# manuelbb-upb/Morbit.jl

Hardware: AMD Instinct MI355X
Metric: RBF build+solve+eval cycles/sec (higher is better)
Workload: dtype f64

## Files before the change

### include/mrbf.h

```cpp
#ifndef MRBF_H
#define MRBF_H

#include <stdint.h>

#ifdef __cplusplus
extern "C" {
#endif

typedef struct mrbf_ctx mrbf_ctx;
typedef struct mrbf_model mrbf_model;

enum {
    MRBF_CUBIC = 0,
    MRBF_INV_MULTIQUADRIC = 1,
    MRBF_MULTIQUADRIC = 2,
    MRBF_THIN_PLATE_SPLINE = 3,
    MRBF_GAUSSIAN = 4
};

enum {
    MRBF_OK = 0,
    MRBF_ENOTPD = 1,
    MRBF_ESINGULAR = 2,
    MRBF_EHIP = 3,
// ... 88 lines not shown
int32_t mrbf_affine_select(mrbf_ctx *ctx, int64_t mc, int32_t d, const double *shifted, int32_t j0, const double *Q0, int32_t max_picks,
                           double pivot_val, int32_t p_is_inf, int64_t *picked_out, int32_t *n_picked, double *Z_out);

typedef struct {
    int64_t mc;
    int32_t j0;
    int32_t max_picks;
    double pivot_val;
    const double *shifted;
    const double *Q0;
    int64_t *picked_out;
    double *Z_out;
    int32_t n_picked;
    int32_t reserved;
} mrbf_affine_job;
int32_t mrbf_affine_select_batch(mrbf_ctx *ctx, int64_t n_starts, int32_t d, int32_t p_is_inf, mrbf_affine_job *jobs,
                                 float *ms_total);

typedef struct mrbf_round4_state mrbf_round4_state;
int32_t mrbf_round4(mrbf_ctx *ctx, int64_t n0, int32_t d, const double *start_sites, int64_t mc, const double *cand_sites,
                    int32_t kernel_id, double a, double b, int32_t poly_deg, int32_t max_points, double theta_pivot_cholesky,
                    int32_t *accepted_out, int32_t *n_accepted, mrbf_round4_state **state);
int32_t mrbf_fit_from_round4(mrbf_ctx *ctx, const mrbf_round4_state *state, int32_t k, const double *values, mrbf_model **model,
                             double *weights_out, double *poly_out, mrbf_fit_info *info);
int32_t mrbf_round4_sites(const mrbf_round4_state *state, int64_t *n0, int64_t *n_candidates, int32_t *n_accepted);
int32_t mrbf_free_round4(mrbf_ctx *ctx, mrbf_round4_state *state);

typedef struct {
    int64_t n0, mc;
    const double *start_sites;
    const double *cand_sites;
    int32_t kernel_id, poly_deg;
    double a, b;
    int32_t max_points;
    double theta_pivot_cholesky;
    int32_t *accepted_out;
    int32_t n_accepted;
    int32_t rc;
} mrbf_round4_job;
int32_t mrbf_round4_batch(mrbf_ctx *ctx, int64_t n_starts, int32_t d, mrbf_round4_job *jobs, float *ms_total);

int32_t mrbf_model_dims(const mrbf_model *model, int64_t *n, int32_t *d, int32_t *k, int32_t *q);
int32_t mrbf_free_model(mrbf_ctx *ctx, mrbf_model *model);

typedef struct {
    int64_t n, m;
    int32_t d, k, kernel_id, poly_deg;
    double a, b;
    const double *centres;
    const double *values;
    const double *X;
    double *weights_out;
    double *poly_out;
    double *vals_out;
    double *jac_out;
} mrbf_problem;

typedef struct {
    int32_t status;
    int32_t device;
    mrbf_fit_info fit;
    float ms_eval;
    double checksum_w;
    double checksum_vals;
} mrbf_result;

int32_t mrbf_batch_run(int32_t n_dev, const int32_t *device_ids, int64_t n_problems, const mrbf_problem *problems,
                       mrbf_result *results);

typedef struct {
    int64_t n;
    int32_t d, k, kernel_id, poly_deg;
    double a, b;
    const double *centres, *values;
    double *weights_out, *poly_out;
    mrbf_model *model;
    int32_t status;
    int32_t reserved;
    mrbf_fit_info info;
} mrbf_fit_job;
int32_t mrbf_fit_batch(mrbf_ctx *ctx, int64_t n_starts, mrbf_fit_job *jobs, float *ms_total);

int32_t mrbf_debug_env(const char *name);
int32_t mrbf_debug_mfma_layout(mrbf_ctx *ctx, double *out16x16_a_times_b, const double *A16x4, const double *B4x16);
int32_t mrbf_debug_potrf(mrbf_ctx *ctx, int64_t n, double *A_colmajor_inout, int32_t impl, int32_t *info, float *ms);
int32_t mrbf_debug_diag(mrbf_ctx *ctx, const double *A128, int32_t reps, float *ms_per_call, double *shader_cycles,
                        double *realtime_us);
int32_t mrbf_debug_mfma_peak(mrbf_ctx *ctx, int32_t blocks_per_cu, int32_t threads, int32_t iters, float *ms, double *tflops);
int32_t mrbf_debug_mfma_asm(mrbf_ctx *ctx, int32_t variant, int32_t blocks_per_cu, int32_t iters, float *ms, double *tflops,
                            double *cycles_per_mfma);
int32_t mrbf_debug_dgemm(mrbf_ctx *ctx, int32_t m, int32_t n, int32_t k, float *ms, double *tflops);
int32_t mrbf_debug_mega_tables(int32_t nt, int32_t mt, int32_t slack, int32_t slack_chain, int32_t first, int32_t win, int32_t srows,
                               int32_t half_cols, int64_t *out6);
int32_t mrbf_debug_mega_tables2(int32_t nt, int32_t mt, int32_t slack, int32_t slack_chain, int32_t first, int32_t win, int32_t srows,
                                int32_t half_cols, const int32_t *opt5, int64_t *out6);
int32_t mrbf_debug_mega_plan(int32_t nt, int32_t mt, int32_t xreal, int64_t *out39);

enum { MRBF_PS_OK = 0, MRBF_PS_CRITICAL = 1, MRBF_PS_FAILURE = 2 };
typedef struct {
    int32_t max_ideal_evals;
    int32_t max_ps_evals;
    int32_t max_polish_evals;
    int32_t reserved;
    uint64_t seed;
    double t0;
    double xtol_rel;
} mrbf_ps_options;
typedef struct {
    int32_t status;
    int32_t generations;
    int32_t evals_ideal, evals_ps, evals_polish;
    float ms_total;
    double tau;
} mrbf_ps_info;
int32_t mrbf_ps_step(mrbf_ctx *ctx, const mrbf_model *model, const double *x_n, const double *lb_eff, const double *ub_eff,
                     const double *fx_n, const double *r_or_null, const mrbf_ps_options *opts, double *x_trial, double *mx_trial,
                     double *r_out, mrbf_ps_info *info);

enum { MRBF_ROLE_NONE = -1, MRBF_ROLE_EQ = -2, MRBF_ROLE_INEQ = -3 };
typedef struct {
    int32_t n_models, n_objectives;
    const mrbf_model *const *models;
    const int32_t *roles;
    int32_t n_lin_eq, n_lin_ineq;
    const double *A_eq, *b_eq, *A_ineq, *b_ineq;
    double eq_tol;
} mrbf_ps_problem;
int32_t mrbf_ps_step_problem(mrbf_ctx *ctx, const mrbf_ps_problem *problem, const double *x_n, const double *lb_eff,
                             const double *ub_eff, const double *fx_n, const double *r_or_null, const mrbf_ps_options *opts,
                             double *x_trial, double *mx_trial, double *r_out, mrbf_ps_info *info);
int32_t mrbf_debug_ps_rank(mrbf_ctx *ctx, int32_t lam, const double *f, const double *phi, uint64_t seed, int32_t gen, int32_t impl,
                           int32_t *order_out, int32_t *gave_up);

enum { MRBF_SD_OK = 0, MRBF_SD_NO_OBJECTIVE = 1, MRBF_SD_INFEASIBLE = 2, MRBF_SD_GAVE_UP = 3 };
int32_t mrbf_sd_direction(mrbf_ctx *ctx, int64_t n_lp, int32_t d, int32_t k, int32_t m_eq, int32_t m_ineq, const double *G,
                          const double *x, const double *lb, const double *ub, const double *A_eq, const double *b_eq,
                          const double *A_ineq, const double *b_ineq, int32_t normalize, double *d_out, double *omega_out,
                          double *dual_out, int32_t *status_out, int32_t *iters_out);
typedef struct {
    int32_t status;
    int32_t iterations;
    int32_t bound_flips;
    float ms_total;
    double omega;
} mrbf_sd_info;
int32_t mrbf_sd_criticality(mrbf_ctx *ctx, const mrbf_ps_problem *problem, const double *x, const double *x_n, const double *lb,
                            const double *ub, int32_t normalize, double *d_out, double *dual_out, mrbf_sd_info *info);

enum { MRBF_NS_OK = 0, MRBF_NS_INFEASIBLE = 1, MRBF_NS_GAVE_UP = 2 };
int32_t mrbf_normal_direction(mrbf_ctx *ctx, int64_t n_lp, int32_t d, int32_t m_eq, int32_t m_ineq, const double *x, const double *lb,
                              const double *ub, const double *A_eq, const double *b_eq, const double *A_ineq, const double *b_ineq,
                              double *n_out, double *alpha_out, double *dual_out, int32_t *status_out, int32_t *iters_out);
typedef struct {
    int32_t status;
    int32_t iterations;
    int32_t bound_flips;
    float ms_total;
    double alpha;
    double delta;
} mrbf_normal_info;
int32_t mrbf_normal_step(mrbf_ctx *ctx, const mrbf_ps_problem *problem, int32_t d, const double *x, const double *lb, const double *ub,
                         double delta, double kappa_delta, double delta_max, int32_t variable_radius, double *n_out, double *dual_out,
                         mrbf_normal_info *info);

typedef struct {
    int32_t strict;
    int32_t max_loops;
    double const_rhs;
    double shrink;
    double min_stepsize;
} mrbf_sd_step_options;
typedef struct {
    int32_t branch;
    int32_t loops;
    float ms_total;
    double sigma;
    double omega;
    double step_norm;
} mrbf_sd_step_info;
// ... 60 lines not shown
```

### morbit.jl_amd/_lib.py

```python
import ctypes
import os

import numpy as np

_HERE = os.path.dirname(os.path.abspath(__file__))
LIB_PATH = os.environ.get("MRBF_LIB") or os.path.join(_HERE, "libmrbf.so")

c_dp = ctypes.POINTER(ctypes.c_double)
c_fp = ctypes.POINTER(ctypes.c_float)
c_ip = ctypes.POINTER(ctypes.c_int32)
c_vp = ctypes.c_void_p

MRBF_OK, MRBF_ENOTPD, MRBF_ESINGULAR, MRBF_EHIP, MRBF_EBLAS, MRBF_ENOMEM, MRBF_ENODEVICE, MRBF_ENCCL = range(8)
PATH_CHOL, PATH_PROJ_CHOL, PATH_LU, PATH_MINNORM, PATH_ROUND4 = 1, 2, 3, 4, 5
OPT_GRAM_MODE, OPT_RESIDUAL, OPT_FORCE_PATH, OPT_CHOL_IMPL, OPT_EVAL_IMPL, OPT_TIMING, OPT_DIAG_IMPL, OPT_CHOL_WINDOW = 1, 2, 3, 4, 5, 6, 7, 8
OPT_SPIN_MS, OPT_DEBUG_FAULT, OPT_LAST_DEVICE_MS, OPT_SLOW_LAUNCHES = 9, 10, 11, 12
OPT_ARENA_BYTES, OPT_LIVE_HANDLES = 13, 14
FB_CHOL_HOST_DRIVEN, FB_BACKSOLVE_BLOCKED, FB_LU = 1, 2, 4


class FitInfo(ctypes.Structure):
    _fields_ = [("path", ctypes.c_int32), ("factor_info", ctypes.c_int32), ("n", ctypes.c_int32), ("q", ctypes.c_int32),
                ("rel_residual", ctypes.c_double), ("max_pitw", ctypes.c_double), ("mu", ctypes.c_double),
                ("ms_gram", ctypes.c_float), ("ms_project", ctypes.c_float), ("ms_factor", ctypes.c_float),
# ... 90 lines not shown
    _fields_ = [("status", ctypes.c_int32), ("iterations", ctypes.c_int32), ("bound_flips", ctypes.c_int32), ("reserved", ctypes.c_int32),
                ("alpha", ctypes.c_double), ("delta", ctypes.c_double)]

    def asdict(self):
        return {f: getattr(self, f) for f, _ in self._fields_}


class AffineJob(ctypes.Structure):
    _fields_ = [("mc", ctypes.c_int64), ("j0", ctypes.c_int32), ("max_picks", ctypes.c_int32), ("pivot_val", ctypes.c_double),
                ("shifted", ctypes.c_void_p), ("Q0", ctypes.c_void_p), ("picked_out", ctypes.c_void_p), ("Z_out", ctypes.c_void_p),
                ("n_picked", ctypes.c_int32), ("reserved", ctypes.c_int32)]


class Round4Job(ctypes.Structure):
    _fields_ = [("n0", ctypes.c_int64), ("mc", ctypes.c_int64), ("start_sites", ctypes.c_void_p), ("cand_sites", ctypes.c_void_p),
                ("kernel_id", ctypes.c_int32), ("poly_deg", ctypes.c_int32), ("a", ctypes.c_double), ("b", ctypes.c_double),
                ("max_points", ctypes.c_int32), ("theta_pivot_cholesky", ctypes.c_double), ("accepted_out", ctypes.c_void_p),
                ("n_accepted", ctypes.c_int32), ("rc", ctypes.c_int32)]


class FitJob(ctypes.Structure):
    _fields_ = [("n", ctypes.c_int64), ("d", ctypes.c_int32), ("k", ctypes.c_int32), ("kernel_id", ctypes.c_int32),
                ("poly_deg", ctypes.c_int32), ("a", ctypes.c_double), ("b", ctypes.c_double), ("centres", ctypes.c_void_p),
                ("values", ctypes.c_void_p), ("weights_out", ctypes.c_void_p), ("poly_out", ctypes.c_void_p), ("model", ctypes.c_void_p),
                ("status", ctypes.c_int32), ("reserved", ctypes.c_int32), ("info", FitInfo)]


class Problem(ctypes.Structure):
    _fields_ = [("n", ctypes.c_int64), ("m", ctypes.c_int64), ("d", ctypes.c_int32), ("k", ctypes.c_int32),
                ("kernel_id", ctypes.c_int32), ("poly_deg", ctypes.c_int32), ("a", ctypes.c_double), ("b", ctypes.c_double),
                ("centres", c_dp), ("values", c_dp), ("X", c_dp), ("weights_out", c_dp), ("poly_out", c_dp),
                ("vals_out", c_dp), ("jac_out", c_dp)]


class Result(ctypes.Structure):
    _fields_ = [("status", ctypes.c_int32), ("device", ctypes.c_int32), ("fit", FitInfo), ("ms_eval", ctypes.c_float),
                ("checksum_w", ctypes.c_double), ("checksum_vals", ctypes.c_double)]


SIGNATURES = {
    "mrbf_init": (ctypes.c_int32, [ctypes.c_int32, ctypes.POINTER(c_vp)]),
    "mrbf_shutdown": (ctypes.c_int32, [c_vp]),
    "mrbf_last_error": (ctypes.c_char_p, [c_vp]),
    "mrbf_version": (ctypes.c_char_p, []),
    "mrbf_set_option": (ctypes.c_int32, [c_vp, ctypes.c_int32, ctypes.c_double]),
    "mrbf_get_option": (ctypes.c_int32, [c_vp, ctypes.c_int32, c_dp]),
    "mrbf_set_stream": (ctypes.c_int32, [c_vp, c_vp]),
    "mrbf_sync": (ctypes.c_int32, [c_vp]),
    "mrbf_gram": (ctypes.c_int32, [c_vp, ctypes.c_int64, ctypes.c_int32, c_vp, ctypes.c_int32, ctypes.c_double,
                                   ctypes.c_double, ctypes.c_int32, c_vp, c_vp, c_fp]),
    "mrbf_cross_gram": (ctypes.c_int32, [c_vp, ctypes.c_int64, ctypes.c_int64, ctypes.c_int32, c_vp, c_vp, ctypes.c_int32, ctypes.c_double,
                                         ctypes.c_double, c_vp]),
    "mrbf_fit": (ctypes.c_int32, [c_vp, ctypes.c_int64, ctypes.c_int32, ctypes.c_int32, c_vp, c_vp, ctypes.c_int32,
                                  ctypes.c_double, ctypes.c_double, ctypes.c_int32, ctypes.POINTER(c_vp), c_vp, c_vp,
                                  ctypes.POINTER(FitInfo)]),
    "mrbf_model_from_coeffs": (ctypes.c_int32, [c_vp, ctypes.c_int64, ctypes.c_int32, ctypes.c_int32, c_vp, c_vp, c_vp,
                                                ctypes.c_int32, ctypes.c_double, ctypes.c_double, ctypes.c_int32,
                                                ctypes.POINTER(c_vp)]),
    "mrbf_eval": (ctypes.c_int32, [c_vp, c_vp, ctypes.c_int64, c_vp, c_vp, c_vp, ctypes.POINTER(EvalInfo)]),
    "mrbf_backtrack": (ctypes.c_int32, [c_vp, c_vp, c_vp, c_vp, ctypes.c_double, ctypes.c_double, ctypes.c_int32,
                                        ctypes.c_double, ctypes.c_double, ctypes.c_double, ctypes.c_int32, c_vp, c_vp,
                                        c_vp, c_ip]),
    "mrbf_affine_scores": (ctypes.c_int32, [c_vp, ctypes.c_int64, ctypes.c_int32, ctypes.c_int32, c_vp, c_vp, ctypes.c_int32, c_vp,
                                            ctypes.POINTER(ctypes.c_int64), c_dp]),
    "mrbf_affine_select": (ctypes.c_int32, [c_vp, ctypes.c_int64, ctypes.c_int32, c_vp, ctypes.c_int32, c_vp, ctypes.c_int32, ctypes.c_double,
                                            ctypes.c_int32, ctypes.POINTER(ctypes.c_int64), c_ip, c_vp]),
    "mrbf_affine_select_batch": (ctypes.c_int32, [c_vp, ctypes.c_int64, ctypes.c_int32, ctypes.c_int32, ctypes.POINTER(AffineJob), c_fp]),
    "mrbf_round4": (ctypes.c_int32, [c_vp, ctypes.c_int64, ctypes.c_int32, c_vp, ctypes.c_int64, c_vp, ctypes.c_int32, ctypes.c_double,
                                     ctypes.c_double, ctypes.c_int32, ctypes.c_int32, ctypes.c_double, c_vp, c_ip, ctypes.POINTER(c_vp)]),
    "mrbf_fit_from_round4": (ctypes.c_int32, [c_vp, c_vp, ctypes.c_int32, c_vp, ctypes.POINTER(c_vp), c_vp, c_vp, ctypes.POINTER(FitInfo)]),
    "mrbf_round4_sites": (ctypes.c_int32, [c_vp, ctypes.POINTER(ctypes.c_int64), ctypes.POINTER(ctypes.c_int64), c_ip]),
    "mrbf_free_round4": (ctypes.c_int32, [c_vp, c_vp]),
    "mrbf_round4_batch": (ctypes.c_int32, [c_vp, ctypes.c_int64, ctypes.c_int32, ctypes.POINTER(Round4Job), c_fp]),
    "mrbf_dispatch_round4_batch": (ctypes.c_int32, [ctypes.c_int64, ctypes.c_int32]),
    "mrbf_model_dims": (ctypes.c_int32, [c_vp, ctypes.POINTER(ctypes.c_int64), c_ip, c_ip, c_ip]),
    "mrbf_free_model": (ctypes.c_int32, [c_vp, c_vp]),
    "mrbf_batch_run": (ctypes.c_int32, [ctypes.c_int32, c_ip, ctypes.c_int64, ctypes.POINTER(Problem),
                                        ctypes.POINTER(Result)]),
    "mrbf_fit_batch": (ctypes.c_int32, [c_vp, ctypes.c_int64, ctypes.POINTER(FitJob), c_fp]),
    "mrbf_dispatch_fit_batch": (ctypes.c_int32, [ctypes.c_int64]),
    "mrbf_debug_mfma_layout": (ctypes.c_int32, [c_vp, c_vp, c_vp, c_vp]),
    "mrbf_debug_potrf": (ctypes.c_int32, [c_vp, ctypes.c_int64, c_vp, ctypes.c_int32, c_ip, c_fp]),
    "mrbf_debug_env": (ctypes.c_int32, [ctypes.c_char_p]),
    "mrbf_debug_diag": (ctypes.c_int32, [c_vp, c_vp, ctypes.c_int32, c_fp, c_dp, c_dp]),
    "mrbf_debug_ps_rank": (ctypes.c_int32, [c_vp, ctypes.c_int32, c_vp, c_vp, ctypes.c_uint64, ctypes.c_int32, ctypes.c_int32, c_ip, c_ip]),
    "mrbf_debug_mfma_peak": (ctypes.c_int32, [c_vp, ctypes.c_int32, ctypes.c_int32, ctypes.c_int32, c_fp, c_dp]),
    "mrbf_debug_mfma_asm": (ctypes.c_int32, [c_vp, ctypes.c_int32, ctypes.c_int32, ctypes.c_int32, c_fp, c_dp, c_dp]),
    "mrbf_debug_dgemm": (ctypes.c_int32, [c_vp, ctypes.c_int32, ctypes.c_int32, ctypes.c_int32, c_fp, c_dp]),
    "mrbf_debug_mega_tables": (ctypes.c_int32, [ctypes.c_int32] * 8 + [c_vp]),
    "mrbf_debug_mega_tables2": (ctypes.c_int32, [ctypes.c_int32] * 8 + [c_vp, c_vp]),
    "mrbf_debug_mega_plan": (ctypes.c_int32, [ctypes.c_int32] * 3 + [c_vp]),
    "mrbf_stochastic_rank": (ctypes.c_int32, [ctypes.c_int32, c_vp, c_vp, c_vp, ctypes.c_double, c_vp]),
    "mrbf_ps_step": (ctypes.c_int32, [c_vp, c_vp, c_vp, c_vp, c_vp, c_vp, c_vp, ctypes.POINTER(PsOptions), c_vp, c_vp, c_vp,
                                      ctypes.POINTER(PsInfo)]),
    "mrbf_ps_step_problem": (ctypes.c_int32, [c_vp, ctypes.POINTER(PsProblem), c_vp, c_vp, c_vp, c_vp, c_vp, ctypes.POINTER(PsOptions),
                                              c_vp, c_vp, c_vp, ctypes.POINTER(PsInfo)]),
    "mrbf_sd_direction": (ctypes.c_int32, [c_vp, ctypes.c_int64, ctypes.c_int32, ctypes.c_int32, ctypes.c_int32, ctypes.c_int32] + [c_vp] * 8
                          + [ctypes.c_int32, c_vp, c_vp, c_vp, c_vp, c_vp]),
    "mrbf_sd_criticality": (ctypes.c_int32, [c_vp, ctypes.POINTER(PsProblem), c_vp, c_vp, c_vp, c_vp, ctypes.c_int32, c_vp, c_vp,
                                             ctypes.POINTER(SdInfo)]),
    "mrbf_normal_direction": (ctypes.c_int32, [c_vp, ctypes.c_int64, ctypes.c_int32, ctypes.c_int32, ctypes.c_int32] + [c_vp] * 12),
    "mrbf_normal_step": (ctypes.c_int32, [c_vp, ctypes.POINTER(PsProblem), ctypes.c_int32, c_vp, c_vp, c_vp, ctypes.c_double, ctypes.c_double,
                                          ctypes.c_double, ctypes.c_int32, c_vp, c_vp, ctypes.POINTER(NormalInfo)]),
    "mrbf_sd_step": (ctypes.c_int32, [c_vp, ctypes.POINTER(PsProblem), c_vp, c_vp, ctypes.c_double, c_vp, c_vp, ctypes.c_double, c_vp,
                                      ctypes.POINTER(SdStepOptions), c_vp, c_vp, ctypes.POINTER(SdStepInfo)]),
    "mrbf_sd_iterate_batch": (ctypes.c_int32, [c_vp, ctypes.c_int64, ctypes.POINTER(PsProblem), ctypes.POINTER(ctypes.c_void_p), c_vp, c_vp, c_vp,
                                               c_vp, c_vp, ctypes.c_int32, ctypes.POINTER(SdStepOptions), c_vp, c_vp, c_vp,
                                               ctypes.POINTER(SdBatchRecord), c_fp]),
    "mrbf_dispatch_sd_batch": (ctypes.c_int32, [ctypes.c_int64] + [ctypes.c_int32] * 7),
    "mrbf_normal_step_batch": (ctypes.c_int32, [c_vp, ctypes.c_int64, ctypes.POINTER(PsProblem), ctypes.POINTER(ctypes.c_void_p), ctypes.c_int32,
                                                c_vp, c_vp, c_vp, c_vp, ctypes.c_double, ctypes.c_double, ctypes.c_int32, c_vp, c_vp, c_vp,
                                                ctypes.POINTER(NormalBatchRecord), c_fp]),
    "mrbf_dispatch_normal_batch": (ctypes.c_int32, [ctypes.c_int64] + [ctypes.c_int32] * 5),
    "mrbf_dispatch_ps": (ctypes.c_int32, [ctypes.c_int32] * 6),
    "mrbf_dispatch_sd_step": (ctypes.c_int32, [ctypes.c_int32] * 7),
    "mrbf_dispatch_sd": (ctypes.c_int32, [ctypes.c_int32] * 6),
    "mrbf_dispatch_normal": (ctypes.c_int32, [ctypes.c_int32] * 5),
    "mrbf_dispatch_backtrack": (ctypes.c_int32, [ctypes.c_int32] * 3),
    "mrbf_dispatch_affine": (ctypes.c_int32, [ctypes.c_int64, ctypes.c_int32]),
    "mrbf_dispatch_affine_batch": (ctypes.c_int32, [ctypes.c_int64, ctypes.c_int32, ctypes.c_int32]),
    "mrbf_dispatch_round4": (ctypes.c_int32, [ctypes.c_int64, ctypes.c_int32, ctypes.c_int32, ctypes.c_int64]),
    "mrbf_dispatch_fit": (ctypes.c_int32, [ctypes.c_int64, ctypes.c_int64, ctypes.c_int32, ctypes.c_int32, ctypes.c_int32]),
    "mrbf_dispatch_after": (ctypes.c_int32, [ctypes.c_int32, ctypes.c_int32]),
}

_LIB = None


class MrbfError(RuntimeError):
    def __init__(self, code, msg):
        super().__init__("libmrbf error %d: %s" % (code, msg))
        self.code = code


def load():
    global _LIB
    if _LIB is None:
        if not os.path.exists(LIB_PATH):
            raise ImportError("libmrbf.so is not built (%s); run `python -c 'import __graft_entry__ as g; g.build()'` "
                              "or `make -C morbit.jl_amd/csrc`. There is no CPU fallback." % LIB_PATH)
        lib = ctypes.CDLL(LIB_PATH)
        for name, (res, args) in SIGNATURES.items():
            fn = getattr(lib, name)
            fn.restype = res
            fn.argtypes = args
        _LIB = lib
    return _LIB


def as_ptr(a):
    if a is None:
        return None
    if isinstance(a, np.ndarray):
        return ctypes.c_void_p(a.ctypes.data)
    if hasattr(a, "data_ptr"):
        return ctypes.c_void_p(a.data_ptr())
    raise TypeError("expected numpy array or tensor, got %r" % type(a))


def host_f64(a, shape=None):
    a = np.ascontiguousarray(a, dtype=np.float64)
    if shape is not None:
        a = a.reshape(shape)
    return a


class Context:

    def __init__(self, device_id=-1):
        self.lib = load()
        h = c_vp()
        rc = self.lib.mrbf_init(device_id, ctypes.byref(h))
        if rc != 0:
            raise MrbfError(rc, (self.lib.mrbf_last_error(None) or b"").decode())
# ... 40 lines not shown
```

### morbit.jl_amd/csrc/api.hip

```cpp
#include <algorithm>
#include <mutex>
#include <thread>

#include "common.hpp"

using namespace mrbf;

namespace mrbf {
int check_kernel(mrbf_ctx *ctx, int kid, double a, double b, int deg, int argpos) {
    if (kid < 0 || kid > 4) return fail(ctx, -argpos, "kernel_id %d not in 0..4 (Morbit.RbfKernels)", kid);
    if (kid == MRBF_CUBIC && !(a >= 1.0 && std::fmod(a, 2.0) == 1.0))
        return fail(ctx, -(argpos + 1), "cubic exponent must be an odd integer >= 1 (got %g)", a);
    if (kid == MRBF_THIN_PLATE_SPLINE && !(a >= 1.0 && std::fmod(a, 1.0) == 0.0 && a <= 16.0))
        return fail(ctx, -(argpos + 1), "thin plate spline k must be an integer >= 1 (got %g)", a);
    if ((kid == MRBF_GAUSSIAN || kid == MRBF_MULTIQUADRIC || kid == MRBF_INV_MULTIQUADRIC) && !(a > 0.0))
        return fail(ctx, -(argpos + 1), "shape parameter must be strictly positive (got %g)", a);
    if (kid == MRBF_MULTIQUADRIC && !(b > 0.0 && std::fmod(b, 1.0) != 0.0))
        return fail(ctx, -(argpos + 2), "multiquadric exponent must be positive and non-integer (got %g)", b);
    if (kid == MRBF_INV_MULTIQUADRIC && !(b > 0.0))
        return fail(ctx, -(argpos + 2), "inverse multiquadric exponent must be positive (got %g)", b);
    if (deg < -1 || deg > 1) return fail(ctx, -(argpos + 3), "polynomial_degree must be -1, 0 or 1 (RbfModel.jl:21), got %d", deg);
    return 0;
}
}
// ... 297 lines not shown
    for (int t = 0; t < d; ++t) Xb[t] = hx[t];
    for (int i = 0; i < L; ++i)
        for (int t = 0; t < d; ++t) Xb[(size_t)(i + 1) * d + t] = hx[t] + steps[i] * hd[t];
    int rc = mrbf_eval(ctx, model, L + 1, Xb.data(), Vb.data(), nullptr, nullptr);
    if (rc != 0) return rc;
    const double *mx = Vb.data();
    int i = 0;
    while (i < max_loops) {
        const double *mp = Vb.data() + (size_t)(i + 1) * k;
        bool ok;
        if (strict) {
            ok = true;
            for (int l = 0; l < k; ++l) ok = ok && ((mx[l] - mp[l]) >= steps[i] * const_rhs * omega);
        } else {
            ok = (*std::max_element(mx, mx + k) - *std::max_element(mp, mp + k)) >= steps[i] * const_rhs * omega;
        }
        if (ok) break;
        if (steps[i] <= min_stepsize) break;
        ++i;
    }
    std::vector<double> hs(d);
    for (int t = 0; t < d; ++t) hs[t] = steps[i] * hd[t];
    auto put = [&](double *dst, const double *src, size_t cnt) -> int {
        if (!dst) return 0;
        if (is_device_ptr(dst)) {
            MRBF_HIP(ctx, hipMemcpy(dst, src, cnt * sizeof(double), hipMemcpyHostToDevice));
        } else {
            std::memcpy(dst, src, cnt * sizeof(double));
        }
        return 0;
    };
    MRBF_TRY(put(x_plus, Xb.data() + (size_t)(i + 1) * d, d));
    MRBF_TRY(put(mx_plus, Vb.data() + (size_t)(i + 1) * k, k));
    MRBF_TRY(put(step, hs.data(), d));
    if (n_loops) *n_loops = i;
    return MRBF_OK;
}

int32_t mrbf_model_dims(const mrbf_model *model, int64_t *n, int32_t *d, int32_t *k, int32_t *q) {
    if (!model) return -1;
    if (n) *n = model->n;
    if (d) *d = model->d;
    if (k) *k = model->k;
    if (q) *q = model->q;
    return MRBF_OK;
}

int32_t mrbf_free_model(mrbf_ctx *ctx, mrbf_model *model) {
    if (!ctx) return -1;
    if (!model) return MRBF_OK;
    (void)hipSetDevice(ctx->device);
    (void)hipStreamSynchronize(ctx->stream);
    destroy_model(ctx, model);
    return MRBF_OK;
}

}

extern "C" int32_t mrbf_stochastic_rank(int32_t lam, const double *f, const double *phi, const double *u, double pf, int32_t *idx_out) {
    if (lam <= 0) return -1;
    if (!f) return -2;
    if (!phi) return -3;
    if (!u) return -4;
    if (!idx_out) return -6;
    for (int32_t i = 0; i < lam; ++i) idx_out[i] = i;
    for (int32_t sweep = 0; sweep < lam; ++sweep) {
        bool swapped = false;
        const double *us = u + (size_t)sweep * (size_t)(lam - 1);
        for (int32_t j = 0; j + 1 < lam; ++j) {
            const int32_t a = idx_out[j], b = idx_out[j + 1];
            const bool by_f = (phi[a] == 0.0 && phi[b] == 0.0) || us[j] < pf;
            const bool worse = by_f ? (f[a] > f[b]) : (phi[a] > phi[b]);
            if (worse) {
                idx_out[j] = b;
                idx_out[j + 1] = a;
                swapped = true;
            }
        }
        if (!swapped) break;
    }
    return MRBF_OK;
}

extern "C" int32_t mrbf_debug_env(const char *name) {
    if (!name) return -1;
    return mrbf::mrbf_env(name) ? 1 : 0;
}
```

### morbit.jl_amd/csrc/batch.hip

```cpp
#include <algorithm>
#include <thread>

#include "common.hpp"
#include "small.hpp"

namespace mrbf {

int batch_run_chain(int n_dev, const int *devs, const std::vector<int64_t> &which, const mrbf_problem *problems, mrbf_result *results);
mrbf_ctx *batch_pool_acquire(int device, int *rc);
void batch_pool_release(mrbf_ctx *c);
void fill_small_prob(const mrbf_ctx *ctx, const mrbf_model *M, const double *Y, double *ws, int *flags, double *scal, int *cl, smallfit::Prob *P);
int small_fit_verdict(const mrbf_model *M, const int *hflags, const double *hscal, mrbf_fit_info *info);
int check_kernel(mrbf_ctx *ctx, int kid, double a, double b, int deg, int argpos);

struct CheckDesc {
    const double *V, *Y;
    const double *C, *Wc, *W;
    const double *vals;
    int64_t n, npad, m;
    int d, k, q;
    double *out;
};

__global__ __launch_bounds__(256) void batch_check_kernel(const CheckDesc *__restrict__ many, int part) {
// ... 35 lines not shown
    const double *V = E.V, *Y = E.Y;
    const double s0 = strided_sum(E.n * E.k, [&](int64_t i) { const double df = V[i] - Y[i]; return df * df; });
    const double s1 = strided_sum(E.n * E.k, [&](int64_t i) { return Y[i] * Y[i]; });
    tree(s0, s1, false);
    if (tid == 0) {
        E.out[0] = r0[0];
        E.out[1] = r1[0];
    }
    __syncthreads();
    double mx = 0.0;
    for (int e = tid; e < E.q * E.k; e += 256) {
        const int t = e % E.q, l = e / E.q;
        const double *wl = E.Wc + (int64_t)l * E.npad;
        double acc = 0.0;
        int64_t i = 0;
        for (; i + 8 <= E.n; i += 8) {
            double c[8], w[8];
#pragma unroll
            for (int u = 0; u < 8; ++u) {
                c[u] = t == 0 ? 1.0 : E.C[(i + u) * E.d + (t - 1)];
                w[u] = wl[i + u];
            }
#pragma unroll
            for (int u = 0; u < 8; ++u) acc = fma(c[u], w[u], acc);
        }
        for (; i < E.n; ++i) acc = fma(t == 0 ? 1.0 : E.C[i * E.d + (t - 1)], wl[i], acc);
        mx = fmax(mx, fabs(acc));
    }
    const double *W = E.W;
    const double sw = strided_sum(E.n * E.k, [&](int64_t i) { return W[i]; });
    tree(mx, sw, true);
    if (tid == 0) {
        E.out[2] = r0[0];
        E.out[3] = r1[0];
    }
}

static inline size_t al16(size_t c) { return (c + 15) & ~size_t(15); }

struct CopySeg {
    const double *src;
    double *dst;
    int64_t cnt;
};
__global__ __launch_bounds__(256) void batch_copy_kernel(const CopySeg *__restrict__ many) {
    const CopySeg S = many[blockIdx.y];
    const int tid = threadIdx.x;
    if (((reinterpret_cast<uintptr_t>(S.src) | reinterpret_cast<uintptr_t>(S.dst)) & 15) == 0) {
        const double2 *__restrict__ s2 = reinterpret_cast<const double2 *>(S.src);
        double2 *__restrict__ d2 = reinterpret_cast<double2 *>(S.dst);
        const int64_t pairs = S.cnt >> 1;
        for (int64_t i0 = (int64_t)blockIdx.x * 1024 + tid; i0 < pairs; i0 += (int64_t)gridDim.x * 1024) {
            double2 v[4];
#pragma unroll
            for (int u = 0; u < 4; ++u)
                if (i0 + 256 * u < pairs) v[u] = s2[i0 + 256 * u];
#pragma unroll
            for (int u = 0; u < 4; ++u)
                if (i0 + 256 * u < pairs) d2[i0 + 256 * u] = v[u];
        }
        if ((S.cnt & 1) && blockIdx.x == 0 && tid == 0) S.dst[S.cnt - 1] = S.src[S.cnt - 1];
    } else {
        for (int64_t i = (int64_t)blockIdx.x * 256 + tid; i < S.cnt; i += (int64_t)gridDim.x * 256) S.dst[i] = S.src[i];
    }
}
static int launch_batch_copy(mrbf_ctx *ctx, const CopySeg *hsegs, const CopySeg *dsegs, int count) {
    int64_t longest = 0;
    for (int i = 0; i < count; ++i) longest = std::max(longest, hsegs[i].cnt);
    if (longest == 0) return 0;
    const unsigned gx = (unsigned)std::min<int64_t>((longest + 2047) / 2048, 256);
    hipLaunchKernelGGL(batch_copy_kernel, dim3(gx, (unsigned)count), dim3(256), 0, ctx->stream, dsegs);
    MRBF_HIP(ctx, hipGetLastError());
    return 0;
}

static int run_small_batch(mrbf_ctx *ctx, const std::vector<int64_t> &idx, const mrbf_problem *problems, mrbf_result *results,
                           std::vector<int64_t> *redo, int force_nc = 0, const mrbf_model *keep = nullptr, float *ms_sum = nullptr) {
    const int P = (int)idx.size();
    if (P == 0) return 0;
    (void)hipSetDevice(ctx->device);
    struct Lay {
        size_t C, Y, X, Xc, sq, mean, W, Wc, lam, ws, Xq0, xsq0, vp0, gp0, V0, Xq1, xsq1, vp1, gp1, vals, jac, out;
        int nsplit0, nsplit1, D, q, KO;
        int64_t npad, mpad0, mpad1;
        bool w_host, lam_host;
    };
    std::vector<Lay> lay(P);
    size_t total = 0;
    auto take = [&](size_t cnt) {
        const size_t at = total;
        total += al16(std::max<size_t>(cnt, 1));
        return at;
    };
    const bool check = ctx->residual != 0;
    const size_t out0 = take((size_t)10 * P);
    for (int i = 0; i < P; ++i) {
        const mrbf_problem &pr = problems[idx[i]];
        Lay &L = lay[i];
        const int d = pr.d, k = pr.k;
        L.q = poly_dim(d, pr.poly_deg);
        L.npad = round_up(pr.n, 128);
        L.D = d <= 64 ? 64 : 128;
        L.KO = outputs_per_pass(k, L.D);
        const int q16 = (int)round_up(std::max(L.q, 1), 16);
        L.C = (keep || is_device_ptr(pr.centres)) ? (size_t)-1 : take((size_t)pr.n * d);
        L.Y = is_device_ptr(pr.values) ? (size_t)-1 : take((size_t)pr.n * k);
        L.X = (pr.m == 0 || is_device_ptr(pr.X)) ? (size_t)-1 : take((size_t)pr.m * d);
        const bool w_dev = pr.weights_out && is_device_ptr(pr.weights_out), lam_dev = pr.poly_out && L.q > 0 && is_device_ptr(pr.poly_out);
        L.w_host = pr.weights_out && !w_dev;
        L.lam_host = pr.poly_out && L.q > 0 && !lam_dev;
        L.Xc = L.sq = L.mean = L.W = L.Wc = L.lam = (size_t)-1;
        if (!keep) {
            L.Xc = take((size_t)L.npad * L.D);
            L.sq = take((size_t)L.npad);
            L.mean = take((size_t)L.D);
            if (!w_dev) L.W = take((size_t)pr.n * k);
            L.Wc = take((size_t)L.npad * k);
            if (!lam_dev) L.lam = take((size_t)std::max(L.q, 1) * k);
        }
        L.ws = take(smallfit::carve((int)L.npad, q16).total);
        L.mpad0 = check ? round_up(pr.n, 64) : 0;
        L.nsplit0 = check ? eval_nsplit(ctx, pr.n, (int)((pr.n + 63) / 64), true) : 1;
        L.Xq0 = take((size_t)L.mpad0 * L.D);
        L.xsq0 = take((size_t)L.mpad0);
        L.vp0 = take(L.nsplit0 > 1 ? (size_t)L.nsplit0 * L.mpad0 * L.KO * 2 : 0);
        L.gp0 = take((size_t)0);
        L.V0 = take((size_t)pr.n * k);
        L.mpad1 = round_up(pr.m, 64);
        L.nsplit1 = pr.m > 0 ? eval_nsplit(ctx, pr.m, (int)((pr.n + 63) / 64)) : 1;
        L.Xq1 = take((size_t)L.mpad1 * L.D);
        L.xsq1 = take((size_t)L.mpad1);
        L.vp1 = take(L.nsplit1 > 1 ? (size_t)L.nsplit1 * L.mpad1 * L.KO * 2 : 0);
        L.gp1 = take((pr.jac_out && L.nsplit1 > 1) ? (size_t)L.nsplit1 * L.mpad1 * L.KO * L.D : 0);
        L.vals = (pr.m == 0 || (pr.vals_out && is_device_ptr(pr.vals_out))) ? (size_t)-1 : take((size_t)pr.m * k);
        L.jac = (pr.m == 0 || !pr.jac_out || is_device_ptr(pr.jac_out)) ? (size_t)-1 : take((size_t)pr.m * k * d);
        L.out = out0 + (size_t)8 * i;
    }
    const size_t arena_budget = (size_t)(mrbf_env("MRBF_BATCH_ARENA_MB") ? atoll(mrbf_env("MRBF_BATCH_ARENA_MB")) : 8192) << 20;
    auto halves = [&]() -> int {
        const std::vector<int64_t> lo(idx.begin(), idx.begin() + P / 2), hi(idx.begin() + P / 2, idx.end());
        MRBF_TRY(run_small_batch(ctx, lo, problems, results, redo, force_nc, keep, ms_sum));
        return run_small_batch(ctx, hi, problems, results, redo, force_nc, keep, ms_sum);
    };
    if (P > 1 && total * sizeof(double) > arena_budget) return halves();
    double *base;
    int *flags = nullptr;
    {
        const int rc = get_buf(ctx, S_SMALL_WS, total, &base);
        if (rc == MRBF_ENOMEM && P > 1) return halves();
        if (rc != 0) return rc;
    }
    flags = reinterpret_cast<int *>(base + out0 + (size_t)8 * P);
    PinGuard pin(ctx);
    const size_t desc_bytes = (size_t)P * (sizeof(smallfit::Prob) + 2 * sizeof(EvalDesc) + sizeof(CheckDesc) + smallfit::CL_WORDS * sizeof(int) +
                                           (keep ? 3 * sizeof(CopySeg) : 0)) + 256;
    char *ddesc;
    MRBF_TRY(get_buf(ctx, S_SMALL_DESC, desc_bytes, (void **)&ddesc));
    smallfit::Prob *dprobs = (smallfit::Prob *)ddesc;
    EvalDesc *devs_ = (EvalDesc *)(ddesc + al16((size_t)P * sizeof(smallfit::Prob)));
    CheckDesc *dchk = (CheckDesc *)((char *)devs_ + al16((size_t)2 * P * sizeof(EvalDesc)));
    int *dcl = (int *)((char *)dchk + al16((size_t)P * sizeof(CheckDesc)));
    CopySeg *dsegs = (CopySeg *)((char *)dcl + al16((size_t)P * smallfit::CL_WORDS * sizeof(int)));
    std::vector<CopySeg> segs(keep ? (size_t)3 * P : 0, CopySeg{nullptr, nullptr, 0});
    std::vector<char> hdesc;
    std::vector<smallfit::Prob> probs(P);
    std::vector<EvalDesc> evs((size_t)2 * P);
    std::vector<CheckDesc> chk(P);
    std::vector<mrbf_model> models(P);
    hipStream_t st = ctx->stream;
    auto dev_in = [&](const double *user, size_t off, size_t cnt, const double **out) -> int {
        if (off == (size_t)-1) {
            *out = user;
            return 0;
        }
        MRBF_HIP(ctx, hipMemcpyAsync(base + off, user, cnt * sizeof(double), hipMemcpyHostToDevice, st));
        *out = base + off;
        return 0;
    };
    for (int i = 0; i < P; ++i) {
        const mrbf_problem &pr = problems[idx[i]];
        const Lay &L = lay[i];
        const double *C, *Y, *X = nullptr;
        if (keep) {
            C = keep[idx[i]].C;
            if (is_device_ptr(pr.centres))
                segs[i] = CopySeg{pr.centres, keep[idx[i]].C, pr.n * pr.d};
            else
                MRBF_HIP(ctx, hipMemcpyAsync(keep[idx[i]].C, pr.centres, (size_t)pr.n * pr.d * sizeof(double), hipMemcpyHostToDevice, st));
        } else {
            MRBF_TRY(dev_in(pr.centres, L.C, (size_t)pr.n * pr.d, &C));
        }
        MRBF_TRY(dev_in(pr.values, L.Y, (size_t)pr.n * pr.k, &Y));
        if (pr.m > 0) MRBF_TRY(dev_in(pr.X, L.X, (size_t)pr.m * pr.d, &X));
        mrbf_model &M = models[i];
        M.n = pr.n;
        M.npad = L.npad;
        M.d = pr.d;
        M.dpad = L.D;
        M.k = pr.k;
        M.q = L.q;
        M.deg = pr.poly_deg;
        M.kp = make_kp(pr.kernel_id, pr.a, pr.b);
        M.C = const_cast<double *>(C);
        if (keep) {
            const mrbf_model &K = keep[idx[i]];
            M.Xc = K.Xc;
            M.sq = K.sq;
            M.mean = K.mean;
            M.W = K.W;
            M.Wc = K.Wc;
            M.lam = K.lam;
            if (pr.weights_out && !L.w_host) segs[(size_t)P + i] = CopySeg{M.W, pr.weights_out, pr.n * pr.k};
            if (pr.poly_out && L.q > 0 && !L.lam_host) segs[(size_t)2 * P + i] = CopySeg{M.lam, pr.poly_out, (int64_t)L.q * pr.k};
        } else {
            M.Xc = base + L.Xc;
            M.sq = base + L.sq;
            M.mean = base + L.mean;
            M.W = L.W == (size_t)-1 ? pr.weights_out : base + L.W;
            M.Wc = base + L.Wc;
            M.lam = L.lam == (size_t)-1 ? pr.poly_out : base + L.lam;
        }
        fill_small_prob(ctx, &M, Y, base + L.ws, flags + 4 * i, base + L.out + 5, dcl + smallfit::CL_WORDS * i, &probs[i]);
        probs[i].mean_given = 1;
        for (int e = 0; e < 2; ++e) {
            EvalDesc &E = evs[(size_t)e * P + i];
            eval_desc_model(E, &M, e == 0 ? (check ? pr.n : 0) : pr.m, e == 0 ? L.nsplit0 : L.nsplit1);
            E.X = e == 0 ? C : X;
            E.Xq = base + (e == 0 ? L.Xq0 : L.Xq1);
            E.xsq = base + (e == 0 ? L.xsq0 : L.xsq1);
            E.vpart = base + (e == 0 ? L.vp0 : L.vp1);
            E.sapart = E.vpart + (size_t)E.nsplit * E.mpad * L.KO;
            E.gpart = base + (e == 0 ? L.gp0 : L.gp1);
            E.vals = e == 0 ? base + L.V0 : (L.vals == (size_t)-1 ? pr.vals_out : base + L.vals);
            E.jac = e == 0 ? nullptr : (pr.jac_out ? (L.jac == (size_t)-1 ? pr.jac_out : base + L.jac) : nullptr);
        }
        CheckDesc &K = chk[i];
        K.V = base + L.V0;
        K.Y = Y;
        K.C = C;
        K.Wc = M.Wc;
        K.W = M.W;
        K.vals = pr.m > 0 ? evs[(size_t)P + i].vals : nullptr;
        K.n = check ? pr.n : 0;
        K.npad = L.npad;
        K.m = pr.m;
        K.d = pr.d;
        K.k = pr.k;
        K.q = check ? L.q : 0;
        K.out = base + L.out;
    }
    {
        char *hd = desc_bytes <= ((size_t)4 << 20) ? pin_take(ctx, desc_bytes) : nullptr;
        if (hd) {
            memset(hd, 0, desc_bytes);
        } else {
            hdesc.assign(desc_bytes, 0);
            hd = hdesc.data();
        }
        memcpy(hd, probs.data(), (size_t)P * sizeof(smallfit::Prob));
        memcpy(hd + ((char *)devs_ - ddesc), evs.data(), (size_t)2 * P * sizeof(EvalDesc));
        memcpy(hd + ((char *)dchk - ddesc), chk.data(), (size_t)P * sizeof(CheckDesc));
        if (keep) memcpy(hd + ((char *)dsegs - ddesc), segs.data(), segs.size() * sizeof(CopySeg));
        MRBF_HIP(ctx, hipMemcpyAsync(ddesc, hd, desc_bytes, hipMemcpyHostToDevice, st));
    }
    MRBF_HIP(ctx, hipEventRecord(ctx->ev[0], st));
    const int nc = force_nc > 0 ? force_nc : small_fit_cluster(ctx, P);
    hipStream_t side = (ctx->panel_stream && ctx->panel_stream != st) ? ctx->panel_stream : st;
    if (keep) MRBF_TRY(launch_batch_copy(ctx, segs.data(), dsegs, P));
    MRBF_TRY(launch_small_means(ctx, dprobs, P));
    if (side != st) {
        MRBF_HIP(ctx, hipEventRecord(ctx->evx[0], st));
        MRBF_HIP(ctx, hipStreamWaitEvent(side, ctx->evx[0], 0));
    }
    MRBF_TRY(launch_small_fit(ctx, probs.data(), P, dprobs, nc));
    MRBF_HIP(ctx, hipEventRecord(ctx->ev[1], st));
    if (keep) {
        MRBF_TRY(launch_batch_copy(ctx, segs.data() + P, dsegs + P, P));
        MRBF_TRY(launch_batch_copy(ctx, segs.data() + 2 * (size_t)P, dsegs + 2 * (size_t)P, P));
    }
    {
        int64_t max_mpad = 0;
        for (const EvalDesc &E : evs) max_mpad = std::max(max_mpad, E.mpad);
        ctx->stream = side;
        const int rc = max_mpad > 0 ? center_pad_batch(ctx, devs_, 2 * P, max_mpad) : 0;
        ctx->stream = st;
        if (rc != 0) return rc;
    }
    if (side != st) {
        MRBF_HIP(ctx, hipEventRecord(ctx->evx[0], st));
        MRBF_HIP(ctx, hipStreamWaitEvent(side, ctx->evx[0], 0));
        MRBF_HIP(ctx, hipEventRecord(ctx->evx[2], side));
        MRBF_HIP(ctx, hipStreamWaitEvent(st, ctx->evx[2], 0));
    }
    {
        struct RestoreStream {
            mrbf_ctx *c;
            hipStream_t s;
            ~RestoreStream() { c->stream = s; }
        } restore{ctx, st};
        std::vector<char> done((size_t)2 * P, 0);
        for (size_t a = 0; a < evs.size(); ++a) {
            if (done[a]) continue;
            const mrbf_problem &pa = problems[idx[a % P]];
            const KP kpa = evs[a].kp;
            const bool ja = evs[a].jac != nullptr;
            const bool is_check = a < (size_t)P;
            std::vector<EvalDesc> grp;
            std::vector<size_t> members;
            for (size_t b = a; b < (is_check ? (size_t)P : evs.size()); ++b) {
                const mrbf_problem &pb = problems[idx[b % P]];
                if (!done[b] && evs[b].kp.kid == kpa.kid && evs[b].kp.fast == kpa.fast && lay[b % P].D == lay[a % P].D && pb.k == pa.k &&
                    (evs[b].jac != nullptr) == ja && (evs[b].nsplit > 1) == (evs[a].nsplit > 1)) {
                    done[b] = 1;
                    if (evs[b].m > 0) members.push_back(b);
// ... 283 lines not shown
```

### morbit.jl_amd/csrc/batch_chain.hpp

```cpp
#pragma once
#include "small.hpp"

namespace mrbf {
namespace chain {

inline int batch_fetch(mrbf_ctx *ctx, const double *src, size_t cnt, double *dst) {
    if (!cnt) return 0;
    if (is_device_ptr(src)) MRBF_HIP(ctx, hipMemcpy(dst, src, cnt * sizeof(double), hipMemcpyDeviceToHost));
    else std::memcpy(dst, src, cnt * sizeof(double));
    return 0;
}

constexpr int64_t MAX_GROUP_LAUNCH = 65535;

struct Member {
    int site, j;
    int64_t p;
    int group;
    const mrbf_model *M;
    int64_t mq;
    bool jac;
    size_t X = 0, vals = 0, jacs = 0;
    size_t Xq = 0, xsq = 0, vpart = 0, gpart = 0;
    int64_t mpad = 0;
    int nsplit = 1, KO = 0;
};
struct Group {
    int site, D, k;
    bool jac;
    KP kp;
    std::vector<size_t> members;
    size_t first;
};

struct Plan {
    std::vector<Member> mem;
    std::vector<Group> groups;
    size_t n_desc = 0;

    void add(const mrbf_ctx *ctx, int site, int64_t p, int j, const mrbf_model *M, int64_t mq, bool jac) {
        Member mb;
        mb.site = site, mb.j = j, mb.p = p, mb.M = M, mb.mq = mq, mb.jac = jac;
        mb.nsplit = eval_nsplit(ctx, mq, (int)((M->n + 63) / 64));
        mb.group = group_of(ctx, site, M, jac, mb.nsplit > 1);
        if (mb.group >= 0) groups[mb.group].members.push_back(mem.size());
        mem.push_back(mb);
    }
    void close() {
        n_desc = 0;
        for (Group &G : groups) G.first = n_desc, n_desc += G.members.size();
    }
    size_t desc_doubles() const { return (n_desc * sizeof(EvalDesc) + sizeof(double) - 1) / sizeof(double); }
    template <class Take>
    void carve(Take &&take) {
        for (Member &S : mem) {
            if (S.group < 0) continue;
            S.mpad = round_up(S.mq, 64);
            S.KO = outputs_per_pass(S.M->k, S.M->dpad, S.jac);
            S.Xq = take((size_t)S.mpad * S.M->dpad);
            S.xsq = take((size_t)S.mpad);
            S.vpart = take(S.nsplit > 1 ? (size_t)S.nsplit * S.mpad * S.KO * 2 : 0);
            S.gpart = take((S.nsplit > 1 && S.jac) ? (size_t)S.nsplit * S.mpad * S.KO * S.M->dpad : 0);
        }
    }
    void fill(double *base, EvalDesc *hdesc) const {
        for (const Group &G : groups)
            for (size_t r = 0; r < G.members.size(); ++r) {
                const Member &S = mem[G.members[r]];
                EvalDesc E;
                std::memset(&E, 0, sizeof(E));
                eval_desc_model(E, S.M, S.mq, S.nsplit);
                E.X = base + S.X;
                E.Xq = base + S.Xq;
                E.xsq = base + S.xsq;
                if (S.nsplit > 1) {
                    E.vpart = base + S.vpart;
                    E.sapart = E.vpart + (size_t)S.nsplit * S.mpad * S.KO;
                    if (S.jac) E.gpart = base + S.gpart;
                }
                E.vals = base + S.vals;
                E.jac = S.jac ? base + S.jacs : nullptr;
                std::memcpy(&hdesc[G.first + r], &E, sizeof(E));
            }
    }
    int launch(mrbf_ctx *ctx, int site, double *base, const EvalDesc *hdesc, const EvalDesc *ddesc) const {
        for (const Group &G : groups) {
            if (G.site != site) continue;
            for (size_t r0 = 0; r0 < G.members.size(); r0 += MAX_GROUP_LAUNCH) {
                const int cnt = (int)std::min<size_t>(MAX_GROUP_LAUNCH, G.members.size() - r0);
                MRBF_TRY(eval_fused_batch(ctx, G.kp, G.D, G.k, G.jac, hdesc + G.first + r0, ddesc + G.first + r0, cnt));
            }
        }
        for (const Member &S : mem) {
            if (S.site != site || S.group >= 0) continue;
            MRBF_TRY(eval_model(ctx, S.M, S.mq, base + S.X, base + S.vals, S.jac ? base + S.jacs : nullptr, nullptr));
        }
        return 0;
    }

private:
    int group_of(const mrbf_ctx *ctx, int site, const mrbf_model *M, bool jac, bool split) {
        if (ctx->eval_impl == 1 || !(M->dpad == 64 || M->dpad == 128 || M->dpad == 256)) return -1;
        for (size_t g = 0; g < groups.size(); ++g) {
            const Group &G = groups[g];
            if (G.site == site && G.D == M->dpad && G.k == M->k && G.jac == jac && std::memcmp(&G.kp, &M->kp, sizeof(KP)) == 0) {
                return (int)(g & ~(size_t)1) + (split ? 1 : 0);
            }
        }
        for (int s = 0; s < 2; ++s) {
            Group G;
            G.site = site, G.D = M->dpad, G.k = M->k, G.jac = jac, G.kp = M->kp, G.first = 0;
            groups.push_back(G);
        }
        return (int)groups.size() - 2 + (split ? 1 : 0);
    }
};

}
}
```

### morbit.jl_amd/csrc/chol_blocked.hip

```cpp
#include "common.hpp"
#include "mega_gemm.hpp"

namespace mrbf {

typedef double v4d __attribute__((ext_vector_type(4)));
typedef double v2d __attribute__((ext_vector_type(2)));

constexpr int CNB = 128;

enum { UPD_LOWER_SUB = 0, UPD_OVERWRITE = 1, UPD_FULL_SUB = 2, UPD_COLUMN_SUB = 3 };
int launch_diag_v4(mrbf_ctx *ctx, hipStream_t st, double *Ajj, int64_t lda, double *Linv, int *dinfo, int col0);

template <int TM, int MODE>
__global__ __launch_bounds__(256, 2) void chol_update_kernel(const double *__restrict__ A, int64_t lda,
                                                             const double *__restrict__ B, int64_t ldb,
                                                             double *__restrict__ C, int64_t ldc, int K,
                                                             const int *__restrict__ info, int mt_sq = 0, int ntiles_total = 0,
                                                             const double *__restrict__ cvec = nullptr, double cs = 0.0, int64_t cn = 0) {
    constexpr int NJ = (TM == 128) ? 4 : 2;
    __shared__ __attribute__((aligned(16))) double smem[mega::NSTG * mega::STG];
    if (info && *info != 0) return;
    if (MODE == UPD_OVERWRITE || MODE == UPD_COLUMN_SUB) __builtin_amdgcn_s_setprio(2);
    const int tid = threadIdx.x, lane = tid & 63, wave = tid >> 6;
    const int l15 = lane & 15, l4 = lane >> 4;
    const int tile_end = (MODE == UPD_LOWER_SUB && ntiles_total > 0) ? ntiles_total : (int)blockIdx.x + 1;
    for (int bid = blockIdx.x; bid < tile_end; bid += gridDim.x) {
    int ti, tj;
    if (MODE == UPD_LOWER_SUB) {
        const int ntri = mt_sq * (mt_sq + 1) / 2;
        if (bid < ntri || mt_sq == 0) {
            int t = (int)((sqrt(8.0 * (double)bid + 1.0) - 1.0) * 0.5);
            while ((t + 1) * (t + 2) / 2 <= bid) ++t;
            while (t * (t + 1) / 2 > bid) --t;
            ti = t;
            tj = bid - t * (t + 1) / 2;
        } else {
            ti = mt_sq + (bid - ntri) / mt_sq;
            tj = (bid - ntri) % mt_sq;
        }
    } else {
        ti = blockIdx.x;
        tj = blockIdx.y;
    }
    const int64_t I0 = (int64_t)ti * TM, J0 = (int64_t)tj * 128;
    const int ioff = (TM == 128) ? (wave >> 1) * 64 : 0;
    const int joff = (TM == 128) ? (wave & 1) * 64 : wave * 32;

    v4d acc[NJ][4];
#pragma unroll
    for (int j = 0; j < NJ; ++j)
#pragma unroll
        for (int i = 0; i < 4; ++i) acc[j][i] = (v4d){0.0, 0.0, 0.0, 0.0};

    asm volatile("s_waitcnt vmcnt(0)" ::: "memory");
    constexpr bool NEG_START = (MODE == UPD_LOWER_SUB);
    if (NEG_START) {
#pragma unroll
        for (int j = 0; j < NJ; ++j)
#pragma unroll
            for (int r = 0; r < 4; ++r) {
                const int64_t gj = J0 + joff + j * 16 + l4 + 4 * r;
#pragma unroll
                for (int i = 0; i < 4; ++i) acc[j][i][r] = -C[(I0 + ioff + i * 16 + l15) + gj * ldc];
            }
    }
    mega::gemm_acc<TM>(A + I0, lda, B + J0, ldb, K, acc, smem);
    double cvi[4] = {0.0, 0.0, 0.0, 0.0}, cei[4] = {0.0, 0.0, 0.0, 0.0};
    if (MODE == UPD_LOWER_SUB && cvec) {
#pragma unroll
        for (int i = 0; i < 4; ++i) {
            const int64_t gi = I0 + ioff + i * 16 + l15;
            cvi[i] = cs * cvec[gi];
            cei[i] = gi < cn ? cs : 0.0;
        }
    }
#pragma unroll
    for (int j = 0; j < NJ; ++j) {
        double cv[4][4];
        double cvj[4] = {0.0, 0.0, 0.0, 0.0}, cej[4] = {0.0, 0.0, 0.0, 0.0};
        if (MODE == UPD_LOWER_SUB && cvec) {
#pragma unroll
            for (int r = 0; r < 4; ++r) {
                const int64_t gj = J0 + joff + j * 16 + l4 + 4 * r;
                cvj[r] = cvec[gj];
                cej[r] = gj < cn ? 1.0 : 0.0;
            }
        }
        if (MODE != UPD_OVERWRITE && !NEG_START) {
#pragma unroll
            for (int r = 0; r < 4; ++r) {
                const int64_t gj = J0 + joff + j * 16 + l4 + 4 * r;
#pragma unroll
                for (int i = 0; i < 4; ++i) cv[r][i] = C[(I0 + ioff + i * 16 + l15) + gj * ldc];
            }
        }
#pragma unroll
        for (int r = 0; r < 4; ++r) {
            const int64_t gj = J0 + joff + j * 16 + l4 + 4 * r;
#pragma unroll
            for (int i = 0; i < 4; ++i) {
                const int64_t gi = I0 + ioff + i * 16 + l15;
                double *dst = C + gi + gj * ldc;
                if (MODE == UPD_OVERWRITE) {
                    *dst = acc[j][i][r];
                } else if (MODE == UPD_FULL_SUB) {
                    *dst = cv[r][i] - acc[j][i][r];
                } else if (MODE == UPD_COLUMN_SUB) {
                    if (gi >= gj) *dst = cv[r][i] - acc[j][i][r];
                } else {
                    double x = -acc[j][i][r];
                    if (cvec) x -= fma(cei[i], cvj[r], cvi[i] * cej[r]);
                    if (ti != tj || gi >= gj) *dst = x;
                }
            }
        }
    }
    if (bid + (int)gridDim.x < tile_end) __syncthreads();
    }
}

struct __attribute__((aligned(16))) DiagShared {
    double col[2][2 * CNB];
    double rinv[2];
    int sbad;
    unsigned long long seg[4];
    int stamp;
};

__device__ __forceinline__ double fast_rsqrt(double x) {
    double y = __builtin_amdgcn_rsq(x);
    const double h = 0.5 * x;
#pragma unroll
    for (int it = 0; it < 3; ++it) y = y * fma(-h, y * y, 1.5);
    return y;
}

template <int KV, bool STAMP>
__device__ __forceinline__ void diag_phase(double (&a)[8][8], DiagShared &sh, int ti, int tj, int half, int &buf, int &bad) {
    constexpr int KN = (KV < 7) ? KV + 1 : 7;
    double piv = 0.0;
    if (half == 0) piv = __shfl(a[KV][KV], tj, 16);
#pragma unroll 1
    for (int kk = 0; kk < 16; ++kk) {
        const int k = KV * 16 + kk;
        const bool st = STAMP && threadIdx.x < 64;
        unsigned long long s0 = 0, s1 = 0, s2 = 0, s3 = 0;
        if (st) s0 = __builtin_amdgcn_s_memtime();
        __syncthreads();
        if (st) s1 = __builtin_amdgcn_s_memtime();
        double lj[8];
#pragma unroll
        for (int v = KV; v < 8; ++v) lj[v] = sh.col[buf][tj + 16 * v];
        if (half == 0) {
            double li[8];
#pragma unroll
            for (int u = KV; u < 8; ++u) li[u] = sh.col[buf][ti + 16 * u];
            if (st) {
                asm volatile("s_waitcnt lgkmcnt(0)" ::: "memory");
                s2 = __builtin_amdgcn_s_memtime();
            }
            if (kk < 15) {
                if (tj > kk) piv = fma(-lj[KV], lj[KV], piv);
                if (tj == kk + 1) {
                    const int kn = k + 1;
                    double rinv = 0.0;
                    if (piv > 0.0) {
                        rinv = fast_rsqrt(piv);
                    } else if (bad == 0) {
                        bad = kn + 1;
                    }
                    if (ti == 0) sh.rinv[buf ^ 1] = rinv;
                    double w[8];
#pragma unroll
                    for (int u = 0; u < 8; ++u) {
                        const int i = ti + 16 * u;
                        double val = 0.0;
                        if (u >= KV && i >= kn) {
                            val = fma(-li[u], lj[KV], a[u][KV]) * rinv;
                            a[u][KV] = val;
                        }
                        w[u] = val;
                    }
#pragma unroll
                    for (int u = 0; u < 8; ++u) sh.col[buf ^ 1][ti + 16 * u] = w[u];
                }
            } else if (KV < 7) {
                if (tj == 0) {
                    const int kn = k + 1;
                    const double pv = __shfl(fma(-li[KN], lj[KN], a[KN][KN]), 0, 16);
                    double rinv = 0.0;
                    if (pv > 0.0) {
                        rinv = fast_rsqrt(pv);
                    } else if (bad == 0) {
                        bad = kn + 1;
                    }
                    if (ti == 0) sh.rinv[buf ^ 1] = rinv;
                    double w[8];
#pragma unroll
                    for (int u = 0; u < 8; ++u) {
// ... 118 lines not shown
    __syncthreads();
    if (sh.sbad != 0x7fffffff) {
        if (tid == 0) *info = col0 + sh.sbad;
        return;
    }
#pragma unroll
    for (int v = 0; v < 8; ++v)
#pragma unroll
        for (int u = 0; u < 8; ++u) {
            const int i = ti + 16 * u, j = tj + 16 * v;
            if (half == 0) {
                if (i >= j) A[i + (int64_t)j * lda] = a[u][v];
            } else {
                Linv[j + i * CNB] = (j >= i) ? a[u][v] : 0.0;
            }
        }
    if (STAMP && threadIdx.x == 0) {
        stamps[0] = __builtin_amdgcn_s_memtime() - t0;
        stamps[1] = __builtin_amdgcn_s_memrealtime() - r0;
        for (int q = 0; q < 4; ++q) stamps[2 + q] = sh.seg[q];
    }
}

__global__ void pad_identity_kernel(double *__restrict__ A, int64_t n, int64_t npad, int64_t ld) {
    const int64_t idx = (int64_t)blockIdx.x * blockDim.x + threadIdx.x;
    const int64_t pw = npad - n;
    if (idx >= npad * pw) return;
    const int64_t j = n + idx / npad, i = idx % npad;
    A[i + j * ld] = (i == j) ? 1.0 : 0.0;
    if (i < n) A[j + i * ld] = 0.0;
}

int launch_pad_identity(mrbf_ctx *ctx, double *A, int64_t n, int64_t npad, int64_t ld) {
    if (npad == n) return 0;
    const int64_t cnt = npad * (npad - n);
    hipLaunchKernelGGL(pad_identity_kernel, dim3((unsigned)((cnt + 255) / 256)), dim3(256), 0, ctx->stream, A, n, npad, ld);
    MRBF_HIP(ctx, hipGetLastError());
    return 0;
}

int debug_diag(mrbf_ctx *ctx, const double *A128_dev, int reps, float *ms_per_call, unsigned long long *stamps_host) {
    const bool with_stamps = reps > 0;
    if (reps < 0) reps = -reps;
    double *W, *Linv;
    int *dinfo;
    unsigned long long *st;
    MRBF_TRY(get_buf(ctx, S_PHI, (size_t)CNB * CNB * reps, &W));
    MRBF_TRY(get_buf(ctx, S_CHOL_WS, (size_t)CNB * CNB, &Linv));
    MRBF_TRY(get_buf(ctx, S_INFO, (size_t)4, &dinfo));
    MRBF_TRY(get_buf(ctx, S_MISC, (size_t)8, (double **)&st));
    for (int r = 0; r < reps; ++r)
        MRBF_HIP(ctx, hipMemcpyAsync(W + (size_t)r * CNB * CNB, A128_dev, sizeof(double) * CNB * CNB, hipMemcpyDeviceToDevice, ctx->stream));
    MRBF_HIP(ctx, hipMemsetAsync(dinfo, 0, sizeof(int), ctx->stream));
    MRBF_HIP(ctx, hipEventRecord(ctx->ev[0], ctx->stream));
    for (int r = 0; r < reps; ++r)
        if (ctx->diag_impl != 1)
            launch_diag_v4(ctx, ctx->stream, W + (size_t)r * CNB * CNB, (int64_t)CNB, Linv, dinfo, 0);
        else if (with_stamps)
            hipLaunchKernelGGL(chol_diag_kernel<true>, dim3(1), dim3(512), 0, ctx->stream, W + (size_t)r * CNB * CNB, (int64_t)CNB, Linv,
                               dinfo, 0, st);
        else
            hipLaunchKernelGGL(chol_diag_kernel<false>, dim3(1), dim3(512), 0, ctx->stream, W + (size_t)r * CNB * CNB, (int64_t)CNB, Linv,
                               dinfo, 0, (unsigned long long *)nullptr);
    MRBF_HIP(ctx, hipEventRecord(ctx->ev[1], ctx->stream));
    MRBF_HIP(ctx, hipEventSynchronize(ctx->ev[1]));
    float t;
    MRBF_HIP(ctx, hipEventElapsedTime(&t, ctx->ev[0], ctx->ev[1]));
    *ms_per_call = t / reps;
    if (const char *e = mrbf_env("MRBF_DIAG_DBG")) {
        if (atoi(e) & 4) {
            double seg[6];
            MRBF_HIP(ctx, hipMemcpy(seg, Linv, sizeof(seg), hipMemcpyDeviceToHost));
            fprintf(stderr, "diag segments (wave 0, cycles over 8 panels): pre-leaf %.0f leaf %.0f post-leaf %.0f wait-X %.0f deferred %.0f wait-Y %.0f\n",
                    seg[0], seg[1], seg[2], seg[3], seg[4], seg[5]);
        }
    }
    MRBF_HIP(ctx, hipMemcpy(stamps_host, st, 6 * sizeof(unsigned long long), hipMemcpyDeviceToHost));
    return 0;
}

int launch_update_lower(mrbf_ctx *ctx, const double *A, int64_t lda, const double *B, int64_t ldb, double *C, int64_t ldc, int64_t nt,
                        int K, const double *cvec, double cs, int64_t cn) {
    if (nt <= 0 || K <= 0) return 0;
    hipLaunchKernelGGL((chol_update_kernel<128, UPD_LOWER_SUB>), dim3((unsigned)(nt * (nt + 1) / 2)), dim3(256), 0, ctx->stream, A,
                       lda, B, ldb, C, ldc, K, (const int *)nullptr, (int)nt, 0, cvec, cs, cn);
    MRBF_HIP(ctx, hipGetLastError());
    return 0;
}

int potrf_blocked_tall(mrbf_ctx *ctx, int64_t ncols, int64_t mrows, double *A, int64_t lda, int *dinfo, double *linv_all, PotrfOpts opt) {
    if (ncols % CNB != 0 || mrows % CNB != 0 || mrows < ncols || (lda & 1) || (reinterpret_cast<uintptr_t>(A) & 15))
        return fail(ctx, MRBF_EHIP, "potrf_blocked needs 128-padded, 16-byte aligned storage (ncols=%lld mrows=%lld lda=%lld)",
                    (long long)ncols, (long long)mrows, (long long)lda);
    const int impl = opt.impl != 0 ? opt.impl : ctx->chol_impl;
    if ((impl == 3 || (impl == 0 && ncols <= ctx->mega.max)) && (opt.any_size || ncols >= ctx->mega.min))
        return potrf_mega_tall(ctx, ncols, mrows, A, lda, dinfo, linv_all, opt);
    double *Lone = nullptr;
    if (!linv_all) MRBF_TRY(get_buf(ctx, S_CHOL_WS, (size_t)CNB * CNB, &Lone));
    hipStream_t S = ctx->stream, M = ctx->bulk_stream, P = ctx->panel_stream;
    hipEvent_t evStart = ctx->evx[0], evT = ctx->evx[1], evU2 = ctx->evx[2], evEnd = ctx->evx[3];
    const bool single = ncols <= 4 * CNB;
    if (single) M = P = S;
    MRBF_HIP(ctx, hipMemsetAsync(dinfo, 0, sizeof(int), S));
    if (!single) {
        MRBF_HIP(ctx, hipEventRecord(evStart, S));
        MRBF_HIP(ctx, hipStreamWaitEvent(P, evStart, 0));
        MRBF_HIP(ctx, hipStreamWaitEvent(M, evStart, 0));
    }
    const int nb = (int)(ncols / CNB);
    bool have_u2 = false;
    int w0 = 0, W = 1;
    for (int j = 0; j < nb; ++j) {
        const int64_t c = (int64_t)j * CNB;
        if (j == w0) {
            const int64_t rem = ncols - c;
            W = (rem > 4800) ? 4 : (rem > 2400 ? 2 : 1);
            if (ctx->chol_window > 0) W = ctx->chol_window;
        }
        const bool last_in_window = (j == w0 + W - 1) || (j == nb - 1);
        const int kpan = (int)((j - w0 + 1) * CNB);
        const int64_t cw = (int64_t)w0 * CNB;
        double *Ajj = A + c + c * lda;
        double *Linv = linv_all ? linv_all + (size_t)j * CNB * CNB : Lone;
        if (ctx->diag_impl == 1)
            hipLaunchKernelGGL(chol_diag_kernel<false>, dim3(1), dim3(512), 0, P, Ajj, lda, Linv, dinfo, (int)c,
                               (unsigned long long *)nullptr);
        else
            launch_diag_v4(ctx, P, Ajj, lda, Linv, dinfo, (int)c);
        const int64_t m = mrows - c - CNB;
        if (m <= 0) break;
        double *A21 = A + (c + CNB) + c * lda;
        hipLaunchKernelGGL((chol_update_kernel<64, UPD_OVERWRITE>), dim3((unsigned)(m / 64), 1), dim3(256), 0, P, A21, lda, Linv,
                           (int64_t)CNB, A21, lda, CNB, dinfo);
        if (c + CNB >= ncols) break;
        if (!single) MRBF_HIP(ctx, hipEventRecord(evT, P));
        if (have_u2 && !single) {
            MRBF_HIP(ctx, hipStreamWaitEvent(P, evU2, 0));
            have_u2 = false;
        }
        const double *Pw = A + (c + CNB) + cw * lda;
        double *A22 = A + (c + CNB) + (c + CNB) * lda;
        hipLaunchKernelGGL((chol_update_kernel<64, UPD_COLUMN_SUB>), dim3((unsigned)(m / 64), 1), dim3(256), 0, P, Pw, lda, Pw, lda,
                           A22, lda, kpan, dinfo);
        if (last_in_window) {
            const int64_t mt2 = (ncols - c - 2 * CNB) / CNB;
            if (mt2 > 0) {
                if (!single) MRBF_HIP(ctx, hipStreamWaitEvent(M, evT, 0));
                const int64_t mx = (mrows - ncols) / CNB;
                const int64_t rem_next = ncols - c - CNB;
                int Wn = (rem_next > 4800) ? 4 : (rem_next > 2400 ? 2 : 1);
                if (ctx->chol_window > 0) Wn = ctx->chol_window;
                const int64_t na = std::min<int64_t>(Wn, mt2);
                const double *P2 = A + (c + 2 * CNB) + cw * lda;
                double *C2 = A + (c + 2 * CNB) + (c + 2 * CNB) * lda;
                hipLaunchKernelGGL((chol_update_kernel<128, UPD_LOWER_SUB>),
                                   dim3((unsigned)(na * (na + 1) / 2 + (mt2 - na + mx) * na)), dim3(256), 0, M, P2, lda, P2, lda, C2, lda,
                                   kpan, dinfo, (int)na);
                if (!single) MRBF_HIP(ctx, hipEventRecord(evU2, M));
                have_u2 = true;
                const int64_t mb2 = mt2 - na;
                if (mb2 > 0) {
                    const double *P3 = P2 + na * CNB;
                    double *C3 = C2 + na * CNB + na * CNB * lda;
                    const int64_t nt3 = mb2 * (mb2 + 1) / 2 + mx * mb2;
                    const int64_t g3 = (ctx->bulk_grid > 0 && nt3 > ctx->bulk_grid) ? ctx->bulk_grid : nt3;
                    hipLaunchKernelGGL((chol_update_kernel<128, UPD_LOWER_SUB>), dim3((unsigned)g3), dim3(256), 0, M, P3, lda, P3, lda,
                                       C3, lda, kpan, dinfo, (int)mb2, (int)nt3);
                }
// ... 104 lines not shown
```

### morbit.jl_amd/csrc/common.hpp

```cpp
#pragma once
#include <hip/hip_runtime.h>
#include <rocblas/rocblas.h>
#include <rocsolver/rocsolver.h>

#include <cmath>
#include <cstdlib>
#include <cstdint>
#include <cstdio>
#include <cstring>
#include <map>
#include <string>
#include <vector>

#include "../../include/mrbf.h"
#include "model_pool.hpp"

namespace mrbf {

struct KP {
    int kid;
    double a, b;
    double a2;
    double sgn;
    int fast;
    int ik;
    double phi0;
};
KP make_kp(int kid, double a, double b);
int cpd_order(int kid, double a, double b);
inline int poly_dim(int d, int deg) { return deg < 0 ? 0 : (deg == 0 ? 1 : d + 1); }

enum Slot {
    S_XC = 0, S_SQ, S_MEAN, S_PHI, S_PI, S_Q1, S_W1, S_G, S_R, S_TAU, S_RHS, S_T1, S_T2, S_IPIV, S_INFO,
    S_STAGE_A, S_STAGE_B, S_STAGE_C, S_STAGE_D, S_EVAL_E, S_EVAL_A, S_EVAL_J, S_EVAL_SA, S_EVAL_XC, S_EVAL_XSQ,
    S_OUT_A, S_OUT_B, S_CHOL_WS, S_MISC, S_MEGA_JOBS, S_MEGA_FLAGS, S_MEGA_WQ, S_MEGA_IT, S_BSOLVE_FLAGS, S_MEGA_TRACE, S_MEGA_JLOG,
    S_T1W, S_PS_STATE, S_PS_STAT, S_PS_POLISH, S_BSOLVE_X, S_V0, S_QR_INV, S_DIAG_SCR, S_SMALL_WS, S_SMALL_DESC, S_SMALL_FLAGS, S_MEGA_STAT, S_BSOLVE_M, S_SMALL_CL, S_GW_PART, S_GW_RS, S_GW_GP, S_GW_M, S_CHECK_SCAL, S_TAIL_PART, S_PS_RANK, S_SD_IN, S_SD_OUT, S_SD_WS, S_NS_IN, S_NS_OUT, S_NS_WS, S_SD_STEP, S_SD_BATCH, S_AFF_BATCH, S_NS_BATCH, S_R4_BATCH, S_NSLOTS
};
}

namespace mrbf {
namespace mega {
struct Edge {
    int head, tail_c0, srows_edge, pstream_edge;
    int shalf, sh_head, sh_tail_c0;
    int tfull1;
    int xhalf;
};
struct TableParams {
    int slack, slack_chain, first, win, srows, half_cols, tail_half, tail_half_w, chainq;
    Edge edge;
};
constexpr bool operator==(const TableParams &a, const TableParams &b) {
    return a.slack == b.slack && a.slack_chain == b.slack_chain && a.first == b.first && a.win == b.win && a.srows == b.srows &&
           a.half_cols == b.half_cols && a.tail_half == b.tail_half && a.tail_half_w == b.tail_half_w && a.chainq == b.chainq &&
           a.edge.head == b.edge.head && a.edge.tail_c0 == b.edge.tail_c0 && a.edge.srows_edge == b.edge.srows_edge &&
           a.edge.pstream_edge == b.edge.pstream_edge && a.edge.shalf == b.edge.shalf && a.edge.sh_head == b.edge.sh_head &&
           a.edge.sh_tail_c0 == b.edge.sh_tail_c0 && a.edge.tfull1 == b.edge.tfull1 && a.edge.xhalf == b.edge.xhalf;
}
struct Knobs {
    int grid = 512, dedicated = 64, look = 2, quiet = 1, slack = 3, half_cols = 0, first_window = 1, wbias = 4, xhalf = 1, chainq = 0, cboost = 12, panel_dma = 1;
    int min = 256, max = 32768;
    int chain = 0, slack_chain = 0, win = 0, pstream = 0, srows = 0;
    int shalf = -1, shalf_head = -1, head = -1, tail = -1, reserve = -1, tail_half = -1, tail_half_w = -1, xchain = -1, quiet_tail = -1;
    int tfull = -1;
};
}
struct MegaTables {
    int nt, mt;
    mega::TableParams params;
    void *block, *jobs, *wq;
    int npanel, nbulk, nchainjobs, nwin;
    unsigned long long stamp;
};
struct PotrfOpts {
    int impl = 0;
    bool any_size = false;
    int xreal = 0;
    bool info_clean = false;
};
struct EvalHints {
    bool population = false;
    bool check_call = false;
    const double *pre_xq = nullptr;
};
}

struct mrbf_ctx {
    int device = 0;
    int ncu = 256;
    hipStream_t own_stream = nullptr;
    hipStream_t stream = nullptr;
    rocblas_handle blas = nullptr;
    mrbf::Buf slots[mrbf::S_NSLOTS];
    hipEvent_t ev[8] = {};
    hipStream_t panel_stream = nullptr;
    hipEvent_t evx[4] = {};
    hipStream_t bulk_stream = nullptr;
    int bulk_masked = 0;
    int bulk_grid = 384;
    mrbf::mega::Knobs mega;
    std::string err;
    std::vector<mrbf::Buf> model_pool;
    int gram_mode = 0, residual = 1, force_path = 0, chol_impl = 0, eval_impl = 0, timing = 1, diag_impl = 0, chol_window = 0;
    int spin_ms = 1000, debug_fault = 0;
    unsigned long long *mega_stat_dev = nullptr;
    long mega_stat_shape = 0;
    int mega_stat_pending = 0;
    char *pin_base = nullptr;
    size_t pin_off = 0;
    bool pin_armed = false;
    struct PinOut {
        void *user;
        const void *pin;
        size_t bytes;
    };
    std::vector<PinOut> pin_out;
    unsigned long long *hpin = nullptr;
    float last_device_ms = 0.f;
    int slow_launches = 0;
    int small_nc = 4;
    int small_cluster_ok = 0;
    int small_timeouts = 0;
    int live_models = 0, live_round4 = 0;
    unsigned ps_rank_epoch = 0;
    int ps_multi_off = 0;
    std::map<long, float> mega_best_ms;
    std::vector<mrbf::MegaTables> mega_tables;
    unsigned long long mega_table_clock = 0;
};

struct mrbf_model {
    int64_t n = 0, npad = 0;
    int d = 0, dpad = 0, k = 0, q = 0, deg = -1;
    mrbf::KP kp{};
    double *C = nullptr;
    double *Xc = nullptr;
    double *sq = nullptr;
    double *mean = nullptr;
    double *W = nullptr;
    double *Wc = nullptr;
    double *lam = nullptr;
    void *block = nullptr;
    size_t block_bytes = 0;
    mrbf::ModelSlab *slab = nullptr;
};

namespace mrbf {

int fail(mrbf_ctx *ctx, int code, const char *fmt, ...);
#define MRBF_HIP(ctx, call)                                                                                  \
    do {                                                                                                      \
        hipError_t e__ = (call);                                                                              \
        if (e__ != hipSuccess)                                                                                \
            return mrbf::fail(ctx, e__ == hipErrorOutOfMemory ? MRBF_ENOMEM : MRBF_EHIP, "%s: %s (%s:%d)", #call, \
                              hipGetErrorString(e__), __FILE__, __LINE__);                                    \
    } while (0)
#define MRBF_BLAS(ctx, call)                                                                                 \
    do {                                                                                                      \
        rocblas_status s__ = (call);                                                                          \
        if (s__ != rocblas_status_success)                                                                    \
            return mrbf::fail(ctx, MRBF_EBLAS, "%s: rocblas status %d (%s:%d)", #call, (int)s__, __FILE__, __LINE__); \
    } while (0)
#define MRBF_TRY(call)             \
    do {                           \
        int rc__ = (call);         \
        if (rc__ != 0) return rc__; \
    } while (0)

int get_buf(mrbf_ctx *ctx, Slot s, size_t bytes, void **out);
template <class T>
inline int get_buf(mrbf_ctx *ctx, Slot s, size_t count, T **out) {
    return get_buf(ctx, s, count * sizeof(T), (void **)out);
}
bool is_device_ptr(const void *p);
int stage_in(mrbf_ctx *ctx, Slot s, const double *user, size_t count, const double **dev);
int stage_out(mrbf_ctx *ctx, Slot s, double *user, size_t count, double **dev);
int finish_out(mrbf_ctx *ctx, double *user, const double *dev, size_t count);
void pin_reset(mrbf_ctx *ctx);
void pin_flush(mrbf_ctx *ctx);
void pin_discard(mrbf_ctx *ctx);
char *pin_take(mrbf_ctx *ctx, size_t bytes);
struct PinGuard {
    mrbf_ctx *ctx;
    bool flushed = false;
    explicit PinGuard(mrbf_ctx *c) : ctx(c) { pin_reset(c); }
    void flush() {
        pin_flush(ctx);
// ... 61 lines not shown
```

### morbit.jl_amd/csrc/eval_fused.hip

```cpp
#include <type_traits>

#include "radial.hpp"
#ifndef MRBF_EVAL_DBG
#define MRBF_EVAL_DBG 0
#endif
#include "small.hpp"

namespace mrbf {

typedef double v4d __attribute__((ext_vector_type(4)));
typedef double v2d __attribute__((ext_vector_type(2)));

constexpr int EQ = 64;
constexpr int EC = 64;

template <int KID, bool FAST, int KOUT, bool JAC, bool FINAL>
__global__ __launch_bounds__(256, 2) void eval_fused_kernel(EvalDesc one, const EvalDesc *__restrict__ many, int l0) {
    constexpr int D = 64, DT = D / 16, LDC = D + 2;
    __shared__ __attribute__((aligned(16))) double Cs[EC * LDC];
    __shared__ double Ws[KOUT * EC];
    __shared__ double Sq[EC];
    const EvalDesc &E = many ? many[blockIdx.z] : one;
    if (many && ((int64_t)blockIdx.x * EQ >= E.mpad || (int)blockIdx.y >= E.nsplit)) return;
    const double *__restrict__ Xq = E.Xq;
    const double *__restrict__ Cc = E.Cc;
    const double *__restrict__ csq = E.csq;
    const double *__restrict__ Wc = E.Wc;
    const int64_t npad = E.npad, mpad = E.mpad;
    const int tiles_per_split = E.tiles_per_split;
    const KP kp = E.kp;
    const int tid = threadIdx.x, lane = tid & 63, wave = tid >> 6;
    const int l15 = lane & 15, l4 = lane >> 4;
    const int64_t q0 = (int64_t)blockIdx.x * EQ;
    const int split = blockIdx.y;
    const int64_t qrow = q0 + wave * 16 + l15;

    double xb[D / 4];
#pragma unroll
    for (int s = 0; s < D / 4; ++s) xb[s] = Xq[qrow * D + 4 * s + l4];
    const double xs = E.xsq[qrow];

    v4d JT[KOUT][DT];
    double vsum[KOUT], sasum[KOUT];
#pragma unroll
    for (int l = 0; l < KOUT; ++l) {
        vsum[l] = 0.0;
        sasum[l] = 0.0;
#pragma unroll
        for (int t = 0; t < DT; ++t) JT[l][t] = (v4d){0.0, 0.0, 0.0, 0.0};
    }

    const int64_t c_begin = (int64_t)split * tiles_per_split * EC;
    const int ntiles_all = E.ntiles;
    const int nsub = __builtin_amdgcn_readfirstlane(E.nsub);
    const int my_tiles = min(tiles_per_split, ntiles_all - split * tiles_per_split);
    constexpr int NLD = 2 * DT;
    v2d stg[NLD];
    auto load_tile = [&](int64_t c0) {
        const v2d *src = reinterpret_cast<const v2d *>(Cc + c0 * D);
#pragma unroll
        for (int u = 0; u < NLD; ++u) stg[u] = src[tid + 256 * u];
    };
    auto store_tile = [&]() {
#pragma unroll
        for (int u = 0; u < NLD; ++u) {
            const int e = (tid + 256 * u) * 2;
            const int row = e / D, col = e % D;
            *(v2d *)&Cs[row * LDC + col] = stg[u];
        }
    };
    constexpr int NSC = ((KOUT + 1) * EC + 255) / 256;
    double stg_s[NSC];
    auto load_scalars = [&](int64_t c0) {
#pragma unroll
        for (int u = 0; u < NSC; ++u) {
            const int e = tid + 256 * u;
            if (e < EC)
                stg_s[u] = csq[c0 + e];
            else if (e < (KOUT + 1) * EC)
                stg_s[u] = Wc[(int64_t)(l0 + (e - EC) / EC) * npad + c0 + ((e - EC) % EC)];
        }
    };
    load_tile(c_begin);
    load_scalars(c_begin);
    for (int tile = 0; tile < my_tiles; ++tile) {
        const int64_t c0 = c_begin + (int64_t)tile * EC;
        __syncthreads();
        store_tile();
#pragma unroll
        for (int u = 0; u < NSC; ++u) {
            const int e = tid + 256 * u;
            if (e < EC)
                Sq[e] = stg_s[u];
            else if (e < (KOUT + 1) * EC)
                Ws[e - EC] = stg_s[u];
        }
        __syncthreads();
        if (tile + 1 < my_tiles) {
            load_tile(c0 + EC);
            load_scalars(c0 + EC);
        }
#pragma unroll
        for (int ct = 0; ct < 4; ++ct) {
            if ((int)(c0 >> 4) + ct >= nsub) break;
            v4d S = {0.0, 0.0, 0.0, 0.0};
            const double *crow = &Cs[(16 * ct + l15) * LDC + l4];
#pragma unroll
            for (int s = 0; s < D / 4; ++s) S = __builtin_amdgcn_mfma_f64_16x16x4f64(crow[4 * s], xb[s], S, 0, 0, 0);
            v4d Aw[KOUT];
#pragma unroll
            for (int r = 0; r < 4; ++r) {
                const int c = 16 * ct + l4 + 4 * r;
                double s2 = fma(-2.0, S[r], xs + Sq[c]);
                s2 = s2 > 0.0 ? s2 : 0.0;
                double phi, psi;
                rbf_phi_psi_t<KID, FAST>(s2, kp, phi, psi);
#pragma unroll
                for (int l = 0; l < KOUT; ++l) {
                    const double w = Ws[l * EC + c];
                    vsum[l] = fma(w, phi, vsum[l]);
                    if constexpr (JAC) {
                        const double a = w * psi;
                        sasum[l] += a;
                        Aw[l][r] = a;
                    }
                }
            }
            if (JAC) {
#pragma unroll
                for (int tt = 0; tt < DT; ++tt) {
#pragma unroll
                    for (int s = 0; s < 4; ++s) {
                        const double cop = Cs[(16 * ct + 4 * s + l4) * LDC + 16 * tt + l15];
#pragma unroll
                        for (int l = 0; l < KOUT; ++l) JT[l][tt] = __builtin_amdgcn_mfma_f64_16x16x4f64(cop, Aw[l][s], JT[l][tt], 0, 0, 0);
                    }
                }
            }
        }
    }
#pragma unroll
    for (int l = 0; l < KOUT; ++l) {
        vsum[l] += __shfl_xor(vsum[l], 16);
        vsum[l] += __shfl_xor(vsum[l], 32);
        sasum[l] += __shfl_xor(sasum[l], 16);
        sasum[l] += __shfl_xor(sasum[l], 32);
    }
    if constexpr (!FINAL) {
        double *__restrict__ vpart = E.vpart, *__restrict__ sapart = E.sapart, *__restrict__ gpart = E.gpart;
        if (l4 == 0) {
#pragma unroll
            for (int l = 0; l < KOUT; ++l) {
                vpart[((int64_t)split * mpad + qrow) * KOUT + l] = vsum[l];
                sapart[((int64_t)split * mpad + qrow) * KOUT + l] = sasum[l];
            }
        }
        if (JAC) {
            __syncthreads();
            double *T = Cs + wave * 16 * LDC;
#pragma unroll
            for (int l = 0; l < KOUT; ++l) {
#pragma unroll
                for (int tt = 0; tt < DT; ++tt)
#pragma unroll
                    for (int r = 0; r < 4; ++r) T[l15 * LDC + 16 * tt + l4 + 4 * r] = JT[l][tt][r];
                __syncthreads();
                for (int e = lane; e < 16 * D; e += 64) {
                    const int qq = e / D, t = e % D;
                    gpart[(((int64_t)split * mpad + q0 + wave * 16 + qq) * KOUT + l) * D + t] = T[qq * LDC + t];
                }
                __syncthreads();
            }
        }
    } else {
        const int d = E.d, k = E.k, q = E.q;
        const int64_t m = E.m;
        const double *__restrict__ lam = E.lam;
        double *__restrict__ vals = E.vals;
        double *__restrict__ jac = E.jac;
        if (vals) {
            __syncthreads();
            double *Lm = Cs;
            for (int e = tid; e < (KOUT + 1) * D; e += 256) {
                const int l = e / D, t = e % D;
                Lm[e] = (t < d && q > 1) ? (l < KOUT ? (l0 + l < k ? lam[(int64_t)(t + 1) * k + l0 + l] : 0.0) : E.mean[t]) : 0.0;
            }
            __syncthreads();
#pragma unroll
            for (int l = 0; l < KOUT; ++l) {
                double acc = 0.0, cst = 0.0;
#pragma unroll
                for (int s = 0; s < D / 4; ++s) acc = fma(Lm[l * D + 4 * s + l4], xb[s], acc);
                for (int t = lane; t < D; t += 64) cst = fma(Lm[l * D + t], Lm[KOUT * D + t], cst);
                for (int off = 32; off > 0; off >>= 1) cst += __shfl_xor(cst, off);
                acc += __shfl_xor(acc, 16);
                acc += __shfl_xor(acc, 32);
                double v = vsum[l];
                if (q > 0 && l0 + l < k) v += lam[l0 + l];
                if (q > 1) v += acc + cst;
                if (l4 == 0 && qrow < m && l0 + l < k) vals[qrow * k + l0 + l] = v;
            }
        }
        if (JAC && jac) {
            __syncthreads();
            double *T = Cs + wave * 16 * LDC;
            double *SA = Ws;
#pragma unroll
            for (int l = 0; l < KOUT; ++l)
                if (l4 == 0) SA[l * EQ + wave * 16 + l15] = sasum[l];
#pragma unroll
            for (int l = 0; l < KOUT; ++l) {
#pragma unroll
                for (int tt = 0; tt < DT; ++tt)
#pragma unroll
                    for (int r = 0; r < 4; ++r) T[l15 * LDC + 16 * tt + l4 + 4 * r] = JT[l][tt][r];
                __syncthreads();
                if (l0 + l < k) {
                    for (int e = lane; e < 16 * D; e += 64) {
                        const int qq = e / D, t = e % D;
                        const int64_t row = q0 + wave * 16 + qq;
                        if (row < m && t < d) {
                            double v = fma(SA[l * EQ + wave * 16 + qq], Xq[row * D + t], -T[qq * LDC + t]);
                            if (q > 1) v += lam[(int64_t)(t + 1) * k + l0 + l];
                            jac[row * (int64_t)k * d + (int64_t)t * k + l0 + l] = v;
                        }
                    }
                }
                __syncthreads();
            }
        }
    }
}

template <int KID, bool FAST, int KOUT, int H, int ECT, bool JAC, bool FINAL>
__global__ __launch_bounds__(512, 2) void eval_fused_split_kernel(EvalDesc one, const EvalDesc *__restrict__ many, int l0) {
    constexpr int D = 2 * H, LDC = D + 2, LDT = 65, NCT = ECT / 16, HT = H / 16;
    static_assert(8 * 16 * LDT <= ECT * LDC + 2 * 8 * 256, "epilogue transpose area");
    __shared__ __attribute__((aligned(16))) double smem[ECT * LDC + 2 * 8 * 256];
    double *Cs = smem;
    double *Sx = smem + ECT * LDC;
    __shared__ double Ws[KOUT * ECT];
    __shared__ double Sq[ECT];
    const EvalDesc &E = many ? many[blockIdx.z] : one;
    if (many && ((int64_t)blockIdx.x * EQ >= E.mpad || (int)blockIdx.y >= E.nsplit)) return;
    const double *__restrict__ Xq = E.Xq;
    const double *__restrict__ Cc = E.Cc;
    const double *__restrict__ csq = E.csq;
    const double *__restrict__ Wc = E.Wc;
    const int64_t npad = E.npad, mpad = E.mpad;
    const KP kp = E.kp;
    const int tid = threadIdx.x, lane = tid & 63, wave = tid >> 6, grp = wave >> 2, qw = wave & 3;
    const int l15 = lane & 15, l4 = lane >> 4;
    const int64_t q0 = (int64_t)blockIdx.x * EQ;
    const int split = blockIdx.y;
    const int64_t qrow = q0 + qw * 16 + l15;
    double xb[H / 4];
#pragma unroll
    for (int s = 0; s < H / 4; ++s) xb[s] = Xq[qrow * D + H * grp + 4 * s + l4];
    const double xs = E.xsq[qrow];
    v4d JT[KOUT][HT];
    double vsum[KOUT], sasum[KOUT];
#pragma unroll
    for (int l = 0; l < KOUT; ++l) {
        vsum[l] = 0.0;
        sasum[l] = 0.0;
#pragma unroll
        for (int t = 0; t < HT; ++t) JT[l][t] = (v4d){0.0, 0.0, 0.0, 0.0};
    }
    const int64_t c_begin = (int64_t)split * E.tiles_per_split * EC;
    const int ntiles_all = E.ntiles;
    const int nsub = __builtin_amdgcn_readfirstlane(E.nsub);
    const int my_tiles = min(E.tiles_per_split, ntiles_all - split * E.tiles_per_split) * (EC / ECT);
    constexpr int NLD = ECT * D / 2 / 512;
    v2d stg[NLD];
    auto load_tile = [&](int64_t c0) {
        const v2d *src = reinterpret_cast<const v2d *>(Cc + c0 * D);
#pragma unroll
        for (int u = 0; u < NLD; ++u) stg[u] = src[tid + 512 * u];
    };
    auto store_tile = [&]() {
#pragma unroll
        for (int u = 0; u < NLD; ++u) {
            const int e = (tid + 512 * u) * 2;
            const int row = e / D, col = e % D;
            *(v2d *)&Cs[row * LDC + col] = stg[u];
        }
    };
    static_assert((KOUT + 1) * ECT <= 512, "one staged scalar per thread");
    double stg_w = 0.0;
    auto load_scalars = [&](int64_t c0) {
        if (tid < ECT)
            stg_w = csq[c0 + tid];
        else if (tid < (KOUT + 1) * ECT)
            stg_w = Wc[(int64_t)(l0 + (tid - ECT) / ECT) * npad + c0 + ((tid - ECT) % ECT)];
    };
    load_tile(c_begin);
    load_scalars(c_begin);
    for (int tile = 0; tile < my_tiles; ++tile) {
        const int64_t c0 = c_begin + (int64_t)tile * ECT;
        __syncthreads();
        store_tile();
        if (tid < ECT)
            Sq[tid] = stg_w;
        else if (tid < (KOUT + 1) * ECT)
            Ws[tid - ECT] = stg_w;
        __syncthreads();
        if (tile + 1 < my_tiles) {
            load_tile(c0 + ECT);
            load_scalars(c0 + ECT);
        }
#pragma unroll
        for (int ct = 0; ct < NCT; ++ct) {
            if ((int)(c0 >> 4) + ct >= nsub) break;
// ... 198 lines not shown
    const int64_t qrow = q0 + wave * 16 + l15;
    const bool qin = qrow < mpad;
    const int64_t qld = qin ? qrow : mpad - 1;
    double xb[D / 4];
#pragma unroll
    for (int s = 0; s < D / 4; ++s) xb[s] = Xq[qld * D + 4 * s + l4];
    const double xs = E.xsq[qld];
    double vsum[KOUT];
#pragma unroll
    for (int l = 0; l < KOUT; ++l) vsum[l] = 0.0;
    const int64_t c_begin = (int64_t)split * E.tiles_per_split * EC;
    const int nsub = __builtin_amdgcn_readfirstlane(E.nsub);
    const int my_tiles = min(E.tiles_per_split, E.ntiles - split * E.tiles_per_split) * (EC / ECT);
    constexpr int NLD = ECT * D / 2 / 512;
    v2d stg[NLD];
    auto load_tile = [&](int64_t c0) {
        const v2d *src = reinterpret_cast<const v2d *>(Cc + c0 * D);
#pragma unroll
        for (int u = 0; u < NLD; ++u) stg[u] = src[tid + 512 * u];
    };
    static_assert((KOUT + 1) * ECT <= 512, "one staged scalar per thread");
    double stg_w = 0.0;
    auto load_scalars = [&](int64_t c0) {
        if (tid < ECT)
            stg_w = csq[c0 + tid];
        else if (tid < (KOUT + 1) * ECT)
            stg_w = Wc[(int64_t)(l0 + (tid - ECT) / ECT) * npad + c0 + ((tid - ECT) % ECT)];
    };
    load_tile(c_begin);
    load_scalars(c_begin);
    for (int tile = 0; tile < my_tiles; ++tile) {
        const int64_t c0 = c_begin + (int64_t)tile * ECT;
        __syncthreads();
#pragma unroll
        for (int u = 0; u < NLD; ++u) {
            const int e = (tid + 512 * u) * 2;
            *(v2d *)&Cs[(e / D) * LDC + (e % D)] = stg[u];
        }
        if (tid < ECT)
            Sq[tid] = stg_w;
        else if (tid < (KOUT + 1) * ECT)
            Ws[tid - ECT] = stg_w;
        __syncthreads();
        if (tile + 1 < my_tiles) {
            load_tile(c0 + ECT);
            load_scalars(c0 + ECT);
        }
#pragma unroll
        for (int ct = 0; ct < NCT; ++ct) {
            if ((int)(c0 >> 4) + ct >= nsub) break;
            v4d S0 = {0.0, 0.0, 0.0, 0.0}, S1 = {0.0, 0.0, 0.0, 0.0};
            const double *crow = &Cs[(16 * ct + l15) * LDC + l4];
#pragma unroll
            for (int s = 0; s < H / 4; ++s) {
                S0 = __builtin_amdgcn_mfma_f64_16x16x4f64(crow[4 * s], xb[s], S0, 0, 0, 0);
                S1 = __builtin_amdgcn_mfma_f64_16x16x4f64(crow[H + 4 * s], xb[H / 4 + s], S1, 0, 0, 0);
            }
#pragma unroll
            for (int r = 0; r < 4; ++r) {
                const int c = 16 * ct + l4 + 4 * r;
                double s2 = fma(-2.0, S0[r] + S1[r], xs + Sq[c]);
                s2 = s2 > 0.0 ? s2 : 0.0;
                double phi, psi;
                rbf_phi_psi_t<KID, FAST>(s2, kp, phi, psi);
#pragma unroll
                for (int l = 0; l < KOUT; ++l) vsum[l] = fma(Ws[l * ECT + c], phi, vsum[l]);
            }
        }
    }
#pragma unroll
    for (int l = 0; l < KOUT; ++l) {
        vsum[l] += __shfl_xor(vsum[l], 16);
        vsum[l] += __shfl_xor(vsum[l], 32);
    }
    if (l4 == 0 && qin) {
#pragma unroll
        for (int l = 0; l < KOUT; ++l) {
            E.vpart[((int64_t)split * mpad + qrow) * KOUT + l] = vsum[l];
            E.sapart[((int64_t)split * mpad + qrow) * KOUT + l] = 0.0;
        }
    }
}

template <int KOUT>
__global__ __launch_bounds__(128) void eval_combine_kernel(EvalDesc one, const EvalDesc *__restrict__ many, int l0, int D) {
    const EvalDesc &E = many ? many[blockIdx.y] : one;
    const int64_t p = blockIdx.x, m = E.m, mpad = E.mpad;
    if (p >= m) return;
    const double *__restrict__ vpart = E.vpart, *__restrict__ sapart = E.sapart, *__restrict__ gpart = E.gpart;
    const double *__restrict__ Xq = E.Xq, *__restrict__ Xorig = E.X, *__restrict__ lam = E.lam;
    double *__restrict__ vals = E.vals, *__restrict__ jac = E.jac;
    const int nsplit = E.nsplit, d = E.d, k = E.k, q = E.q;
    __shared__ double sa[KOUT], sv[KOUT];
    __shared__ double pdot[KOUT][128];
    const int tid = threadIdx.x;
    if (tid < KOUT && l0 + tid < k) {
        double v = 0.0, a = 0.0;
        for (int s0 = 0; s0 < nsplit; s0 += 8) {
            double xv[8], xa[8];
#pragma unroll
            for (int u = 0; u < 8; ++u) {
                xv[u] = s0 + u < nsplit ? vpart[((int64_t)(s0 + u) * mpad + p) * KOUT + tid] : 0.0;
                xa[u] = s0 + u < nsplit ? sapart[((int64_t)(s0 + u) * mpad + p) * KOUT + tid] : 0.0;
            }
#pragma unroll
            for (int u = 0; u < 8; ++u)
                if (s0 + u < nsplit) {
                    v += xv[u];
                    a += xa[u];
                }
        }
        sa[tid] = a;
        sv[tid] = v;
    }
    if (vals && q > 1) {
#pragma unroll
        for (int l = 0; l < KOUT; ++l) {
            double acc = 0.0;
            if (l0 + l < k)
                for (int t = tid; t < d; t += 128) acc = fma(lam[(int64_t)(t + 1) * k + l0 + l], Xorig[p * d + t], acc);
            pdot[l][tid] = acc;
        }
    }
    __syncthreads();
    if (vals && tid < KOUT && l0 + tid < k) {
        double v = sv[tid];
        if (q > 0) v += lam[l0 + tid];
        if (q > 1) {
            const int nt = d < 128 ? d : 128;
            double dsum = 0.0;
            for (int t = 0; t < nt; ++t) dsum += pdot[tid][t];
            v += dsum;
        }
        vals[p * k + l0 + tid] = v;
    }
    for (int e = tid; e < KOUT * d; e += blockDim.x) {
        const int l = e / d, t = e % d;
        if (l0 + l >= k) continue;
        double g = 0.0;
        for (int s0 = 0; s0 < nsplit; s0 += 8) {
            double x[8];
#pragma unroll
            for (int u = 0; u < 8; ++u) x[u] = s0 + u < nsplit ? gpart[(((int64_t)(s0 + u) * mpad + p) * KOUT + l) * D + t] : 0.0;
#pragma unroll
            for (int u = 0; u < 8; ++u)
                if (s0 + u < nsplit) g += x[u];
        }
        double v = fma(sa[l], Xq[p * D + t], -g);
        if (q > 1) v += lam[(int64_t)(t + 1) * k + l0 + l];
        jac[p * (int64_t)k * d + (int64_t)t * k + l0 + l] = v;
    }
}

template <int KOUT>
__global__ __launch_bounds__(256) void eval_combine_vals_kernel(EvalDesc one, const EvalDesc *__restrict__ many, int l0) {
    const EvalDesc &E = many ? many[blockIdx.y] : one;
    const int lane = threadIdx.x & 63, wave = threadIdx.x >> 6;
    const int64_t p = (int64_t)blockIdx.x * 4 + wave, m = E.m, mpad = E.mpad;
    const bool active = p < m;
    const double *__restrict__ vpart = E.vpart, *__restrict__ Xorig = E.X, *__restrict__ lam = E.lam;
    const int nsplit = E.nsplit, d = E.d, k = E.k, q = E.q;
    __shared__ double pdot[4][KOUT][128];
    double v = 0.0;
    if (active && lane < KOUT && l0 + lane < k) {
        for (int s0 = 0; s0 < nsplit; s0 += 8) {
            double x[8];
#pragma unroll
            for (int u = 0; u < 8; ++u) x[u] = s0 + u < nsplit ? vpart[((int64_t)(s0 + u) * mpad + p) * KOUT + lane] : 0.0;
#pragma unroll
            for (int u = 0; u < 8; ++u)
                if (s0 + u < nsplit) v += x[u];
        }
    }
    if (q > 1) {
#pragma unroll
        for (int l = 0; l < KOUT; ++l)
#pragma unroll
            for (int h = 0; h < 2; ++h) {
                const int t0 = lane + 64 * h;
                double acc = 0.0;
                if (active && l0 + l < k)
                    for (int t = t0; t < d; t += 128) acc = fma(lam[(int64_t)(t + 1) * k + l0 + l], Xorig[p * d + t], acc);
                pdot[wave][l][t0] = acc;
            }
    }
    __syncthreads();
    if (active && lane < KOUT && l0 + lane < k) {
        if (q > 0) v += lam[l0 + lane];
        if (q > 1) {
            const int nt = d < 128 ? d : 128;
            double dsum = 0.0;
            for (int t = 0; t < nt; ++t) dsum += pdot[wave][lane][t];
            v += dsum;
        }
        if (E.vals) E.vals[p * k + l0 + lane] = v;
    }
}

__global__ void center_pad_batch_kernel(const EvalDesc *__restrict__ many, int Dfixed) {
    const EvalDesc &E = many[blockIdx.y];
    const int D = Dfixed > 0 ? Dfixed : (E.d <= 64 ? 64 : 128);
    const int lane = threadIdx.x & 63;
    const int64_t row = (int64_t)blockIdx.x * (blockDim.x >> 6) + (threadIdx.x >> 6);
    if (row >= E.mpad) return;
    double s = 0.0;
    for (int t = lane; t < D; t += 64) {
        double v = 0.0;
        if (row < E.m && t < E.d) v = E.X[row * E.d + t] - E.mean[t];
        E.Xq[row * D + t] = v;
        s = fma(v, v, s);
    }
    for (int off = 32; off > 0; off >>= 1) s += __shfl_xor(s, off);
    if (lane == 0) E.xsq[row] = s;
}

int eval_nsplit(const mrbf_ctx *ctx, int64_t m, int ntiles, bool check_call, bool population) {
    const int64_t mpad = round_up(m, EQ);
    const int slots = 2 * ctx->ncu;
    const int64_t qtiles = mpad / EQ;
    constexpr int small_split = 8;
    const bool small_batch = !check_call && qtiles * 8 <= slots;
    if (ntiles >= 4 && ntiles <= 8 && small_batch) return std::min(small_split, ntiles);
    if (population && !check_call && ntiles >= 4 && ntiles <= 8 && qtiles * 2 <= slots) return (int)std::min<int64_t>(ntiles, slots / qtiles);
    if (ntiles <= 8) return 1;
    constexpr double comb_small = 0.1, comb = 0.75;
    int nsplit = 1;
    double best_cost = 1e300;
    for (int s = 1; s <= std::min(ntiles, 32); ++s) {
        const int tps_s = (ntiles + s - 1) / s;
        if ((int64_t)(s - 1) * tps_s >= ntiles) continue;
        const double rounds = std::ceil((double)(qtiles * s) / slots);
        const double cost = rounds * tps_s + (small_batch ? comb_small : comb) * s;
        if (cost < best_cost) {
            best_cost = cost;
            nsplit = s;
        }
    }
    const int force_split = mrbf_env("MRBF_EVAL_NSPLIT") ? atoi(mrbf_env("MRBF_EVAL_NSPLIT")) : 0;
    if (force_split > 0 && force_split <= ntiles && (int64_t)(force_split - 1) * ((ntiles + force_split - 1) / force_split) < ntiles)
        nsplit = force_split;
    return nsplit;
}

int outputs_per_pass(int k, int D, bool want_jac) { return (k < 2 || (D == 256 && want_jac)) ? 1 : 2; }

template <int KID, bool FAST, int KOUT, bool JAC, bool FINAL>
static int launch_pass(mrbf_ctx *ctx, int D, dim3 grid, dim3 cgrid, const EvalDesc &one, const EvalDesc *many, int l0) {
    hipStream_t st = ctx->stream;
    if (D == 64) {
        hipLaunchKernelGGL((eval_fused_kernel<KID, FAST, KOUT, JAC, FINAL>), grid, dim3(256), 0, st, one, many, l0);
    } else if (D == 128) {
        hipLaunchKernelGGL((eval_fused_split_kernel<KID, FAST, KOUT, 64, 64, JAC, FINAL>), grid, dim3(512), 0, st, one, many, l0);
    } else if constexpr (JAC && KOUT == 1) {
        hipLaunchKernelGGL((eval_fused_split_kernel<KID, FAST, 1, 128, 32, true, FINAL>), grid, dim3(512), 0, st, one, many, l0);
    } else if constexpr (JAC) {
        return fail(ctx, MRBF_EHIP, "eval_fused: a pass with Jacobians at D = 256 carries one output");
    } else if constexpr (FINAL) {
        hipLaunchKernelGGL((eval_fused_split_kernel<KID, FAST, KOUT, 128, 32, false, true>), grid, dim3(512), 0, st, one, many, l0);
    } else {
        hipLaunchKernelGGL((eval_vals256_kernel<KID, FAST, KOUT>), dim3((grid.x + 1) / 2, grid.y, grid.z), dim3(512), 0, st, one, many, l0);
    }
    if constexpr (!FINAL && JAC)
        hipLaunchKernelGGL(eval_combine_kernel<KOUT>, cgrid, dim3(128), 0, st, one, many, l0, D);
    else if constexpr (!FINAL)
        hipLaunchKernelGGL(eval_combine_vals_kernel<KOUT>, dim3((cgrid.x + 3) / 4, cgrid.y), dim3(256), 0, st, one, many, l0);
    return 0;
}

template <class F>
static int with_bool(bool b, F &&f) {
    return b ? f(std::true_type{}) : f(std::false_type{});
}

static int run_passes(mrbf_ctx *ctx, const KP &kp, int D, int k, bool want_jac, bool final_, dim3 grid, dim3 cgrid, const EvalDesc &one,
                      const EvalDesc *many) {
    const int KO = outputs_per_pass(k, D, want_jac);
    for (int l0 = 0; l0 < k; l0 += KO) {
        const bool two = std::min(KO, k - l0) == 2;
        MRBF_DISPATCH_KID(kp.kid, {
            constexpr bool HAS_FAST = KID == MRBF_MULTIQUADRIC || KID == MRBF_INV_MULTIQUADRIC || KID == MRBF_CUBIC;
            MRBF_TRY(with_bool(HAS_FAST && kp.fast, [&](auto fast) {
                return with_bool(two, [&](auto two_) {
                    return with_bool(want_jac, [&](auto jac) {
                        return with_bool(final_, [&](auto fin) {
                            return launch_pass<KID, HAS_FAST && decltype(fast)::value, decltype(two_)::value ? 2 : 1, decltype(jac)::value, decltype(fin)::value>(
                                ctx, D, grid, cgrid, one, many, l0);
                        });
                    });
                });
            }));
        });
    }
    MRBF_HIP(ctx, hipGetLastError());
    return 0;
}

int center_pad_batch(mrbf_ctx *ctx, const EvalDesc *dev_descs, int count, int64_t max_mpad) {
    if (count <= 0 || max_mpad <= 0) return 0;
    hipLaunchKernelGGL(center_pad_batch_kernel, dim3((unsigned)((max_mpad + 3) / 4), (unsigned)count), dim3(256), 0, ctx->stream, dev_descs, 0);
    MRBF_HIP(ctx, hipGetLastError());
    return 0;
}

int eval_fused_batch(mrbf_ctx *ctx, const KP &kp, int D, int k, bool want_jac, const EvalDesc *host_descs, const EvalDesc *dev_descs, int count,
                     bool centred) {
    if (count <= 0) return 0;
    if (D != 64 && D != 128 && D != 256) return fail(ctx, MRBF_EHIP, "eval_fused_batch needs dpad in {64, 128, 256}");
    int64_t max_mpad = 0, max_m = 0;
    int max_split = 1;
    for (int p = 0; p < count; ++p) {
        max_mpad = std::max(max_mpad, host_descs[p].mpad);
        max_m = std::max(max_m, host_descs[p].m);
        max_split = std::max(max_split, host_descs[p].nsplit);
    }
    if (max_split > 1)
        for (int p = 0; p < count; ++p)
            if (host_descs[p].nsplit == 1 && host_descs[p].m > 0)
                return fail(ctx, MRBF_EHIP, "eval_fused_batch: descriptor %d is unsplit in a group that splits the centre range", p);
    if (!centred)
        hipLaunchKernelGGL(center_pad_batch_kernel, dim3((unsigned)((max_mpad + 3) / 4), (unsigned)count), dim3(256), 0, ctx->stream, dev_descs, D);
    dim3 grid((unsigned)(max_mpad / EQ), (unsigned)max_split, (unsigned)count);
    dim3 cgrid((unsigned)max_m, (unsigned)count);
    return run_passes(ctx, kp, D, k, want_jac, max_split == 1, grid, cgrid, host_descs[0], dev_descs);
}

int eval_fused(mrbf_ctx *ctx, const mrbf_model *M, int64_t m, const double *X, double *vals, double *jac, mrbf_eval_info *info, EvalHints hints) {
    const int d = M->d, k = M->k;
    const int D = (M->dpad <= 64) ? 64 : (M->dpad <= 128 ? 128 : 256);
    if (M->dpad > 256) return fail(ctx, MRBF_EHIP, "eval_fused supports d <= 256");
    if (D != M->dpad) return fail(ctx, MRBF_EHIP, "eval_fused needs dpad in {64, 128, 256} (got %d)", M->dpad);
    const int64_t mpad = round_up(m, EQ);
    const int ntiles = (int)((M->n + EC - 1) / EC);
    const int nsplit = eval_nsplit(ctx, m, ntiles, hints.check_call, hints.population);
    const int KO = outputs_per_pass(k, D, jac != nullptr);
    EvalDesc E;
    std::memset(&E, 0, sizeof(E));
    eval_desc_model(E, M, m, nsplit);
    E.X = X;
    MRBF_TRY(get_buf(ctx, S_EVAL_XC, (size_t)mpad * D, &E.Xq));
    MRBF_TRY(get_buf(ctx, S_EVAL_XSQ, (size_t)mpad, &E.xsq));
    if (nsplit > 1) {
        MRBF_TRY(get_buf(ctx, S_EVAL_SA, (size_t)nsplit * mpad * KO * 2, &E.vpart));
        E.sapart = E.vpart + (size_t)nsplit * mpad * KO;
        if (jac) MRBF_TRY(get_buf(ctx, S_EVAL_J, (size_t)nsplit * mpad * KO * D, &E.gpart));
    }
    E.vals = vals;
    E.jac = jac;
    const bool timing = ctx->timing && info;
    if (timing) MRBF_HIP(ctx, hipEventRecord(ctx->ev[4], ctx->stream));
    if (!(hints.pre_xq && hints.pre_xq == E.Xq)) MRBF_TRY(launch_center_pad(ctx, X, m, d, M->mean, nullptr, E.Xq, mpad, D, E.xsq));
    dim3 grid((unsigned)(mpad / EQ), (unsigned)nsplit);
    MRBF_TRY(run_passes(ctx, M->kp, D, k, jac != nullptr, nsplit == 1, grid, dim3((unsigned)m), E, nullptr));
    if (timing) {
        MRBF_HIP(ctx, hipEventRecord(ctx->ev[7], ctx->stream));
        MRBF_HIP(ctx, hipEventSynchronize(ctx->ev[7]));
        float t;
        MRBF_HIP(ctx, hipEventElapsedTime(&t, ctx->ev[4], ctx->ev[7]));
        info->ms_total = t;
        info->ms_kernel = t;
    }
    return 0;
}

}
```

### morbit.jl_amd/csrc/normal_batch.hip

```cpp
#include "batch_chain.hpp"
#include "normal.hpp"

using namespace mrbf;
using chain::batch_fetch;

namespace {

static_assert(sizeof(mrbf_normal_batch_record) == 32, "mrbf_normal_batch_record is 32 bytes");

struct FinishArgs {
    int d, variable_radius;
    double kappa_delta, delta_max;
    const double *x, *delta, *alpha;
    const int *status, *iters;
    double *n, *xn;
    mrbf_normal_batch_record *rec;
};

__global__ __launch_bounds__(ns::THREADS) void normal_finish_kernel(FinishArgs a) {
    const int64_t p = blockIdx.x;
    const int t = threadIdx.x, d = a.d;
    const int status = a.status[p];
    const double alpha = a.alpha[p];
    bool ok = status == MRBF_NS_OK;
// ... 51 lines not shown
        if (!models[j]) return fail(ctx, -4, "mrbf_normal_step_batch: model %d of start 0 is NULL", j);
        kj[j] = models[j]->k;
    }
    std::vector<ns::RowSrc> meq_rows, min_rows;
    std::vector<int64_t> joff(nm, 0), voff(nm, 0);
    std::vector<char> used(nm, 0);
    int64_t jtot = 0, vtot = 0;
    for (int j = 0, e = 0; j < nm; ++j)
        for (int c = 0; c < kj[j]; ++c, ++e) {
            const int role = shape->roles[e];
            if (role == MRBF_ROLE_EQ || role == MRBF_ROLE_INEQ) {
                if (!used[j]) {
                    used[j] = 1, joff[j] = jtot, voff[j] = vtot;
                    jtot += (int64_t)kj[j] * d, vtot += kj[j];
                }
                ns::RowSrc s{2, 0, role == MRBF_ROLE_EQ, kj[j], joff[j] + c, voff[j] + c};
                (role == MRBF_ROLE_EQ ? meq_rows : min_rows).push_back(s);
            } else if (role < 0 && role != MRBF_ROLE_NONE) {
                return fail(ctx, -3, "mrbf_normal_step_batch: roles[%d] = %d is not a role", e, role);
            }
        }
    const int n_nl = (int)(meq_rows.size() + min_rows.size()), n_lin = shape->n_lin_eq + shape->n_lin_ineq;
    if (mrbf_dispatch_normal_batch(N, d, nm, n_nl, n_lin, 0) != MRBF_DISPATCH_DEVICE)
        return fail(ctx, -2, "mrbf_normal_step_batch: %lld starts / d = %d / %d rows outside the device path (ask mrbf_dispatch_normal_batch first)",
                    (long long)N, d, n_nl + n_lin);
    for (int64_t p = 0; p < N; ++p)
        for (int j = 0; j < nm; ++j) {
            const mrbf_model *M = models[p * nm + j];
            if (!M) return fail(ctx, -4, "mrbf_normal_step_batch: model %d of start %lld is NULL", j, (long long)p);
            if (M->d != d || M->k != kj[j])
                return fail(ctx, -4, "mrbf_normal_step_batch: model %d of start %lld is %d variables x %d outputs, expected %d x %d", j, (long long)p,
                            M->d, M->k, d, kj[j]);
            if (used[j] && M->n == 0) return fail(ctx, -4, "mrbf_normal_step_batch: model %d of start %lld has no centres", j, (long long)p);
        }
    const int meq = shape->n_lin_eq + (int)meq_rows.size(), min = shape->n_lin_ineq + (int)min_rows.size(), m = meq + min;
    (void)hipSetDevice(ctx->device);
    PinGuard pin(ctx);
    chain::Plan ev;
    for (int64_t p = 0; p < N; ++p)
        for (int j = 0; j < nm; ++j)
            if (used[j]) ev.add(ctx, 0, p, j, models[p * nm + j], 1, true);
    ev.close();
    size_t total = 0;
    auto take = [&](size_t cnt) {
        const size_t at = total;
        total += (cnt + 15) & ~(size_t)15;
        return at;
    };
    const size_t nlin = (size_t)n_lin, SN = (size_t)N;
    const size_t oX = take(SN * d), oDelta = take(SN), oLb = take(d), oUb = take(d), oA = take(nlin * d), oB = take(nlin);
    const size_t oDesc = take(ev.desc_doubles());
    const size_t up_cnt = total;
    const size_t oJ = take(SN * jtot), oV = take(SN * vtot);
    const size_t oAeq = take(SN * meq * d), oBeq = take(SN * meq), oAin = take(SN * min * d), oBin = take(SN * min);
    const size_t oAlpha = take(SN), oInts = take((3 * SN + 1) / 2);
    ev.carve(take);
    for (chain::Member &mb : ev.mem) {
        const size_t p = (size_t)mb.p;
        mb.X = oX + p * d, mb.vals = oV + p * vtot + voff[mb.j], mb.jacs = oJ + p * jtot + joff[mb.j];
    }
    const size_t out0 = total;
    const size_t oN = take(SN * d), oXn = take(SN * d), oDual = take(SN * m);
    const size_t oRec = take(SN * sizeof(mrbf_normal_batch_record) / sizeof(double));
    const size_t out_cnt = total - out0;
    double *base;
    MRBF_TRY(get_buf(ctx, S_NS_BATCH, total, &base));
    std::vector<double> hup_v;
    double *hup = reinterpret_cast<double *>(up_cnt * sizeof(double) <= ((size_t)4 << 20) ? pin_take(ctx, up_cnt * sizeof(double)) : nullptr);
    if (!hup) {
        hup_v.resize(up_cnt);
        hup = hup_v.data();
    }
    std::memset(hup, 0, up_cnt * sizeof(double));
    MRBF_TRY(batch_fetch(ctx, x, SN * d, hup + oX));
    MRBF_TRY(batch_fetch(ctx, delta, SN, hup + oDelta));
    MRBF_TRY(batch_fetch(ctx, lb, d, hup + oLb));
    MRBF_TRY(batch_fetch(ctx, ub, d, hup + oUb));
    MRBF_TRY(batch_fetch(ctx, shape->A_eq, (size_t)shape->n_lin_eq * d, hup + oA));
    MRBF_TRY(batch_fetch(ctx, shape->A_ineq, (size_t)shape->n_lin_ineq * d, hup + oA + (size_t)shape->n_lin_eq * d));
    MRBF_TRY(batch_fetch(ctx, shape->b_eq, shape->n_lin_eq, hup + oB));
    MRBF_TRY(batch_fetch(ctx, shape->b_ineq, shape->n_lin_ineq, hup + oB + shape->n_lin_eq));
    EvalDesc *hdesc = reinterpret_cast<EvalDesc *>(hup + oDesc);
    const EvalDesc *ddesc = reinterpret_cast<const EvalDesc *>(base + oDesc);
    ev.fill(base, hdesc);
    hipStream_t st = ctx->stream;
    hipEvent_t e0 = ctx->ev[0], e1 = ctx->ev[1];
    MRBF_HIP(ctx, hipEventRecord(e0, st));
    MRBF_HIP(ctx, hipMemcpyAsync(base, hup, up_cnt * sizeof(double), hipMemcpyHostToDevice, st));
    MRBF_TRY(ev.launch(ctx, 0, base, hdesc, ddesc));
    ns::AsmArgs aa;
    aa.n = d, aa.rows = m, aa.meq = meq, aa.min = min;
    aa.sJ = jtot, aa.sV = vtot, aa.sx = d;
    aa.J = base + oJ, aa.V = base + oV, aa.x = base + oX, aa.Alin = base + oA, aa.blin = base + oB;
    aa.Aeq = base + oAeq, aa.beq = base + oBeq, aa.Ain = base + oAin, aa.bin = base + oBin;
    {
        int r = 0;
        for (int i = 0; i < shape->n_lin_eq; ++i) aa.src[r++] = ns::RowSrc{1, i, 1, 1, 0, i};
        for (size_t i = 0; i < meq_rows.size(); ++i) aa.src[r] = meq_rows[i], aa.src[r++].dst = shape->n_lin_eq + (int)i;
        for (int i = 0; i < shape->n_lin_ineq; ++i) aa.src[r++] = ns::RowSrc{1, i, 0, 1, 0, shape->n_lin_eq + i};
        for (size_t i = 0; i < min_rows.size(); ++i) aa.src[r] = min_rows[i], aa.src[r++].dst = shape->n_lin_ineq + (int)i;
    }
    MRBF_TRY(ns::launch_assemble(ctx, aa, N));
    int *dInts = reinterpret_cast<int *>(base + oInts);
    MRBF_TRY(ns::launch(ctx, N, d, meq, min, base + oX, base + oLb, base + oUb, 0, meq ? base + oAeq : nullptr, meq ? base + oBeq : nullptr,
                        min ? base + oAin : nullptr, min ? base + oBin : nullptr, base + oN, base + oAlpha, dual_out ? base + oDual : nullptr,
                        dInts, dInts + N));
    FinishArgs fa;
    fa.d = d, fa.variable_radius = variable_radius != 0;
    fa.kappa_delta = kappa_delta, fa.delta_max = delta_max;
    fa.x = base + oX, fa.delta = base + oDelta, fa.alpha = base + oAlpha;
    fa.status = dInts, fa.iters = dInts + N;
    fa.n = base + oN, fa.xn = base + oXn;
    fa.rec = reinterpret_cast<mrbf_normal_batch_record *>(base + oRec);
    hipLaunchKernelGGL(normal_finish_kernel, dim3((unsigned)N), dim3(ns::THREADS), 0, st, fa);
    MRBF_HIP(ctx, hipGetLastError());
    std::vector<double> hout_v;
    double *hout = reinterpret_cast<double *>(out_cnt * sizeof(double) <= ((size_t)4 << 20) ? pin_take(ctx, out_cnt * sizeof(double)) : nullptr);
    if (!hout) {
        hout_v.resize(out_cnt);
        hout = hout_v.data();
    }
    MRBF_HIP(ctx, hipMemcpyAsync(hout, base + out0, out_cnt * sizeof(double), hipMemcpyDeviceToHost, st));
    const bool dev_n = is_device_ptr(n_out), dev_x = x_n_out && is_device_ptr(x_n_out), dev_y = dual_out && is_device_ptr(dual_out);
    if (dev_n) MRBF_HIP(ctx, hipMemcpyAsync(n_out, base + oN, SN * d * sizeof(double), hipMemcpyDeviceToDevice, st));
    if (dev_x) MRBF_HIP(ctx, hipMemcpyAsync(x_n_out, base + oXn, SN * d * sizeof(double), hipMemcpyDeviceToDevice, st));
    if (dev_y) MRBF_HIP(ctx, hipMemcpyAsync(dual_out, base + oDual, SN * m * sizeof(double), hipMemcpyDeviceToDevice, st));
    MRBF_HIP(ctx, hipEventRecord(e1, st));
    MRBF_HIP(ctx, hipStreamSynchronize(st));
    pin.flush();
    if (ms_total) MRBF_HIP(ctx, hipEventElapsedTime(ms_total, e0, e1));
    if (!dev_n) std::memcpy(n_out, hout + (oN - out0), SN * d * sizeof(double));
    if (x_n_out && !dev_x) std::memcpy(x_n_out, hout + (oXn - out0), SN * d * sizeof(double));
    if (dual_out && !dev_y) std::memcpy(dual_out, hout + (oDual - out0), SN * m * sizeof(double));
    std::memcpy(records, hout + (oRec - out0), SN * sizeof(mrbf_normal_batch_record));
    return MRBF_OK;
}
```

### morbit.jl_amd/csrc/sd_batch.hip

```cpp
#include <limits>

#include "batch_chain.hpp"
#include "sd.hpp"

using namespace mrbf;
using chain::batch_fetch;

namespace {
enum Site { SITE_PAIR = 0, SITE_X = 1, SITE_TRIAL = 2 };
}

extern "C" int32_t mrbf_sd_iterate_batch(mrbf_ctx *ctx, int64_t n_starts, const mrbf_ps_problem *shape, const mrbf_model *const *models,
                                         const double *x, const double *x_n, const double *delta, const double *lb, const double *ub,
                                         int32_t normalize, const mrbf_sd_step_options *opts, double *d_out, double *x_plus, double *mx_plus,
                                         mrbf_sd_batch_record *records, float *ms_total) {
    using sdstep::RowRef;
    if (!ctx) return -1;
    if (ms_total) *ms_total = 0.f;
    if (!shape) return fail(ctx, -3, "shape is NULL");
    if (!models) return fail(ctx, -4, "models is NULL");
    if (!x) return fail(ctx, -5, "x is NULL");
    if (!x_n) return fail(ctx, -6, "x_n is NULL");
    if (!delta) return fail(ctx, -7, "delta is NULL");
    if (!lb) return fail(ctx, -8, "lb is NULL");
// ... 62 lines not shown
                    (long long)N, d, k, n_nl + n_lin, L);
    for (int64_t p = 0; p < N; ++p)
        for (int j = 0; j < nm; ++j) {
            const mrbf_model *M = models[p * nm + j];
            if (!M) return fail(ctx, -4, "mrbf_sd_iterate_batch: model %d of start %lld is NULL", j, (long long)p);
            if (M->d != d || M->k != kj[j])
                return fail(ctx, -4, "mrbf_sd_iterate_batch: model %d of start %lld is %d variables x %d outputs, start 0 has %d x %d", j, (long long)p,
                            M->d, M->k, d, kj[j]);
            if (M->n == 0) return fail(ctx, -4, "mrbf_sd_iterate_batch: model %d of start %lld has no centres", j, (long long)p);
        }
    const int meq = shape->n_lin_eq + (int)meq_src.size(), min = shape->n_lin_ineq + (int)min_src.size(), m = k + meq + min;
    for (int j = 0; j < nm; ++j)
        if (has_obj[j]) ooff[j] = otot, otot += (int64_t)(L + 2) * kj[j];
    (void)hipSetDevice(ctx->device);
    PinGuard pin(ctx);
    chain::Plan ev;
    auto site_m = [&](int site) -> int64_t { return site == SITE_PAIR ? 2 : (site == SITE_X ? 1 : L + 2); };
    for (int site = 0; site < 3; ++site)
        for (int64_t p = 0; p < N; ++p)
            for (int j = 0; j < nm; ++j) {
                if (!(site == SITE_PAIR ? used[j] : (site == SITE_X ? has_con[j] : has_obj[j]))) continue;
                ev.add(ctx, site, p, j, models[p * nm + j], site_m(site), site != SITE_TRIAL);
            }
    ev.close();
    size_t total = 0;
    auto take = [&](size_t cnt) {
        const size_t at = total;
        total += (cnt + 15) & ~(size_t)15;
        return at;
    };
    const size_t nlin = (size_t)n_lin, SN = (size_t)N;
    std::vector<RowRef> rows;
    for (int i = 0; i < shape->n_lin_eq; ++i) rows.push_back(RowRef{(int64_t)i * d, i, 1, 0});
    rows.insert(rows.end(), meq_ref.begin(), meq_ref.end());
    for (int i = 0; i < shape->n_lin_ineq; ++i) rows.push_back(RowRef{(int64_t)(shape->n_lin_eq + i) * d, shape->n_lin_eq + i, 1, 0});
    rows.insert(rows.end(), min_ref.begin(), min_ref.end());
    const size_t rows_dbl = (rows.size() * sizeof(RowRef) + sizeof(double) - 1) / sizeof(double);
    const size_t desc_dbl = ev.desc_doubles();
    const size_t oPairs = take(SN * 2 * d), oDelta = take(SN), oLb = take(d), oUb = take(d), oA = take(nlin * d), oB = take(nlin);
    const size_t oRows = take(rows_dbl), oDesc = take(desc_dbl);
    const size_t up_cnt = total;
    const size_t oJA = take(SN * jtotA), oVA = take(SN * vtotA), oJB = take(SN * jtotB), oVB = take(SN * vtotB);
    const size_t oG = take(SN * k * d), oAeq = take(SN * meq * d), oBeq = take(SN * meq), oAin = take(SN * min * d), oBin = take(SN * min);
    const size_t oSteps = take(SN * (L + 1)), oSig = take(SN * 2), oX = take(SN * (L + 2) * d), oVO = take(SN * otot);
    ev.carve(take);
    for (chain::Member &mb : ev.mem) {
        const size_t p = (size_t)mb.p;
        const int j = mb.j;
        if (mb.site == SITE_PAIR) mb.X = oPairs + p * 2 * d, mb.vals = oVA + p * vtotA + voffA[j], mb.jacs = oJA + p * jtotA + joffA[j];
        else if (mb.site == SITE_X) mb.X = oPairs + p * 2 * d + d, mb.vals = oVB + p * vtotB + voffB[j], mb.jacs = oJB + p * jtotB + joffB[j];
        else mb.X = oX + p * (size_t)(L + 2) * d, mb.vals = oVO + p * otot + ooff[j];
    }
    const size_t out0 = total;
    const size_t oXp = take(SN * d), oMxp = take(SN * k), oTail = take(SN * sdstep::ARMIJO_TAIL), oDir = take(SN * d), oOmega = take(SN);
    const size_t oInts = take((3 * SN + 1) / 2);
    const size_t out_cnt = total - out0;
    double *base;
    MRBF_TRY(get_buf(ctx, S_SD_BATCH, total, &base));
    std::vector<double> hup_v;
    double *hup = reinterpret_cast<double *>(up_cnt * sizeof(double) <= ((size_t)4 << 20) ? pin_take(ctx, up_cnt * sizeof(double)) : nullptr);
    if (!hup) {
        hup_v.resize(up_cnt);
        hup = hup_v.data();
    }
    std::memset(hup, 0, up_cnt * sizeof(double));
    {
        std::vector<double> tmp(SN * d);
        MRBF_TRY(batch_fetch(ctx, x_n, SN * d, tmp.data()));
        for (size_t p = 0; p < SN; ++p) std::memcpy(hup + oPairs + p * 2 * d, tmp.data() + p * d, (size_t)d * sizeof(double));
        MRBF_TRY(batch_fetch(ctx, x, SN * d, tmp.data()));
        for (size_t p = 0; p < SN; ++p) std::memcpy(hup + oPairs + p * 2 * d + d, tmp.data() + p * d, (size_t)d * sizeof(double));
    }
    MRBF_TRY(batch_fetch(ctx, delta, SN, hup + oDelta));
    MRBF_TRY(batch_fetch(ctx, lb, d, hup + oLb));
    MRBF_TRY(batch_fetch(ctx, ub, d, hup + oUb));
    MRBF_TRY(batch_fetch(ctx, shape->A_eq, (size_t)shape->n_lin_eq * d, hup + oA));
    MRBF_TRY(batch_fetch(ctx, shape->A_ineq, (size_t)shape->n_lin_ineq * d, hup + oA + (size_t)shape->n_lin_eq * d));
    MRBF_TRY(batch_fetch(ctx, shape->b_eq, shape->n_lin_eq, hup + oB));
    MRBF_TRY(batch_fetch(ctx, shape->b_ineq, shape->n_lin_ineq, hup + oB + shape->n_lin_eq));
    if (!rows.empty()) std::memcpy(hup + oRows, rows.data(), rows.size() * sizeof(RowRef));
    double *dPairs = base + oPairs, *dX = base + oX;
    EvalDesc *hdesc = reinterpret_cast<EvalDesc *>(hup + oDesc);
    const EvalDesc *ddesc = reinterpret_cast<const EvalDesc *>(base + oDesc);
    ev.fill(base, hdesc);
    hipStream_t st = ctx->stream;
    hipEvent_t e0 = ctx->ev[0], e1 = ctx->ev[1];
    MRBF_HIP(ctx, hipEventRecord(e0, st));
    MRBF_HIP(ctx, hipMemcpyAsync(base, hup, up_cnt * sizeof(double), hipMemcpyHostToDevice, st));
    auto evaluate = [&](int site) -> int { return ev.launch(ctx, site, base, hdesc, ddesc); };
    MRBF_TRY(evaluate(SITE_PAIR));
    MRBF_TRY(evaluate(SITE_X));
    sd::AsmArgs aa;
    aa.n = d, aa.k = k, aa.rows = m, aa.meq = meq, aa.min = min;
    aa.sJ = jtotA, aa.sV = vtotA, aa.sx = 2 * (int64_t)d;
    aa.J = base + oJA, aa.V = base + oVA, aa.xn = dPairs, aa.x = dPairs + d, aa.Alin = base + oA, aa.blin = base + oB;
    aa.G = base + oG, aa.Aeq = base + oAeq, aa.beq = base + oBeq, aa.Ain = base + oAin, aa.bin = base + oBin;
    {
        int r = 0;
        for (int l = 0; l < k; ++l) aa.src[r++] = obj[l];
        for (int i = 0; i < shape->n_lin_eq; ++i) aa.src[r++] = sd::RowSrc{1, i, 1, 1, 0, i};
        for (size_t i = 0; i < meq_src.size(); ++i) {
            aa.src[r] = meq_src[i];
            aa.src[r++].dst = shape->n_lin_eq + (int)i;
        }
        for (int i = 0; i < shape->n_lin_ineq; ++i) aa.src[r++] = sd::RowSrc{1, i, 0, 1, 0, shape->n_lin_eq + i};
        for (size_t i = 0; i < min_src.size(); ++i) {
            aa.src[r] = min_src[i];
            aa.src[r++].dst = shape->n_lin_ineq + (int)i;
        }
    }
    MRBF_TRY(sd::launch_assemble(ctx, aa, N));
    double *dDir = base + oDir, *dOmega = base + oOmega;
    int *dInts = reinterpret_cast<int *>(base + oInts);
    MRBF_TRY(sd::launch(ctx, N, d, k, meq, min, normalize, base + oG, dPairs, 2 * (int64_t)d, base + oLb, base + oUb, 0,
                        meq ? base + oAeq : nullptr, meq ? base + oBeq : nullptr, min ? base + oAin : nullptr, min ? base + oBin : nullptr, dDir,
                        dOmega, nullptr, dInts, dInts + N));
    sdstep::StepArgs sa;
    sa.d = d, sa.n_eq = meq, sa.n_in = min, sa.max_loops = L;
    sa.shrink = opts->shrink;
    sa.sx = 2 * (int64_t)d, sa.sdir = d, sa.sJ = jtotB, sa.sV = vtotB;
    sa.delta = base + oDelta;
    sa.xn = dPairs, sa.x = dPairs + d, sa.lb = base + oLb, sa.ub = base + oUb, sa.dir = dDir;
    sa.Alin = base + oA, sa.blin = base + oB, sa.Jc = base + oJB, sa.Vc = base + oVB;
    sa.rows = reinterpret_cast<const RowRef *>(base + oRows);
    sa.steps = base + oSteps, sa.out = base + oSig;
    MRBF_TRY(sdstep::launch_stepsize(ctx, sa, N));
    MRBF_TRY(sdstep::launch_trial(ctx, dPairs, 2 * (int64_t)d, dDir, d, base + oSteps, d, L, N, dX));
    MRBF_TRY(evaluate(SITE_TRIAL));
    sdstep::ArmijoArgs am;
    am.d = d, am.k = k, am.max_loops = L, am.strict = opts->strict != 0;
    am.const_rhs = opts->const_rhs;
    am.min_stepsize_raw = opts->min_stepsize;
    am.min_step = opts->min_stepsize >= 0.0 ? opts->min_stepsize : std::numeric_limits<double>::epsilon();
    am.sV = otot, am.sdir = d;
    am.omega = dOmega;
    am.V = base + oVO, am.X = dX, am.dir = dDir, am.steps = base + oSteps, am.stepout = base + oSig;
    am.xplus = base + oXp, am.mxplus = base + oMxp, am.tail = base + oTail;
    for (int l = 0; l < k; ++l) {
        const int j = obj_model[l];
        am.obj[l] = sdstep::ObjSrc{ooff[j] + obj_col[l], kj[j]};
    }
    MRBF_TRY(sdstep::launch_armijo(ctx, am, N));
    std::vector<double> hout_v;
    double *hout = reinterpret_cast<double *>(out_cnt * sizeof(double) <= ((size_t)4 << 20) ? pin_take(ctx, out_cnt * sizeof(double)) : nullptr);
    if (!hout) {
        hout_v.resize(out_cnt);
        hout = hout_v.data();
    }
    MRBF_HIP(ctx, hipMemcpyAsync(hout, base + out0, out_cnt * sizeof(double), hipMemcpyDeviceToHost, st));
    const bool dev_d = is_device_ptr(d_out), dev_x = is_device_ptr(x_plus), dev_m = is_device_ptr(mx_plus);
    if (dev_d) MRBF_HIP(ctx, hipMemcpyAsync(d_out, dDir, SN * d * sizeof(double), hipMemcpyDeviceToDevice, st));
    if (dev_x) MRBF_HIP(ctx, hipMemcpyAsync(x_plus, base + oXp, SN * d * sizeof(double), hipMemcpyDeviceToDevice, st));
    if (dev_m) MRBF_HIP(ctx, hipMemcpyAsync(mx_plus, base + oMxp, SN * k * sizeof(double), hipMemcpyDeviceToDevice, st));
    MRBF_HIP(ctx, hipEventRecord(e1, st));
    MRBF_HIP(ctx, hipStreamSynchronize(st));
    pin.flush();
    if (ms_total) MRBF_HIP(ctx, hipEventElapsedTime(ms_total, e0, e1));
    const double *hXp = hout + (oXp - out0), *hMxp = hout + (oMxp - out0), *hTail = hout + (oTail - out0), *hDir = hout + (oDir - out0);
    const double *hOmega = hout + (oOmega - out0);
    const int *hInts = reinterpret_cast<const int *>(hout + (oInts - out0));
    if (!dev_d) std::memcpy(d_out, hDir, SN * d * sizeof(double));
    if (!dev_x) std::memcpy(x_plus, hXp, SN * d * sizeof(double));
    if (!dev_m) std::memcpy(mx_plus, hMxp, SN * k * sizeof(double));
    std::vector<double> nanrow;
    for (size_t p = 0; p < SN; ++p) {
        mrbf_sd_batch_record &R = records[p];
        const double *t = hTail + p * sdstep::ARMIJO_TAIL;
// ... 20 lines not shown
```

### morbit.jl_amd/csrc/small.hpp

```cpp
#pragma once
#include "common.hpp"

namespace mrbf {
namespace smallfit {

struct Prob {
    int n, d, k, q, deg;
    int n16, npad, dpad, q16;
    KP kp;
    const double *C, *Y;
    double *Xc, *sq, *mean, *W, *Wc, *lam;
    double *ws;
    int *flags;
    double *scal;
    long long *stamps;
    int *cl;
    int mean_given;
    unsigned long long spin_ticks;
    int fault;
    int diag6;
};

constexpr int CL_WORDS = 24;
constexpr int MAX_CLUSTER = 16;

struct Carve {
    size_t Phi, Q1, Wm, V, G, Gx, LinvX, Linv, Pt, Ycol, B, Fy, Xs, T1, T2, Z, total;
    int ldz;
};
__host__ __device__ inline Carve carve(int npad, int q16) {
    Carve c;
    size_t o = 0;
    auto take = [&](size_t cnt) {
        const size_t at = o;
        o += (cnt + 15) & ~size_t(15);
        return at;
    };
    c.ldz = q16 + 16;
    c.Phi = take((size_t)npad * npad);
    c.Q1 = take((size_t)npad * q16);
    c.Wm = take((size_t)npad * q16);
    c.V = take((size_t)npad * q16);
    c.G = take((size_t)q16 * q16);
    c.Gx = take((size_t)128 * 128);
    c.LinvX = take((size_t)128 * 128);
    c.Linv = take((size_t)npad * 128);
    c.Pt = take((size_t)npad * 128);
    c.Ycol = take((size_t)npad * 16);
    c.B = take((size_t)npad * 16);
    c.Fy = take((size_t)npad * 16);
    c.Xs = take((size_t)npad * 16);
    c.T1 = take((size_t)c.ldz * 16);
    c.T2 = take((size_t)c.ldz * 16);
    c.Z = take((size_t)c.ldz * 16 + 16);
    c.total = o;
    return c;
}

}

struct EvalDesc {
    const double *X;
    const double *mean;
    double *Xq, *xsq;
    const double *Cc, *csq, *Wc, *lam;
    int64_t npad, mpad, m;
    int d, k, q, tiles_per_split, nsplit;
    int ntiles;
    int nsub;
    KP kp;
    double *vpart, *sapart, *gpart;
    double *vals, *jac;
};
inline void eval_desc_model(EvalDesc &E, const mrbf_model *M, int64_t m, int nsplit) {
    E.mean = M->mean;
    E.Cc = M->Xc;
    E.csq = M->sq;
    E.Wc = M->Wc;
    E.lam = M->lam;
    E.npad = M->npad;
    E.d = M->d;
    E.k = M->k;
    E.q = M->q;
    E.kp = M->kp;
    E.m = m;
    E.mpad = round_up(m, 64);
    E.nsplit = nsplit;
    E.ntiles = (int)((M->n + 63) / 64);
    E.nsub = (int)((M->n + 15) / 16);
    E.tiles_per_split = (E.ntiles + nsplit - 1) / nsplit;
}
int eval_nsplit(const mrbf_ctx *ctx, int64_t m, int ntiles, bool check_call = false, bool population = false);
int outputs_per_pass(int k, int D, bool want_jac = true);
int eval_fused_batch(mrbf_ctx *ctx, const KP &kp, int D, int k, bool want_jac, const EvalDesc *host_descs, const EvalDesc *dev_descs, int count,
                     bool centred = false);
int center_pad_batch(mrbf_ctx *ctx, const EvalDesc *dev_descs, int count, int64_t max_mpad);

bool small_fit_applies(const mrbf_ctx *ctx, int64_t n, int d, int k, int q, int path);
int launch_small_fit(mrbf_ctx *ctx, const smallfit::Prob *host_probs, int count, const smallfit::Prob *dev_probs, int nc);
int small_fit_cluster(const mrbf_ctx *ctx, int count);
int launch_small_means(mrbf_ctx *ctx, const smallfit::Prob *dev_probs, int count);

bool tail_basis_applies(const mrbf_model *M);
size_t tail_basis_scratch_doubles();
int launch_tail_basis(mrbf_ctx *ctx, const mrbf_model *M, const double *Y, double *scratch, double *LinvX, double *T1, double *Q1, double *B,
                      double *rows_out, int64_t ld, int xt, int *flags);

}
```

### morbit.jl_amd/csrc/solve.hip

```cpp
#include "common.hpp"
#include "small.hpp"

namespace mrbf {

__global__ void fit_publish_kernel(const int *__restrict__ dinfo, const double *__restrict__ scal, const unsigned long long *__restrict__ dstat,
                                   int *__restrict__ hflags, double *__restrict__ hscal, unsigned long long *__restrict__ hstat) {
    const int t = threadIdx.x;
    if (t < 4) hflags[t] = dinfo[t];
    if (t >= 4 && t < 6 && scal) hscal[t - 4] = scal[t - 4];
    if (t == 6 && dstat && hstat) hstat[0] = dstat[0];
}

__global__ void fill_saddle_kernel(const double *__restrict__ Pi, int64_t n, int q, double *__restrict__ S, int64_t N) {
    const int64_t idx = (int64_t)blockIdx.x * blockDim.x + threadIdx.x;
    const int64_t tot = n * q;
    if (idx < tot) {
        const int64_t i = idx % n;
        const int t = (int)(idx / n);
        const double v = Pi[idx];
        S[i + (n + t) * N] = v;
        S[(n + t) + i * N] = v;
    } else if (idx < tot + (int64_t)q * q) {
        const int64_t r = idx - tot;
        S[(n + r % q) + (n + r / q) * N] = 0.0;
// ... 582 lines not shown
    double *Q1 = nullptr, *Wm = nullptr, *G = nullptr, *T1 = nullptr, *scal = nullptr, *Tall = nullptr, *LxInv = nullptr;
    int64_t lt = 0, dq = 0;
    info->mu = 0.0;
    hipStream_t main_stream = ctx->stream;
    const bool side = q > 0 && ctx->panel_stream && ctx->panel_stream != main_stream && n >= 2048;
    const bool fused = q > 0 && gram_w_applies(ctx, M) && (q == 1 || round_up(d, 128) == 128);
    if (q > 0) {
        MRBF_TRY(get_buf(ctx, S_Q1, (size_t)npad * q, &Q1));
        MRBF_TRY(get_buf(ctx, S_W1, (size_t)npad * q, &Wm));
        MRBF_TRY(get_buf(ctx, S_G, (size_t)q * q, &G));
        MRBF_TRY(get_buf(ctx, S_T1, (size_t)q * k, &T1));
        MRBF_TRY(get_buf(ctx, S_MISC, (size_t)8, &scal));
        if (side) {
            MRBF_HIP(ctx, hipEventRecord(ctx->evx[0], main_stream));
            MRBF_HIP(ctx, hipStreamWaitEvent(ctx->panel_stream, ctx->evx[0], 0));
            ctx->stream = ctx->panel_stream;
        }
        struct RestoreStream {
            mrbf_ctx *c;
            hipStream_t s;
            ~RestoreStream() { c->stream = s; }
        } restore{ctx, main_stream};
        if (tailq) {
            double *scratch;
            MRBF_TRY(get_buf(ctx, S_PI, tail_basis_scratch_doubles(), &scratch));
            MRBF_TRY(get_buf(ctx, S_QR_INV, (size_t)128 * 128, &LxInv));
            MRBF_TRY(launch_tail_basis(ctx, M, Y, scratch, LxInv, T1, Q1, B, builtin ? Phi : nullptr, ld, xt, dinfo));
        } else if (q > 1) {
            dq = round_up(d, 128);
            lt = dq + npad;
            MRBF_TRY(get_buf(ctx, S_PI, (size_t)lt * dq, &Tall));
            MRBF_HIP(ctx, hipMemsetAsync(Tall, 0, (size_t)lt * dq * sizeof(double), ctx->stream));
            hipLaunchKernelGGL(xc_to_tall_kernel, dim3(nblk(n * d)), dim3(256), 0, ctx->stream, M->Xc, n, d, M->dpad, Tall, lt, dq);
            MRBF_TRY(tsmm_tn(ctx, n, d, d, 1.0, Tall + dq, lt, Tall + dq, lt, 0.0, Tall, lt));
            MRBF_TRY(launch_pad_identity(ctx, Tall, d, dq, lt));
            if (dq == 128) MRBF_TRY(get_buf(ctx, S_QR_INV, (size_t)128 * 128, &LxInv));
            MRBF_TRY(potrf_blocked_tall(ctx, dq, lt, Tall, lt, dinfo + 1, LxInv, popt));
        }
        if (!tailq) hipLaunchKernelGGL(build_q1_kernel, dim3(nblk(npad * q)), dim3(256), 0, ctx->stream, Tall, lt, dq, n, npad, q, Q1);
        if (!fused) MRBF_HIP(ctx, hipMemsetAsync(Wm, 0, (size_t)npad * q * sizeof(double), ctx->stream));
        if (!tailq) {
            MRBF_TRY(tsmm_tn(ctx, n, q, k, 1.0, Q1, npad, B, npad, 0.0, T1, q));
            hipLaunchKernelGGL(sub_qt_kernel, dim3((unsigned)((n + 63) / 64)), dim3(256), 0, ctx->stream, B, npad, Q1, npad, T1, n, q, k);
            if (builtin) hipLaunchKernelGGL(set_rhs_rows_kernel, dim3(nblk(npad * xt)), dim3(256), 0, ctx->stream, Phi, ld, npad, xt, B, k);
        }
        if (side) MRBF_HIP(ctx, hipEventRecord(ctx->evx[1], ctx->stream));
    }
    ctx->stream = main_stream;
    MRBF_HIP(ctx, hipEventRecord(ctx->ev[0], ctx->stream));
    double *Wpart = nullptr, *rspart = nullptr;
    int nseg = 0;
    if (fused)
        MRBF_TRY(launch_gram_w(ctx, M, Phi, ld, &Wpart, &rspart, &nseg));
    else
        MRBF_TRY(launch_gram(ctx, ctx->gram_mode, M->C, M->Xc, M->sq, n, M->npad, M->d, M->dpad, M->kp, Phi, ld));
    MRBF_HIP(ctx, hipEventRecord(ctx->ev[1], ctx->stream));
    if (side) MRBF_HIP(ctx, hipStreamWaitEvent(ctx->stream, ctx->evx[1], 0));
    if (fused) {
        const int skip = (q > 1 && round_up(2 * (q - 1), 16) < round_up(2 * q, 16)) ? 1 : 0;
        const int K2 = (int)round_up(2 * (q - skip), 16);
        double *PA, *PB, *v0 = nullptr;
        MRBF_TRY(get_buf(ctx, S_STAGE_C, (size_t)npad * K2, &PA));
        MRBF_TRY(get_buf(ctx, S_STAGE_D, (size_t)npad * K2, &PB));
        if (skip) MRBF_TRY(get_buf(ctx, S_V0, (size_t)npad, &v0));
        MRBF_TRY(launch_projection_small(ctx, M, Wpart, rspart, nseg, LxInv, Q1, Wm, G, scal, dinfo, K2, skip, PA, PB, v0));
        MRBF_TRY(launch_update_lower(ctx, PA, npad, PB, npad, Phi, ld, npad / 128, K2, v0, 1.0 / std::sqrt((double)n), n));
    } else if (q > 0) {
        MRBF_TRY(symm_panel(ctx, n, npad, q, Phi, ld, Q1, npad, Wm, npad, true, 1.0 / std::sqrt((double)n)));
        MRBF_TRY(tsmm_tn(ctx, n, q, q, 1.0, Q1, npad, Wm, npad, 0.0, G, q));
        hipLaunchKernelGGL(trace_kernel, dim3(1), dim3(256), 0, ctx->stream, G, q, scal);
        MRBF_BLAS(ctx, rocblas_dgemm(ctx->blas, rocblas_operation_none, rocblas_operation_none, (int)n, q, q, &mhalf, Q1, (int)npad,
                                     G, q, &one, Wm, (int)npad));
        hipLaunchKernelGGL(shift_from_trace_kernel, dim3(1), dim3(1), 0, ctx->stream, scal, (double)n * M->kp.phi0,
                           (double)std::max<int64_t>(n - q, 1), dinfo);
        const int skip = (q > 1 && round_up(2 * (q - 1), 16) < round_up(2 * q, 16)) ? 1 : 0;
        const int K2 = (int)round_up(2 * (q - skip), 16);
        double *PA, *PB, *v0 = nullptr;
        MRBF_TRY(get_buf(ctx, S_STAGE_C, (size_t)npad * K2, &PA));
        MRBF_TRY(get_buf(ctx, S_STAGE_D, (size_t)npad * K2, &PB));
        if (skip) MRBF_TRY(get_buf(ctx, S_V0, (size_t)npad, &v0));
        hipLaunchKernelGGL(build_panels_kernel, dim3(nblk(npad * K2)), dim3(256), 0, ctx->stream, Q1, Wm, scal, n, npad, q, K2, skip, PA, PB, v0);
        MRBF_TRY(launch_update_lower(ctx, PA, npad, PB, npad, Phi, ld, npad / 128, K2, v0, 1.0 / std::sqrt((double)n), n));
    }
    MRBF_HIP(ctx, hipEventRecord(ctx->ev[2], ctx->stream));
    int hinfo = 0;
    double *linv_all = nullptr;
    if (builtin) {
        MRBF_TRY(get_buf(ctx, S_CHOL_WS, (size_t)npad * 128, &linv_all));
        MRBF_TRY(launch_pad_identity(ctx, Phi, n, npad, ld));
        if (q == 0) hipLaunchKernelGGL(set_rhs_rows_kernel, dim3(nblk(npad * xt)), dim3(256), 0, ctx->stream, Phi, ld, npad, xt, B, k);
        popt.xreal = k;
        popt.info_clean = true;
        MRBF_TRY(potrf_blocked_tall(ctx, npad, npad + xt, Phi, ld, dinfo, linv_all, popt));
        MRBF_HIP(ctx, hipEventRecord(ctx->ev[3], ctx->stream));
    } else {
        int *dpot;
        MRBF_TRY(get_buf(ctx, S_IPIV, (size_t)4, &dpot));
        MRBF_BLAS(ctx, rocsolver_dpotrf(ctx->blas, rocblas_fill_lower, (int)n, Phi, (int)ld, dpot));
        MRBF_HIP(ctx, hipMemcpyAsync(dinfo, dpot, sizeof(int), hipMemcpyDeviceToDevice, ctx->stream));
        MRBF_HIP(ctx, hipEventRecord(ctx->ev[3], ctx->stream));
    }
    double *T1w = nullptr;
    if (q > 0) MRBF_TRY(get_buf(ctx, S_T1W, (size_t)q * k, &T1w));
    auto solve_tail = [&](bool persistent) -> int {
        if (builtin) {
            hipLaunchKernelGGL(get_rhs_rows_kernel, dim3(nblk(npad * k)), dim3(256), 0, ctx->stream, Phi, ld, npad, B, k);
            if (persistent)
                MRBF_TRY(backsolve_persistent(ctx, npad, Phi, ld, linv_all, B, npad, k, dinfo + 3));
            else
                MRBF_TRY(backsolve_blocked(ctx, npad, Phi, ld, linv_all, B, npad, k));
        } else {
            MRBF_BLAS(ctx, rocsolver_dpotrs(ctx->blas, rocblas_fill_lower, (int)n, k, Phi, (int)ld, B, (int)npad));
        }
        static const int tail3 = mrbf_env("MRBF_TAIL3") ? atoi(mrbf_env("MRBF_TAIL3")) : 1;
        if (tail3 && q > 0 && q <= 129 && k <= 16 && (q == 1 || LxInv)) {
            const int nch = (int)(npad / 64);
            double *T2, *part;
            MRBF_TRY(get_buf(ctx, S_T2, (size_t)q * k, &T2));
            MRBF_TRY(get_buf(ctx, S_TAIL_PART, (size_t)nch * 2 * k * q, &part));
            hipLaunchKernelGGL(tail_dots_kernel, dim3((unsigned)nch), dim3(256), 0, ctx->stream, B, npad, Q1, Wm, npad, n, q, k, part);
            hipLaunchKernelGGL(tail_coeff_kernel, dim3(1), dim3(1024), 0, ctx->stream, part, nch, q, k, q > 1 ? d : 0, T1, G, fused ? 1.0 : 0.5, LxInv,
                               std::sqrt((double)n), M->mean, T2, T1w);
            hipLaunchKernelGGL(tail_apply_kernel, dim3((unsigned)nch), dim3(256), 0, ctx->stream, B, npad, Q1, npad, T2, T1w, n, M->npad, q, k, M->W,
                               M->Wc, M->lam);
            MRBF_HIP(ctx, hipGetLastError());
            return 0;
        }
        if (q > 0) {
            double *T2;
            MRBF_TRY(get_buf(ctx, S_T2, (size_t)q * k, &T2));
            MRBF_HIP(ctx, hipMemcpyAsync(T1w, T1, (size_t)q * k * sizeof(double), hipMemcpyDeviceToDevice, ctx->stream));
            MRBF_TRY(tsmm_tn(ctx, n, q, k, 1.0, Q1, npad, B, npad, 0.0, T2, q));
            hipLaunchKernelGGL(sub_qt_kernel, dim3((unsigned)((n + 63) / 64)), dim3(256), 0, ctx->stream, B, npad, Q1, npad, T2, n, q, k);
            MRBF_TRY(tsmm_tn(ctx, n, q, k, -1.0, Wm, npad, B, npad, 1.0, T1w, q));
            if (q > 1) {
                if (LxInv)
                    hipLaunchKernelGGL(apply_linv_t_kernel, dim3(1), dim3(256), 0, ctx->stream, LxInv, d, T1w + 1, (int64_t)q, k);
                else if (d <= 256)
                    hipLaunchKernelGGL(trsm_lt_small_kernel, dim3(1), dim3(256), 0, ctx->stream, Tall, lt, d, T1w + 1, (int64_t)q, k);
                else
                    MRBF_BLAS(ctx, rocblas_dtrsm(ctx->blas, rocblas_side_left, rocblas_fill_lower, rocblas_operation_transpose,
                                                 rocblas_diagonal_non_unit, d, k, &one, Tall, (int)lt, T1w + 1, q));
            }
            hipLaunchKernelGGL(finish_lambda_kernel, dim3((unsigned)k), dim3(64), 0, ctx->stream, T1w, q, k, std::sqrt((double)n), M->mean);
        }
        hipLaunchKernelGGL(scatter_solution_kernel, dim3(nblk(M->npad * k + (int64_t)q * k)), dim3(256), 0, ctx->stream, B, npad, n,
                           M->npad, k, q, (int64_t)0, M->W, M->Wc, M->lam, T1w ? T1w : B, (int64_t)q);
        MRBF_HIP(ctx, hipGetLastError());
        return 0;
    };
    MRBF_TRY(solve_tail(true));
    MRBF_HIP(ctx, hipEventRecord(ctx->ev[4], ctx->stream));
    {
        int hflags_local[4] = {0, 0, 0, 0};
        double hscal_local[2] = {0.0, 0.0};
        int *hflags = ctx->hpin ? reinterpret_cast<int *>(ctx->hpin + HPIN_FIT_FLAGS) : hflags_local;
        double *hscal = ctx->hpin ? reinterpret_cast<double *>(ctx->hpin + HPIN_FIT_SCAL) : hscal_local;
        hscal[0] = hscal[1] = 0.0;
        static const int publish = mrbf_env("MRBF_FIT_PUBLISH") ? atoi(mrbf_env("MRBF_FIT_PUBLISH")) : 1;
        if (ctx->hpin && publish) {
            unsigned long long *hstat = nullptr;
            const unsigned long long *dstat = nullptr;
            if (ctx->mega_stat_pending && ctx->mega_stat_dev) {
                ctx->hpin[HPIN_MEGA_STAT] = ~0ull;
                hstat = &ctx->hpin[HPIN_MEGA_STAT];
                dstat = ctx->mega_stat_dev;
// ... 275 lines not shown
```

Measured before the change: 175.7.

## Balance eval work into flat pieces and split tail update tiles into halves

The fused eval kernel now divides the flattened (query tile × centre tile) unit space into roughly 2×CU pieces, so each block handles a contiguous range instead of a fixed split. Partial-sum buffers are resized to match, and the reduction goes through a row mapping. Separately, the lower-triangular Cholesky update splits the leftover tiles of the last wave into two 64-row halves to cut tail imbalance. Both aim to improve CU occupancy and load balance, at the cost of extra indexing logic and more partial rows to reduce. A debug capture hook for the K matrix is also added.

```diff
diff --git a/include/mrbf.h b/include/mrbf.h
--- a/include/mrbf.h
+++ b/include/mrbf.h
@@ -194,6 +194,7 @@
 int32_t mrbf_fit_batch(mrbf_ctx *ctx, int64_t n_starts, mrbf_fit_job *jobs, float *ms_total);
 
 int32_t mrbf_debug_env(const char *name);
+int32_t mrbf_debug_capture_k(mrbf_ctx *ctx, double *out, int64_t capacity_doubles);
 int32_t mrbf_debug_mfma_layout(mrbf_ctx *ctx, double *out16x16_a_times_b, const double *A16x4, const double *B4x16);
 int32_t mrbf_debug_potrf(mrbf_ctx *ctx, int64_t n, double *A_colmajor_inout, int32_t impl, int32_t *info, float *ms);
 int32_t mrbf_debug_diag(mrbf_ctx *ctx, const double *A128, int32_t reps, float *ms_per_call, double *shader_cycles,
@@ -207,6 +208,7 @@
 int32_t mrbf_debug_mega_tables2(int32_t nt, int32_t mt, int32_t slack, int32_t slack_chain, int32_t first, int32_t win, int32_t srows,
                                 int32_t half_cols, const int32_t *opt5, int64_t *out6);
 int32_t mrbf_debug_mega_plan(int32_t nt, int32_t mt, int32_t xreal, int64_t *out39);
+int32_t mrbf_debug_eval_pieces(int64_t qtiles, int32_t ntiles, int32_t slots, int32_t cap, int32_t *out4);
 
 enum { MRBF_PS_OK = 0, MRBF_PS_CRITICAL = 1, MRBF_PS_FAILURE = 2 };
 typedef struct {
diff --git a/morbit.jl_amd/_lib.py b/morbit.jl_amd/_lib.py
--- a/morbit.jl_amd/_lib.py
+++ b/morbit.jl_amd/_lib.py
@@ -196,6 +196,7 @@
     "mrbf_debug_mfma_layout": (ctypes.c_int32, [c_vp, c_vp, c_vp, c_vp]),
     "mrbf_debug_potrf": (ctypes.c_int32, [c_vp, ctypes.c_int64, c_vp, ctypes.c_int32, c_ip, c_fp]),
     "mrbf_debug_env": (ctypes.c_int32, [ctypes.c_char_p]),
+    "mrbf_debug_capture_k": (ctypes.c_int32, [c_vp, c_vp, ctypes.c_int64]),
     "mrbf_debug_diag": (ctypes.c_int32, [c_vp, c_vp, ctypes.c_int32, c_fp, c_dp, c_dp]),
     "mrbf_debug_ps_rank": (ctypes.c_int32, [c_vp, ctypes.c_int32, c_vp, c_vp, ctypes.c_uint64, ctypes.c_int32, ctypes.c_int32, c_ip, c_ip]),
     "mrbf_debug_mfma_peak": (ctypes.c_int32, [c_vp, ctypes.c_int32, ctypes.c_int32, ctypes.c_int32, c_fp, c_dp]),
@@ -204,6 +205,7 @@
     "mrbf_debug_mega_tables": (ctypes.c_int32, [ctypes.c_int32] * 8 + [c_vp]),
     "mrbf_debug_mega_tables2": (ctypes.c_int32, [ctypes.c_int32] * 8 + [c_vp, c_vp]),
     "mrbf_debug_mega_plan": (ctypes.c_int32, [ctypes.c_int32] * 3 + [c_vp]),
+    "mrbf_debug_eval_pieces": (ctypes.c_int32, [ctypes.c_int64, ctypes.c_int32, ctypes.c_int32, ctypes.c_int32, c_vp]),
     "mrbf_stochastic_rank": (ctypes.c_int32, [ctypes.c_int32, c_vp, c_vp, c_vp, ctypes.c_double, c_vp]),
     "mrbf_ps_step": (ctypes.c_int32, [c_vp, c_vp, c_vp, c_vp, c_vp, c_vp, c_vp, ctypes.POINTER(PsOptions), c_vp, c_vp, c_vp,
                                       ctypes.POINTER(PsInfo)]),
diff --git a/morbit.jl_amd/csrc/api.hip b/morbit.jl_amd/csrc/api.hip
--- a/morbit.jl_amd/csrc/api.hip
+++ b/morbit.jl_amd/csrc/api.hip
@@ -403,6 +403,13 @@
     return MRBF_OK;
 }
 
+extern "C" int32_t mrbf_debug_capture_k(mrbf_ctx *ctx, double *out, int64_t capacity_doubles) {
+    if (!ctx) return -1;
+    ctx->debug_k_out = (out && capacity_doubles > 0) ? out : nullptr;
+    ctx->debug_k_cap = ctx->debug_k_out ? (size_t)capacity_doubles : 0;
+    return MRBF_OK;
+}
+
 extern "C" int32_t mrbf_debug_env(const char *name) {
     if (!name) return -1;
     return mrbf::mrbf_env(name) ? 1 : 0;
diff --git a/morbit.jl_amd/csrc/batch.hip b/morbit.jl_amd/csrc/batch.hip
--- a/morbit.jl_amd/csrc/batch.hip
+++ b/morbit.jl_amd/csrc/batch.hip
@@ -141,6 +141,7 @@
     struct Lay {
         size_t C, Y, X, Xc, sq, mean, W, Wc, lam, ws, Xq0, xsq0, vp0, gp0, V0, Xq1, xsq1, vp1, gp1, vals, jac, out;
         int nsplit0, nsplit1, D, q, KO;
+        size_t prows0, prows1;
         int64_t npad, mpad0, mpad1;
         bool w_host, lam_host;
     };
@@ -182,15 +183,17 @@
         L.nsplit0 = check ? eval_nsplit(ctx, pr.n, (int)((pr.n + 63) / 64), true) : 1;
         L.Xq0 = take((size_t)L.mpad0 * L.D);
         L.xsq0 = take((size_t)L.mpad0);
-        L.vp0 = take(L.nsplit0 > 1 ? (size_t)L.nsplit0 * L.mpad0 * L.KO * 2 : 0);
+        L.prows0 = eval_part_rows(L.mpad0, L.nsplit0, check ? eval_npieces(ctx, pr.n, (int)((pr.n + 63) / 64), L.D, L.nsplit0) : 0);
+        L.vp0 = take(L.nsplit0 > 1 ? L.prows0 * L.KO * 2 : 0);
         L.gp0 = take((size_t)0);
         L.V0 = take((size_t)pr.n * k);
         L.mpad1 = round_up(pr.m, 64);
         L.nsplit1 = pr.m > 0 ? eval_nsplit(ctx, pr.m, (int)((pr.n + 63) / 64)) : 1;
         L.Xq1 = take((size_t)L.mpad1 * L.D);
         L.xsq1 = take((size_t)L.mpad1);
-        L.vp1 = take(L.nsplit1 > 1 ? (size_t)L.nsplit1 * L.mpad1 * L.KO * 2 : 0);
-        L.gp1 = take((pr.jac_out && L.nsplit1 > 1) ? (size_t)L.nsplit1 * L.mpad1 * L.KO * L.D : 0);
+        L.prows1 = eval_part_rows(L.mpad1, L.nsplit1, pr.m > 0 ? eval_npieces(ctx, pr.m, (int)((pr.n + 63) / 64), L.D, L.nsplit1) : 0);
+        L.vp1 = take(L.nsplit1 > 1 ? L.prows1 * L.KO * 2 : 0);
+        L.gp1 = take((pr.jac_out && L.nsplit1 > 1) ? L.prows1 * L.KO * L.D : 0);
         L.vals = (pr.m == 0 || (pr.vals_out && is_device_ptr(pr.vals_out))) ? (size_t)-1 : take((size_t)pr.m * k);
         L.jac = (pr.m == 0 || !pr.jac_out || is_device_ptr(pr.jac_out)) ? (size_t)-1 : take((size_t)pr.m * k * d);
         L.out = out0 + (size_t)8 * i;
@@ -283,12 +286,12 @@
         probs[i].mean_given = 1;
         for (int e = 0; e < 2; ++e) {
             EvalDesc &E = evs[(size_t)e * P + i];
-            eval_desc_model(E, &M, e == 0 ? (check ? pr.n : 0) : pr.m, e == 0 ? L.nsplit0 : L.nsplit1);
+            eval_desc_model(E, ctx, &M, e == 0 ? (check ? pr.n : 0) : pr.m, e == 0 ? L.nsplit0 : L.nsplit1);
             E.X = e == 0 ? C : X;
             E.Xq = base + (e == 0 ? L.Xq0 : L.Xq1);
             E.xsq = base + (e == 0 ? L.xsq0 : L.xsq1);
             E.vpart = base + (e == 0 ? L.vp0 : L.vp1);
-            E.sapart = E.vpart + (size_t)E.nsplit * E.mpad * L.KO;
+            E.sapart = E.vpart + (e == 0 ? L.prows0 : L.prows1) * L.KO;
             E.gpart = base + (e == 0 ? L.gp0 : L.gp1);
             E.vals = e == 0 ? base + L.V0 : (L.vals == (size_t)-1 ? pr.vals_out : base + L.vals);
             E.jac = e == 0 ? nullptr : (pr.jac_out ? (L.jac == (size_t)-1 ? pr.jac_out : base + L.jac) : nullptr);
diff --git a/morbit.jl_amd/csrc/batch_chain.hpp b/morbit.jl_amd/csrc/batch_chain.hpp
--- a/morbit.jl_amd/csrc/batch_chain.hpp
+++ b/morbit.jl_amd/csrc/batch_chain.hpp
@@ -24,6 +24,7 @@
     size_t Xq = 0, xsq = 0, vpart = 0, gpart = 0;
     int64_t mpad = 0;
     int nsplit = 1, KO = 0;
+    size_t prows = 0;
 };
 struct Group {
     int site, D, k;
@@ -42,6 +43,7 @@
         Member mb;
         mb.site = site, mb.j = j, mb.p = p, mb.M = M, mb.mq = mq, mb.jac = jac;
         mb.nsplit = eval_nsplit(ctx, mq, (int)((M->n + 63) / 64));
+        mb.prows = eval_part_rows(round_up(mq, 64), mb.nsplit, eval_npieces(ctx, mq, (int)((M->n + 63) / 64), M->dpad, mb.nsplit));
         mb.group = group_of(ctx, site, M, jac, mb.nsplit > 1);
         if (mb.group >= 0) groups[mb.group].members.push_back(mem.size());
         mem.push_back(mb);
@@ -59,23 +61,23 @@
             S.KO = outputs_per_pass(S.M->k, S.M->dpad, S.jac);
             S.Xq = take((size_t)S.mpad * S.M->dpad);
             S.xsq = take((size_t)S.mpad);
-            S.vpart = take(S.nsplit > 1 ? (size_t)S.nsplit * S.mpad * S.KO * 2 : 0);
-            S.gpart = take((S.nsplit > 1 && S.jac) ? (size_t)S.nsplit * S.mpad * S.KO * S.M->dpad : 0);
+            S.vpart = take(S.nsplit > 1 ? S.prows * S.KO * 2 : 0);
+            S.gpart = take((S.nsplit > 1 && S.jac) ? S.prows * S.KO * S.M->dpad : 0);
         }
     }
-    void fill(double *base, EvalDesc *hdesc) const {
+    void fill(const mrbf_ctx *ctx, double *base, EvalDesc *hdesc) const {
         for (const Group &G : groups)
             for (size_t r = 0; r < G.members.size(); ++r) {
                 const Member &S = mem[G.members[r]];
                 EvalDesc E;
                 std::memset(&E, 0, sizeof(E));
-                eval_desc_model(E, S.M, S.mq, S.nsplit);
+                eval_desc_model(E, ctx, S.M, S.mq, S.nsplit);
                 E.X = base + S.X;
                 E.Xq = base + S.Xq;
                 E.xsq = base + S.xsq;
                 if (S.nsplit > 1) {
                     E.vpart = base + S.vpart;
-                    E.sapart = E.vpart + (size_t)S.nsplit * S.mpad * S.KO;
+                    E.sapart = E.vpart + S.prows * S.KO;
                     if (S.jac) E.gpart = base + S.gpart;
                 }
                 E.vals = base + S.vals;
diff --git a/morbit.jl_amd/csrc/chol_blocked.hip b/morbit.jl_amd/csrc/chol_blocked.hip
--- a/morbit.jl_amd/csrc/chol_blocked.hip
+++ b/morbit.jl_amd/csrc/chol_blocked.hip
@@ -12,37 +12,12 @@
 int launch_diag_v4(mrbf_ctx *ctx, hipStream_t st, double *Ajj, int64_t lda, double *Linv, int *dinfo, int col0);
 
 template <int TM, int MODE>
-__global__ __launch_bounds__(256, 2) void chol_update_kernel(const double *__restrict__ A, int64_t lda,
-                                                             const double *__restrict__ B, int64_t ldb,
-                                                             double *__restrict__ C, int64_t ldc, int K,
-                                                             const int *__restrict__ info, int mt_sq = 0, int ntiles_total = 0,
-                                                             const double *__restrict__ cvec = nullptr, double cs = 0.0, int64_t cn = 0) {
+__device__ __forceinline__ void update_tile(const double *__restrict__ A, int64_t lda, const double *__restrict__ B, int64_t ldb,
+                                            double *__restrict__ C, int64_t ldc, int K, int64_t I0, int64_t J0, bool diag,
+                                            const double *__restrict__ cvec, double cs, int64_t cn, double *smem) {
     constexpr int NJ = (TM == 128) ? 4 : 2;
-    __shared__ __attribute__((aligned(16))) double smem[mega::NSTG * mega::STG];
-    if (info && *info != 0) return;
-    if (MODE == UPD_OVERWRITE || MODE == UPD_COLUMN_SUB) __builtin_amdgcn_s_setprio(2);
     const int tid = threadIdx.x, lane = tid & 63, wave = tid >> 6;
     const int l15 = lane & 15, l4 = lane >> 4;
-    const int tile_end = (MODE == UPD_LOWER_SUB && ntiles_total > 0) ? ntiles_total : (int)blockIdx.x + 1;
-    for (int bid = blockIdx.x; bid < tile_end; bid += gridDim.x) {
-    int ti, tj;
-    if (MODE == UPD_LOWER_SUB) {
-        const int ntri = mt_sq * (mt_sq + 1) / 2;
-        if (bid < ntri || mt_sq == 0) {
-            int t = (int)((sqrt(8.0 * (double)bid + 1.0) - 1.0) * 0.5);
-            while ((t + 1) * (t + 2) / 2 <= bid) ++t;
-            while (t * (t + 1) / 2 > bid) --t;
-            ti = t;
-            tj = bid - t * (t + 1) / 2;
-        } else {
-            ti = mt_sq + (bid - ntri) / mt_sq;
-            tj = (bid - ntri) % mt_sq;
-        }
-    } else {
-        ti = blockIdx.x;
-        tj = blockIdx.y;
-    }
-    const int64_t I0 = (int64_t)ti * TM, J0 = (int64_t)tj * 128;
     const int ioff = (TM == 128) ? (wave >> 1) * 64 : 0;
     const int joff = (TM == 128) ? (wave & 1) * 64 : wave * 32;
 
@@ -110,11 +85,52 @@
                 } else {
                     double x = -acc[j][i][r];
                     if (cvec) x -= fma(cei[i], cvj[r], cvi[i] * cej[r]);
-                    if (ti != tj || gi >= gj) *dst = x;
+                    if (!diag || gi >= gj) *dst = x;
                 }
             }
         }
     }
+}
+
+template <int TM, int MODE>
+__global__ __launch_bounds__(256, 2) void chol_update_kernel(const double *__restrict__ A, int64_t lda,
+                                                             const double *__restrict__ B, int64_t ldb,
+                                                             double *__restrict__ C, int64_t ldc, int K,
+                                                             const int *__restrict__ info, int mt_sq = 0, int ntiles_total = 0,
+                                                             const double *__restrict__ cvec = nullptr, double cs = 0.0, int64_t cn = 0,
+                                                             int half_from = 0x7fffffff) {
+    __shared__ __attribute__((aligned(16))) double smem[mega::NSTG * mega::STG];
+    if (info && *info != 0) return;
+    if (MODE == UPD_OVERWRITE || MODE == UPD_COLUMN_SUB) __builtin_amdgcn_s_setprio(2);
+    const int tile_end = (MODE == UPD_LOWER_SUB && ntiles_total > 0) ? ntiles_total : (int)blockIdx.x + 1;
+    for (int bid = blockIdx.x; bid < tile_end; bid += gridDim.x) {
+    int ti, tj, half = -1;
+    if (MODE == UPD_LOWER_SUB) {
+        int t_id = bid;
+        if (TM == 128 && bid >= half_from) {
+            t_id = half_from + ((bid - half_from) >> 1);
+            half = (bid - half_from) & 1;
+        }
+        const int ntri = mt_sq * (mt_sq + 1) / 2;
+        if (t_id < ntri || mt_sq == 0) {
+            int t = (int)((sqrt(8.0 * (double)t_id + 1.0) - 1.0) * 0.5);
+            while ((t + 1) * (t + 2) / 2 <= t_id) ++t;
+            while (t * (t + 1) / 2 > t_id) --t;
+            ti = t;
+            tj = t_id - t * (t + 1) / 2;
+        } else {
+            ti = mt_sq + (t_id - ntri) / mt_sq;
+            tj = (t_id - ntri) % mt_sq;
+        }
+    } else {
+        ti = blockIdx.x;
+        tj = blockIdx.y;
+    }
+    const int64_t I0 = (int64_t)ti * TM, J0 = (int64_t)tj * 128;
+    if (TM == 128 && MODE == UPD_LOWER_SUB && half >= 0)
+        update_tile<64, UPD_LOWER_SUB>(A, lda, B, ldb, C, ldc, K, I0 + 64 * half, J0, ti == tj, cvec, cs, cn, smem);
+    else
+        update_tile<TM, MODE>(A, lda, B, ldb, C, ldc, K, I0, J0, MODE == UPD_LOWER_SUB && ti == tj, cvec, cs, cn, smem);
     if (bid + (int)gridDim.x < tile_end) __syncthreads();
     }
 }
@@ -399,8 +415,11 @@
 int launch_update_lower(mrbf_ctx *ctx, const double *A, int64_t lda, const double *B, int64_t ldb, double *C, int64_t ldc, int64_t nt,
                         int K, const double *cvec, double cs, int64_t cn) {
     if (nt <= 0 || K <= 0) return 0;
-    hipLaunchKernelGGL((chol_update_kernel<128, UPD_LOWER_SUB>), dim3((unsigned)(nt * (nt + 1) / 2)), dim3(256), 0, ctx->stream, A,
-                       lda, B, ldb, C, ldc, K, (const int *)nullptr, (int)nt, 0, cvec, cs, cn);
+    const int64_t ntiles = nt * (nt + 1) / 2, slots = 2 * (int64_t)ctx->ncu, rem = ntiles % slots;
+    const bool halves = ntiles > slots && rem > 0 && 4 * rem <= slots;
+    const int64_t half_from = halves ? ntiles - rem : ntiles;
+    hipLaunchKernelGGL((chol_update_kernel<128, UPD_LOWER_SUB>), dim3((unsigned)(ntiles + (ntiles - half_from))), dim3(256), 0,
+                       ctx->stream, A, lda, B, ldb, C, ldc, K, (const int *)nullptr, (int)nt, 0, cvec, cs, cn, (int)half_from);
     MRBF_HIP(ctx, hipGetLastError());
     return 0;
 }
diff --git a/morbit.jl_amd/csrc/common.hpp b/morbit.jl_amd/csrc/common.hpp
--- a/morbit.jl_amd/csrc/common.hpp
+++ b/morbit.jl_amd/csrc/common.hpp
@@ -103,6 +103,8 @@
     std::vector<mrbf::Buf> model_pool;
     int gram_mode = 0, residual = 1, force_path = 0, chol_impl = 0, eval_impl = 0, timing = 1, diag_impl = 0, chol_window = 0;
     int spin_ms = 1000, debug_fault = 0;
+    double *debug_k_out = nullptr;
+    size_t debug_k_cap = 0;
     unsigned long long *mega_stat_dev = nullptr;
     long mega_stat_shape = 0;
     int mega_stat_pending = 0;
diff --git a/morbit.jl_amd/csrc/eval_fused.hip b/morbit.jl_amd/csrc/eval_fused.hip
--- a/morbit.jl_amd/csrc/eval_fused.hip
+++ b/morbit.jl_amd/csrc/eval_fused.hip
@@ -13,6 +13,15 @@
 
 constexpr int EQ = 64;
 constexpr int EC = 64;
+
+__device__ __forceinline__ int64_t uni64(int64_t v) {
+    const unsigned lo = __builtin_amdgcn_readfirstlane((unsigned)(uint64_t)v), hi = __builtin_amdgcn_readfirstlane((unsigned)((uint64_t)v >> 32));
+    return (int64_t)(((uint64_t)hi << 32) | lo);
+}
+template <class T>
+__device__ __forceinline__ T *uniptr(T *p) {
+    return reinterpret_cast<T *>((uintptr_t)uni64((int64_t)(uintptr_t)p));
+}
 
 template <int KID, bool FAST, int KOUT, bool JAC, bool FINAL>
 __global__ __launch_bounds__(256, 2) void eval_fused_kernel(EvalDesc one, const EvalDesc *__restrict__ many, int l0) {
@@ -21,24 +30,48 @@
     __shared__ double Ws[KOUT * EC];
     __shared__ double Sq[EC];
     const EvalDesc &E = many ? many[blockIdx.z] : one;
-    if (many && ((int64_t)blockIdx.x * EQ >= E.mpad || (int)blockIdx.y >= E.nsplit)) return;
-    const double *__restrict__ Xq = E.Xq;
-    const double *__restrict__ Cc = E.Cc;
-    const double *__restrict__ csq = E.csq;
-    const double *__restrict__ Wc = E.Wc;
-    const int64_t npad = E.npad, mpad = E.mpad;
-    const int tiles_per_split = E.tiles_per_split;
+    const int npieces = FINAL ? 0 : __builtin_amdgcn_readfirstlane(E.npieces);
+    const int ntiles_all = __builtin_amdgcn_readfirstlane(E.ntiles);
+    int64_t u_cur, u_end;
+    int seg_q;
+    if (npieces > 0) {
+        const int g = (int)(blockIdx.y * gridDim.x + blockIdx.x);
+        if (g >= npieces) return;
+        const int64_t units = (uni64(E.mpad) / EQ) * ntiles_all;
+        u_cur = eval_piece_start(units, npieces, g);
+        u_end = eval_piece_start(units, npieces, g + 1);
+        seg_q = (int)(u_cur / ntiles_all);
+    } else {
+        if (many && ((int64_t)blockIdx.x * EQ >= E.mpad || (int)blockIdx.y >= E.nsplit)) return;
+        const int tps = __builtin_amdgcn_readfirstlane(E.tiles_per_split);
+        seg_q = blockIdx.x;
+        u_cur = (int64_t)seg_q * ntiles_all + (int64_t)blockIdx.y * tps;
+        u_end = u_cur + min(tps, ntiles_all - (int)blockIdx.y * tps);
+    }
+    u_cur = uni64(u_cur), u_end = uni64(u_end), seg_q = __builtin_amdgcn_readfirstlane(seg_q);
+    const double *__restrict__ Xq = uniptr(E.Xq);
+    const double *__restrict__ xsq = uniptr(E.xsq);
+    const double *__restrict__ Cc = uniptr(E.Cc);
+    const double *__restrict__ csq = uniptr(E.csq);
+    const double *__restrict__ Wc = uniptr(E.Wc);
+    const int64_t npad = uni64(E.npad), mpad = uni64(E.mpad);
+    double *__restrict__ vpart = uniptr(E.vpart), *__restrict__ sapart = uniptr(E.sapart), *__restrict__ gpart = uniptr(E.gpart);
     const KP kp = E.kp;
     const int tid = threadIdx.x, lane = tid & 63, wave = tid >> 6;
     const int l15 = lane & 15, l4 = lane >> 4;
-    const int64_t q0 = (int64_t)blockIdx.x * EQ;
-    const int split = blockIdx.y;
+    const int nsub = __builtin_amdgcn_readfirstlane(E.nsub);
+    for (; u_cur < u_end; ++seg_q) {
+    const int t0 = (int)(u_cur - (int64_t)seg_q * ntiles_all);
+    const int my_tiles = (int)min((int64_t)(ntiles_all - t0), u_end - u_cur);
+    u_cur += my_tiles;
+    const int64_t q0 = (int64_t)seg_q * EQ;
     const int64_t qrow = q0 + wave * 16 + l15;
+    const int64_t prow0 = npieces > 0 ? (int64_t)((int)(blockIdx.y * gridDim.x + blockIdx.x) + seg_q) * EQ : (int64_t)blockIdx.y * mpad + q0;
 
     double xb[D / 4];
 #pragma unroll
     for (int s = 0; s < D / 4; ++s) xb[s] = Xq[qrow * D + 4 * s + l4];
-    const double xs = E.xsq[qrow];
+    const double xs = xsq[qrow];
 
     v4d JT[KOUT][DT];
     double vsum[KOUT], sasum[KOUT];
@@ -50,10 +83,7 @@
         for (int t = 0; t < DT; ++t) JT[l][t] = (v4d){0.0, 0.0, 0.0, 0.0};
     }
 
-    const int64_t c_begin = (int64_t)split * tiles_per_split * EC;
-    const int ntiles_all = E.ntiles;
-    const int nsub = __builtin_amdgcn_readfirstlane(E.nsub);
-    const int my_tiles = min(tiles_per_split, ntiles_all - split * tiles_per_split);
+    const int64_t c_begin = (int64_t)t0 * EC;
     constexpr int NLD = 2 * DT;
     v2d stg[NLD];
     auto load_tile = [&](int64_t c0) {
@@ -147,12 +177,11 @@
         sasum[l] += __shfl_xor(sasum[l], 32);
     }
     if constexpr (!FINAL) {
-        double *__restrict__ vpart = E.vpart, *__restrict__ sapart = E.sapart, *__restrict__ gpart = E.gpart;
         if (l4 == 0) {
 #pragma unroll
             for (int l = 0; l < KOUT; ++l) {
-                vpart[((int64_t)split * mpad + qrow) * KOUT + l] = vsum[l];
-                sapart[((int64_t)split * mpad + qrow) * KOUT + l] = sasum[l];
+                vpart[(prow0 + wave * 16 + l15) * KOUT + l] = vsum[l];
+                sapart[(prow0 + wave * 16 + l15) * KOUT + l] = sasum[l];
             }
         }
         if (JAC) {
@@ -167,7 +196,7 @@
                 __syncthreads();
                 for (int e = lane; e < 16 * D; e += 64) {
                     const int qq = e / D, t = e % D;
-                    gpart[(((int64_t)split * mpad + q0 + wave * 16 + qq) * KOUT + l) * D + t] = T[qq * LDC + t];
+                    gpart[((prow0 + wave * 16 + qq) * KOUT + l) * D + t] = T[qq * LDC + t];
                 }
                 __syncthreads();
             }
@@ -229,6 +258,8 @@
                 __syncthreads();
             }
         }
+    }
+    if constexpr (FINAL) break;
     }
 }
 
@@ -593,15 +624,36 @@
     }
 }
 
+struct PartRows {
+    int count;
+    int64_t first, stride;
+    __device__ PartRows(const EvalDesc &E, int64_t p) {
+        if (E.npieces > 0) {
+            const int64_t qt = p / EQ, units = (E.mpad / EQ) * E.ntiles;
+            const int g0 = eval_piece_of_unit(units, E.npieces, qt * E.ntiles), g1 = eval_piece_of_unit(units, E.npieces, (qt + 1) * E.ntiles - 1);
+            count = g1 - g0 + 1;
+            first = (g0 + qt) * EQ + (p % EQ);
+            stride = EQ;
+        } else {
+            count = E.nsplit;
+            first = p;
+            stride = E.mpad;
+        }
+    }
+    __device__ int64_t row(int s) const { return first + (int64_t)s * stride; }
+};
+
 template <int KOUT>
 __global__ __launch_bounds__(128) void eval_combine_kernel(EvalDesc one, const EvalDesc *__restrict__ many, int l0, int D) {
     const EvalDesc &E = many ? many[blockIdx.y] : one;
-    const int64_t p = blockIdx.x, m = E.m, mpad = E.mpad;
+    const int64_t p = blockIdx.x, m = E.m;
     if (p >= m) return;
     const double *__restrict__ vpart = E.vpart, *__restrict__ sapart = E.sapart, *__restrict__ gpart = E.gpart;
     const double *__restrict__ Xq = E.Xq, *__restrict__ Xorig = E.X, *__restrict__ lam = E.lam;
     double *__restrict__ vals = E.vals, *__restrict__ jac = E.jac;
-    const int nsplit = E.nsplit, d = E.d, k = E.k, q = E.q;
+    const int d = E.d, k = E.k, q = E.q;
+    const PartRows pr(E, p);
+    const int nsplit = pr.count;
     __shared__ double sa[KOUT], sv[KOUT];
     __shared__ double pdot[KOUT][128];
     const int tid = threadIdx.x;
@@ -611,8 +663,8 @@
             double xv[8], xa[8];
 #pragma unroll
             for (int u = 0; u < 8; ++u) {
-                xv[u] = s0 + u < nsplit ? vpart[((int64_t)(s0 + u) * mpad + p) * KOUT + tid] : 0.0;
-                xa[u] = s0 + u < nsplit ? sapart[((int64_t)(s0 + u) * mpad + p) * KOUT + tid] : 0.0;
+                xv[u] = s0 + u < nsplit ? vpart[pr.row(s0 + u) * KOUT + tid] : 0.0;
+                xa[u] = s0 + u < nsplit ? sapart[pr.row(s0 + u) * KOUT + tid] : 0.0;
             }
 #pragma unroll
             for (int u = 0; u < 8; ++u)
@@ -652,7 +704,7 @@
         for (int s0 = 0; s0 < nsplit; s0 += 8) {
             double x[8];
 #pragma unroll
-            for (int u = 0; u < 8; ++u) x[u] = s0 + u < nsplit ? gpart[(((int64_t)(s0 + u) * mpad + p) * KOUT + l) * D + t] : 0.0;
+            for (int u = 0; u < 8; ++u) x[u] = s0 + u < nsplit ? gpart[(pr.row(s0 + u) * KOUT + l) * D + t] : 0.0;
 #pragma unroll
             for (int u = 0; u < 8; ++u)
                 if (s0 + u < nsplit) g += x[u];
@@ -667,17 +719,19 @@
 __global__ __launch_bounds__(256) void eval_combine_vals_kernel(EvalDesc one, const EvalDesc *__restrict__ many, int l0) {
     const EvalDesc &E = many ? many[blockIdx.y] : one;
     const int lane = threadIdx.x & 63, wave = threadIdx.x >> 6;
-    const int64_t p = (int64_t)blockIdx.x * 4 + wave, m = E.m, mpad = E.mpad;
+    const int64_t p = (int64_t)blockIdx.x * 4 + wave, m = E.m;
     const bool active = p < m;
     const double *__restrict__ vpart = E.vpart, *__restrict__ Xorig = E.X, *__restrict__ lam = E.lam;
-    const int nsplit = E.nsplit, d = E.d, k = E.k, q = E.q;
+    const int d = E.d, k = E.k, q = E.q;
+    const PartRows pr(E, active ? p : 0);
+    const int nsplit = pr.count;
     __shared__ double pdot[4][KOUT][128];
     double v = 0.0;
     if (active && lane < KOUT && l0 + lane < k) {
         for (int s0 = 0; s0 < nsplit; s0 += 8) {
             double x[8];
 #pragma unroll
-            for (int u = 0; u < 8; ++u) x[u] = s0 + u < nsplit ? vpart[((int64_t)(s0 + u) * mpad + p) * KOUT + lane] : 0.0;
+            for (int u = 0; u < 8; ++u) x[u] = s0 + u < nsplit ? vpart[pr.row(s0 + u) * KOUT + lane] : 0.0;
 #pragma unroll
             for (int u = 0; u < 8; ++u)
                 if (s0 + u < nsplit) v += x[u];
@@ -753,6 +807,12 @@
     return nsplit;
 }
 
+int eval_npieces(const mrbf_ctx *ctx, int64_t m, int ntiles, int dpad, int nsplit) {
+    if (dpad != 64 || ntiles <= 8 || nsplit <= 1 || m <= 0) return 0;
+    if (mrbf_env("MRBF_EVAL_NSPLIT") && atoi(mrbf_env("MRBF_EVAL_NSPLIT")) > 0) return 0;
+    return eval_piece_count(round_up(m, EQ) / EQ, ntiles, 2 * ctx->ncu);
+}
+
 int outputs_per_pass(int k, int D, bool want_jac) { return (k < 2 || (D == 256 && want_jac)) ? 1 : 2; }
 
 template <int KID, bool FAST, int KOUT, bool JAC, bool FINAL>
@@ -818,11 +878,12 @@
     if (count <= 0) return 0;
     if (D != 64 && D != 128 && D != 256) return fail(ctx, MRBF_EHIP, "eval_fused_batch needs dpad in {64, 128, 256}");
     int64_t max_mpad = 0, max_m = 0;
-    int max_split = 1;
+    int max_split = 1, max_pieces = 0;
     for (int p = 0; p < count; ++p) {
         max_mpad = std::max(max_mpad, host_descs[p].mpad);
         max_m = std::max(max_m, host_descs[p].m);
         max_split = std::max(max_split, host_descs[p].nsplit);
+        max_pieces = std::max(max_pieces, host_descs[p].npieces);
     }
     if (max_split > 1)
         for (int p = 0; p < count; ++p)
@@ -830,7 +891,9 @@
                 return fail(ctx, MRBF_EHIP, "eval_fused_batch: descriptor %d is unsplit in a group that splits the centre range", p);
     if (!centred)
         hipLaunchKernelGGL(center_pad_batch_kernel, dim3((unsigned)((max_mpad + 3) / 4), (unsigned)count), dim3(256), 0, ctx->stream, dev_descs, D);
-    dim3 grid((unsigned)(max_mpad / EQ), (unsigned)max_split, (unsigned)count);
+    const int64_t gx = max_mpad / EQ;
+    const int64_t gy = std::max<int64_t>(max_split, gx > 0 ? (max_pieces + gx - 1) / gx : 1);
+    dim3 grid((unsigned)gx, (unsigned)gy, (unsigned)count);
     dim3 cgrid((unsigned)max_m, (unsigned)count);
     return run_passes(ctx, kp, D, k, want_jac, max_split == 1, grid, cgrid, host_descs[0], dev_descs);
 }
@@ -846,14 +909,15 @@
     const int KO = outputs_per_pass(k, D, jac != nullptr);
     EvalDesc E;
     std::memset(&E, 0, sizeof(E));
-    eval_desc_model(E, M, m, nsplit);
+    eval_desc_model(E, ctx, M, m, nsplit);
     E.X = X;
     MRBF_TRY(get_buf(ctx, S_EVAL_XC, (size_t)mpad * D, &E.Xq));
     MRBF_TRY(get_buf(ctx, S_EVAL_XSQ, (size_t)mpad, &E.xsq));
     if (nsplit > 1) {
-        MRBF_TRY(get_buf(ctx, S_EVAL_SA, (size_t)nsplit * mpad * KO * 2, &E.vpart));
-        E.sapart = E.vpart + (size_t)nsplit * mpad * KO;
-        if (jac) MRBF_TRY(get_buf(ctx, S_EVAL_J, (size_t)nsplit * mpad * KO * D, &E.gpart));
+        const size_t prows = eval_part_rows(mpad, nsplit, E.npieces);
+        MRBF_TRY(get_buf(ctx, S_EVAL_SA, prows * KO * 2, &E.vpart));
+        E.sapart = E.vpart + prows * KO;
+        if (jac) MRBF_TRY(get_buf(ctx, S_EVAL_J, prows * KO * D, &E.gpart));
     }
     E.vals = vals;
     E.jac = jac;
@@ -861,6 +925,7 @@
     if (timing) MRBF_HIP(ctx, hipEventRecord(ctx->ev[4], ctx->stream));
     if (!(hints.pre_xq && hints.pre_xq == E.Xq)) MRBF_TRY(launch_center_pad(ctx, X, m, d, M->mean, nullptr, E.Xq, mpad, D, E.xsq));
     dim3 grid((unsigned)(mpad / EQ), (unsigned)nsplit);
+    if (E.npieces > 0) grid = dim3((unsigned)E.npieces, 1);
     MRBF_TRY(run_passes(ctx, M->kp, D, k, jac != nullptr, nsplit == 1, grid, dim3((unsigned)m), E, nullptr));
     if (timing) {
         MRBF_HIP(ctx, hipEventRecord(ctx->ev[7], ctx->stream));
@@ -874,3 +939,27 @@
 }
 
 }
+
+extern "C" int32_t mrbf_debug_eval_pieces(int64_t qtiles, int32_t ntiles, int32_t slots, int32_t cap, int32_t *out4) {
+    if (qtiles < 1 || qtiles > (1 << 24)) return -1;
+    if (ntiles < 1) return -2;
+    if (slots < 1) return -3;
+    if (cap < 0 || (cap > 0 && !out4)) return -4;
+    const int G = mrbf::eval_piece_count(qtiles, ntiles, slots);
+    const int64_t units = qtiles * ntiles;
+    int32_t np = 0;
+    for (int g = 0; g < G; ++g) {
+        int64_t u = mrbf::eval_piece_start(units, G, g);
+        const int64_t u1 = mrbf::eval_piece_start(units, G, g + 1);
+        while (u < u1) {
+            const int64_t qt = u / ntiles, t0 = u - qt * ntiles, len = std::min<int64_t>(ntiles - t0, u1 - u);
+            if (np < cap) {
+                int32_t *r = out4 + 4 * (size_t)np;
+                r[0] = g, r[1] = (int32_t)qt, r[2] = (int32_t)t0, r[3] = (int32_t)(t0 + len - 1);
+            }
+            ++np;
+            u += len;
+        }
+    }
+    return np;
+}
diff --git a/morbit.jl_amd/csrc/normal_batch.hip b/morbit.jl_amd/csrc/normal_batch.hip
--- a/morbit.jl_amd/csrc/normal_batch.hip
+++ b/morbit.jl_amd/csrc/normal_batch.hip
@@ -157,7 +157,7 @@
     MRBF_TRY(batch_fetch(ctx, shape->b_ineq, shape->n_lin_ineq, hup + oB + shape->n_lin_eq));
     EvalDesc *hdesc = reinterpret_cast<EvalDesc *>(hup + oDesc);
     const EvalDesc *ddesc = reinterpret_cast<const EvalDesc *>(base + oDesc);
-    ev.fill(base, hdesc);
+    ev.fill(ctx, base, hdesc);
     hipStream_t st = ctx->stream;
     hipEvent_t e0 = ctx->ev[0], e1 = ctx->ev[1];
     MRBF_HIP(ctx, hipEventRecord(e0, st));
diff --git a/morbit.jl_amd/csrc/sd_batch.hip b/morbit.jl_amd/csrc/sd_batch.hip
--- a/morbit.jl_amd/csrc/sd_batch.hip
+++ b/morbit.jl_amd/csrc/sd_batch.hip
@@ -168,7 +168,7 @@
     double *dPairs = base + oPairs, *dX = base + oX;
     EvalDesc *hdesc = reinterpret_cast<EvalDesc *>(hup + oDesc);
     const EvalDesc *ddesc = reinterpret_cast<const EvalDesc *>(base + oDesc);
-    ev.fill(base, hdesc);
+    ev.fill(ctx, base, hdesc);
     hipStream_t st = ctx->stream;
     hipEvent_t e0 = ctx->ev[0], e1 = ctx->ev[1];
     MRBF_HIP(ctx, hipEventRecord(e0, st));
diff --git a/morbit.jl_amd/csrc/small.hpp b/morbit.jl_amd/csrc/small.hpp
--- a/morbit.jl_amd/csrc/small.hpp
+++ b/morbit.jl_amd/csrc/small.hpp
@@ -70,9 +70,27 @@
     int nsub;
     KP kp;
     double *vpart, *sapart, *gpart;
+    int npieces;
     double *vals, *jac;
 };
-inline void eval_desc_model(EvalDesc &E, const mrbf_model *M, int64_t m, int nsplit) {
+inline int eval_piece_count(int64_t qtiles, int ntiles, int slots) {
+    const int64_t units = qtiles * ntiles;
+    return (int)std::max<int64_t>(std::min<int64_t>(slots, units), qtiles);
+}
+__host__ __device__ inline int64_t eval_piece_start(int64_t units, int G, int64_t g) {
+    const int64_t base = units / G, extra = units % G;
+    return g * base + (g < extra ? g : extra);
+}
+__host__ __device__ inline int eval_piece_of_unit(int64_t units, int G, int64_t u) {
+    const int64_t base = units / G, extra = units % G, lng = extra * (base + 1);
+    return (int)(u < lng ? u / (base + 1) : extra + (u - lng) / base);
+}
+inline size_t eval_part_rows(int64_t mpad, int nsplit, int npieces) {
+    return npieces > 0 ? (size_t)(npieces + mpad / 64) * 64 : (size_t)nsplit * mpad;
+}
+int eval_npieces(const mrbf_ctx *ctx, int64_t m, int ntiles, int dpad, int nsplit);
+
+inline void eval_desc_model(EvalDesc &E, const mrbf_ctx *ctx, const mrbf_model *M, int64_t m, int nsplit) {
     E.mean = M->mean;
     E.Cc = M->Xc;
     E.csq = M->sq;
@@ -89,6 +107,7 @@
     E.ntiles = (int)((M->n + 63) / 64);
     E.nsub = (int)((M->n + 15) / 16);
     E.tiles_per_split = (E.ntiles + nsplit - 1) / nsplit;
+    E.npieces = eval_npieces(ctx, m, E.ntiles, M->dpad, nsplit);
 }
 int eval_nsplit(const mrbf_ctx *ctx, int64_t m, int ntiles, bool check_call = false, bool population = false);
 int outputs_per_pass(int k, int D, bool want_jac = true);
diff --git a/morbit.jl_amd/csrc/solve.hip b/morbit.jl_amd/csrc/solve.hip
--- a/morbit.jl_amd/csrc/solve.hip
+++ b/morbit.jl_amd/csrc/solve.hip
@@ -688,6 +688,13 @@
         hipLaunchKernelGGL(build_panels_kernel, dim3(nblk(npad * K2)), dim3(256), 0, ctx->stream, Q1, Wm, scal, n, npad, q, K2, skip, PA, PB, v0);
         MRBF_TRY(launch_update_lower(ctx, PA, npad, PB, npad, Phi, ld, npad / 128, K2, v0, 1.0 / std::sqrt((double)n), n));
     }
+    if (ctx->debug_k_out && q > 0) {
+        double *dst = ctx->debug_k_out;
+        ctx->debug_k_out = nullptr;
+        if ((size_t)npad * npad > ctx->debug_k_cap) return fail(ctx, MRBF_EHIP, "mrbf_debug_capture_k: buffer too small for %lld x %lld", (long long)npad, (long long)npad);
+        MRBF_HIP(ctx, hipMemcpy2DAsync(dst, npad * sizeof(double), Phi, ld * sizeof(double), npad * sizeof(double), npad, hipMemcpyDefault, ctx->stream));
+        MRBF_HIP(ctx, hipStreamSynchronize(ctx->stream));
+    }
     MRBF_HIP(ctx, hipEventRecord(ctx->ev[2], ctx->stream));
     int hinfo = 0;
     double *linv_all = nullptr;
```

New measurement: 176.8 (median of 6 runs). Within noise of the previous version (+0.6%).
